# Daniel-Liu-c0deb0t/block-aligner

Measured on AMD Instinct MI355X. Metric: GCUPS (DP cells/s) on 10 kbp DNA X-drop batch; bit-exact score+CIGAR vs AVX2, higher is better.
Workload: dtype i16 (saturating lane scores) + i32 block offsets

## Files before the change

### block_aligner_amd/csrc/ba_driver.hpp

```cpp
#pragma once
#include "ba_device.hpp"

namespace ba {

#ifndef BA_BIG
#define BA_BIG 0
#endif
constexpr bool kBig = BA_BIG != 0;
__device__ __forceinline__ void lds_sync() {
    if (kBig) __builtin_amdgcn_fence(__ATOMIC_ACQ_REL, "workgroup");
    else __builtin_amdgcn_fence(__ATOMIC_ACQ_REL, "wavefront");
    __builtin_amdgcn_wave_barrier();
}
__device__ __forceinline__ void lds_fill0(short* a, uint32_t n) {
    for (uint32_t k = 2 * lane_id(); k < n; k += 128) *(int*)(a + k) = 0;
    lds_sync();
}
__device__ __forceinline__ void lds_copy(short* dst, const short* src, uint32_t n) {
    lds_sync();
    for (uint32_t k = 2 * lane_id(); k < n; k += 128) {
        const int v = *(const int*)(src + k);
        lds_sync();
        *(int*)(dst + k) = v;
    }
    lds_sync();
}
__device__ __forceinline__ int lds_prefix_max8(const short* a) {
    lds_sync();
    const int* p = (const int*)a;
    const s16x2 m = as_s(vmax(vmax(p[0], p[1]), vmax(p[2], p[3])));
    return uni(max((int)m.x, (int)m.y));
}
__device__ __forceinline__ int lds_suffix_max2(const short* a, uint32_t n) {
    lds_sync();
    s16x2 m = as_s(*(const int*)(a + n - 2));
    return uni(max((int)m.x, (int)m.y));
}
__device__ __forceinline__ int lds_shift_and_offset(uint32_t n, short* b1, short* b2, const short* t1, const short* t2, int off_add) {
    const int oa = splat(off_add);
    lds_sync();
    const int corner = uni((int)as_s(adds(splat((int)b1[STEP - 1]), oa)).x);
    for (uint32_t base = 0; base < n; base += 128) {
        const uint32_t k = base + 2 * lane_id();
        int v1 = 0, v2 = 0;
        const bool in = k < n;
        if (in) {
            if (k + STEP < n) {
                v1 = adds(*(const int*)(b1 + k + STEP), oa);
                v2 = adds(*(const int*)(b2 + k + STEP), oa);
            } else {
                v1 = *(const int*)(t1 + (k + STEP - n));
                v2 = *(const int*)(t2 + (k + STEP - n));
            }
        }
        lds_sync();
        if (in) { *(int*)(b1 + k) = v1; *(int*)(b2 + k) = v2; }
        lds_sync();
    }
    return corner;
}

struct Move { uint32_t op, di, dj, next; };
constexpr uint32_t TB_PENDING = 3;
__device__ __forceinline__ Move tb_lut(bool right_blk, uint32_t t, uint32_t t2, uint32_t table) {
    constexpr uint32_t OP_M = 1, OP_I = 4, OP_D = 5;
    const uint32_t gapA_op = right_blk ? OP_D : OP_I, gapB_op = right_blk ? OP_I : OP_D;
    const uint32_t A_di = right_blk ? 0 : 1, A_dj = right_blk ? 1 : 0;
    const uint32_t A_tab = right_blk ? 1 : 2, B_tab = right_blk ? 2 : 1;
    if (table == A_tab) return (t2 & 1) ? Move{gapA_op, A_di, A_dj, 0} : Move{gapA_op, A_di, A_dj, A_tab};
    if (table == B_tab) return Move{gapB_op, 1 - A_di, 1 - A_dj, TB_PENDING};
    if (t == 0) return Move{OP_M, 1, 1, 0};
    if (t & 1) return (t2 & 1) ? Move{gapA_op, A_di, A_dj, 0} : Move{gapA_op, A_di, A_dj, A_tab};
    return Move{gapB_op, 1 - A_di, 1 - A_dj, TB_PENDING};
}
__device__ __forceinline__ uint32_t tb_resolve(bool right_blk, uint32_t table, uint32_t nib) {
    return table == TB_PENDING ? ((nib & 8u) ? 0u : (right_blk ? 2u : 1u)) : table;
}
__device__ __forceinline__ uint32_t tb_next(bool right_blk, uint32_t next, uint32_t v) {
    return (next == TB_PENDING && v == 0) ? (right_blk ? 2u : 1u) : next;
}

__device__ __forceinline__ uint32_t traceback(const BlockRec* __restrict__ blocks, uint32_t nblocks, const uint32_t* __restrict__ trace,
                                     uint32_t i, uint32_t j, const uint8_t* __restrict__ q, const uint8_t* __restrict__ r, uint32_t flags,
                                     uint32_t* __restrict__ out, uint64_t out_lo, uint64_t out_hi, uint32_t* status) {
    const bool eq = flags & F_CIGAR_EQ, local = flags & F_LOCAL, fqs = flags & F_FQS;
    bool stop = false;
    uint64_t wp = out_hi;
    uint32_t run_op = 0, run_len = 0;
    uint32_t table = 0;
    uint32_t bidx = nblocks;
    while ((i > 0 || j > 0) && !stop) {
        BlockRec br;
        for (;;) {
            if (bidx == 0) { *status |= ST_TRACEBACK_LOST; return 0; }
            bidx--;
            br = blocks[bidx];
            if (i >= (br.i & 0x7fffffffu) && j >= br.j) break;
        }
        const bool right_blk = br.trace_base >> 31;
        const bool l2 = br.i >> 31;
        br.i &= 0x7fffffffu;
        if (br.trace_base & 0x40000000u) { *status |= ST_TRACEBACK_LOST; return 0; }
        const uint32_t tbase = br.trace_base & 0x3fffffffu;
        const uint32_t Hv = right_blk ? br.h : br.w;
        const uint32_t nch = Hv > 128 ? Hv / 128 : 1, nl = Hv > 128 ? 64 : Hv / 2;
        while (i >= br.i && j >= br.j && (i > 0 || j > 0)) {
            const uint32_t ci = i - br.i, cj = j - br.j;
            const uint32_t v = right_blk ? ci : cj, w = right_blk ? cj : ci;
            const uint32_t chunk = v >> 7, lane = (v & 127) >> 1;
            if (right_blk && fqs && i == 0) { stop = true; break; }
            uint32_t nib;
            if (l2) {
                const uint32_t word = trace[tbase + (v >> 3) * 8 + (w >> 1) * 2 + ((v >> 2) & 1)];
                nib = ((word >> ((v & 3) * 8 + (w & 1) * 4)) ^ 15u) & 15u;
            } else {
                const uint32_t word = trace[tbase + (((w >> 2) * nch + chunk) * nl + lane) * (local ? 2u : 1u)];
                nib = ((word >> ((v & 1) * 16 + (w & 3) * 4)) ^ 15u) & 15u;
            }
            table = tb_resolve(right_blk, table, nib);
            if (local && table == 0) {
                if (l2) {
                    const uint32_t z = trace[tbase + (uint32_t)br.h * br.w / 8 + (v >> 3) * 2 + ((v >> 2) & 1)];
                    if ((z >> ((v & 3) * 8 + w)) & 1) { stop = true; break; }
                } else {
                    const uint32_t z = trace[tbase + (((w >> 2) * nch + chunk) * nl + lane) * 2u + 1u];
                    if ((z >> ((v & 1) * 16 + (w & 3) * 4)) & 1) { stop = true; break; }
                }
            }
            const Move m = tb_lut(right_blk, nib & 3, (nib >> 2) & 1, table);
            uint32_t op = m.op;
            if (eq && op == 1) op = q[i] == r[j] ? 2 : 3;
            if (m.di > i || m.dj > j) { *status |= ST_TRACEBACK_LOST; return 0; }
            i -= m.di; j -= m.dj; table = tb_next(right_blk, m.next, v);
            if (op == run_op) run_len++;
            else {
                if (run_len) {
                    if (wp == out_lo) { *status |= ST_CIGAR_OVERFLOW; return 0; }
                    out[--wp] = (run_len << 4) | run_op;
                }
                run_op = op; run_len = 1;
            }
        }
    }
    if (run_len) {
        if (wp == out_lo) { *status |= ST_CIGAR_OVERFLOW; return 0; }
        out[--wp] = (run_len << 4) | run_op;
    }
    return (uint32_t)(out_hi - wp);
}

__device__ __forceinline__ uint32_t wave_excl_sum(uint32_t x, uint32_t lane) {
    uint32_t s = x;
#pragma unroll
    for (int d = 1; d < 64; d <<= 1) {
        const uint32_t o = (uint32_t)__shfl_up((int)s, d, 64);
        s += lane >= (uint32_t)d ? o : 0u;
    }
    return s - x;
}
template <bool L2OK>
__device__ __forceinline__ uint32_t walk_wave(const BlockRec* __restrict__ blocks, uint32_t nblocks_in, const uint32_t* __restrict__ trace,
                                              uint32_t i_in, uint32_t j_in, const uint8_t* __restrict__ q, const uint8_t* __restrict__ r, bool eq,
                                              uint32_t* __restrict__ out, uint64_t out_lo, uint64_t out_hi, uint32_t* status,
                                              uint32_t* __restrict__ lds, uint32_t budget) {
    const uint32_t lane = (uint32_t)lane_id();
    uint32_t lutv0, lutv1;
    {
        const Move a = tb_lut(false, lane & 3, (lane >> 2) & 1, (lane >> 4) & 3), b = tb_lut(true, lane & 3, (lane >> 2) & 1, (lane >> 4) & 3);
        lutv0 = a.op | (a.di << 3) | (a.dj << 4) | (a.next << 5);
        lutv1 = b.op | (b.di << 3) | (b.dj << 4) | (b.next << 5);
    }
    uint32_t i = (uint32_t)uni((int)i_in), j = (uint32_t)uni((int)j_in), bidx = (uint32_t)uni((int)nblocks_in);
    uint32_t table = 0, run_op = 0, run_len = 0, nrun = 0, runbuf = 0, st = 0;
    uint64_t wp = out_hi;
    uint32_t qw0 = 0, rw0 = 0, qwin = 0, rwin = 0;
    auto load_q = [&]() { qw0 = i >= 252u ? (i - 252u) & ~3u : 0u; const uint32_t a = qw0 + 4u * lane; qwin = a <= i ? *(const uint32_t*)(q + a) : 0u; };
    auto load_r = [&]() { rw0 = j >= 252u ? (j - 252u) & ~3u : 0u; const uint32_t a = rw0 + 4u * lane; rwin = a <= j ? *(const uint32_t*)(r + a) : 0u; };
    if (eq) { load_q(); load_r(); }
    auto flush = [&]() {
        if (lane < nrun) out[wp - 1u - lane] = runbuf;
        wp -= nrun; nrun = 0;
    };
    auto emit = [&]() -> bool {
        if (!run_len) return true;
        if (wp - nrun == out_lo) return false;
        asm volatile("s_mov_b32 m0, %2\n\tv_writelane_b32 %0, %1, m0" : "+v"(runbuf) : "s"(__builtin_amdgcn_readfirstlane((int)((run_len << 4) | run_op))), "s"(__builtin_amdgcn_readfirstlane((int)nrun)) : "m0");
        if (++nrun == 64u) flush();
        return true;
    };
    bool ok = true;
    while (ok && (i > 0 || j > 0)) {
        if (bidx == 0) { st = ST_TRACEBACK_LOST; ok = false; break; }
        const uint32_t nvalid = min(bidx, 64u);
        uint4 rec = uint4{0, 0, 0, 0};
        if (lane < nvalid) rec = *(const uint4*)(blocks + (bidx - 1u - lane));
        const bool untr = rec.w & 0x40000000u;
        const uint32_t words = untr ? 0u : (rec.z & 0xffffu) * (rec.z >> 16) / 8u;
        const uint32_t tb = rec.w & 0x3fffffffu;
        uint32_t toff = wave_excl_sum(lane < nvalid ? words : 0u, lane);
        const uint32_t nfit = (uint32_t)__popcll(__ballot(lane < nvalid && toff + words <= budget));
        const uint32_t tb_up = (uint32_t)__shfl_up((int)tb, 1, 64);
        const bool flat = nfit > 1 && !__any(lane > 0 && lane < nfit && tb + words != tb_up);
        if (nfit > 0) {
            const uint32_t total = (uint32_t)__builtin_amdgcn_readlane((int)(toff + words), (int)(nfit - 1u));
            if (flat) {
                const uint32_t lo = (uint32_t)__builtin_amdgcn_readlane((int)tb, (int)(nfit - 1u));
                for (uint32_t x = lane; x < total; x += 64u) lds[x] = trace[lo + x];
                toff = tb - lo;
            } else {
                for (uint32_t k = 0; k < nfit; k++) {
                    const uint32_t base = (uint32_t)__builtin_amdgcn_readlane((int)tb, (int)k), sz = (uint32_t)__builtin_amdgcn_readlane((int)words, (int)k);
                    const uint32_t off = (uint32_t)__builtin_amdgcn_readlane((int)toff, (int)k);
                    for (uint32_t x = lane; x < sz; x += 64u) lds[off + x] = trace[base + x];
                }
            }
            asm volatile("s_waitcnt vmcnt(0) lgkmcnt(0)" ::: "memory");
        }
        const bool direct = nfit == 0;
        const uint32_t ntake = direct ? 1u : nfit;
        auto walk_rects = [&](auto direct_c) {
        constexpr bool DIRECT = decltype(direct_c)::value;
        uint32_t cur = 0;
        while (cur < ntake && ok && (i > 0 || j > 0)) {
            const uint32_t rx = (uint32_t)__builtin_amdgcn_readlane((int)rec.x, (int)cur), bj = (uint32_t)__builtin_amdgcn_readlane((int)rec.y, (int)cur);
            const uint32_t bi = rx & 0x7fffffffu;
            if (!(i >= bi && j >= bj)) { cur++; continue; }
            const uint32_t rz = (uint32_t)__builtin_amdgcn_readlane((int)rec.z, (int)cur), rw = (uint32_t)__builtin_amdgcn_readlane((int)rec.w, (int)cur);
            if (rw & 0x40000000u) { st = ST_TRACEBACK_LOST; ok = false; break; }
            const uint32_t off = DIRECT ? (rw & 0x3fffffffu) : (uint32_t)__builtin_amdgcn_readlane((int)toff, (int)cur);
            const bool right = rw >> 31, l2 = L2OK && (rx >> 31);
            const uint32_t Hv = right ? (rz & 0xffffu) : (rz >> 16);
            const uint32_t nch = Hv > 128u ? Hv / 128u : 1u, nl = Hv > 128u ? 64u : Hv / 2u;
            const uint32_t lutr = right ? lutv1 : lutv0;
            while (i >= bi && j >= bj && (i > 0 || j > 0)) {
                const uint32_t ci = i - bi, cj = j - bj;
                const uint32_t v = right ? ci : cj, w = right ? cj : ci;
                uint32_t widx, sh;
                if (l2) { widx = (v >> 3) * 8u + (w >> 1) * 2u + ((v >> 2) & 1u); sh = (v & 3u) * 8u + (w & 1u) * 4u; }
                else { widx = ((w >> 2) * nch + (v >> 7)) * nl + ((v & 127u) >> 1); sh = (v & 1u) * 16u + (w & 3u) * 4u; }
                uint32_t word;
                if (table == 0u && i > 0u && j > 0u && min(v, w) >= 1u) {
                    const uint32_t lim = min(min(v, w), min(i, j) - 1u);
                    const bool valid = lane <= lim;
                    const uint32_t vv = v - lane, ww = w - lane;
                    uint32_t widx_k, sh_k;
                    if (l2) { widx_k = (vv >> 3) * 8u + (ww >> 1) * 2u + ((vv >> 2) & 1u); sh_k = (vv & 3u) * 8u + (ww & 1u) * 4u; }
                    else { widx_k = ((ww >> 2) * nch + (vv >> 7)) * nl + ((vv & 127u) >> 1); sh_k = (vv & 1u) * 16u + (ww & 3u) * 4u; }
                    uint32_t word_k = 0;
                    if (valid) { if constexpr (DIRECT) word_k = trace[off + widx_k]; else word_k = lds[off + widx_k]; }
                    const unsigned long long cm = __ballot(valid && ((word_k >> sh_k) & 3u) == 3u);
                    uint32_t n = cm == ~0ull ? 64u : (uint32_t)__builtin_ctzll(~cm);
                    if (eq && n >= 2u) {
                        if (i < qw0) load_q();
                        if (j < rw0) load_r();
                        n = min(n, min(i - qw0, j - rw0) + 1u);
                    }
                    if (n >= 2u) {
                        bool fits = true;
                        if (!eq) {
                            if (run_op == 1u) run_len += n;
                            else { fits = emit(); run_op = 1u; run_len = n; }
                        } else {
                            const uint32_t qa = i - lane - qw0, ra = j - lane - rw0;
                            const uint32_t qd = (uint32_t)__builtin_amdgcn_ds_bpermute((int)(qa & ~3u), (int)qwin), rd = (uint32_t)__builtin_amdgcn_ds_bpermute((int)(ra & ~3u), (int)rwin);
                            const bool same = ((qd >> ((qa & 3u) * 8u)) & 255u) == ((rd >> ((ra & 3u) * 8u)) & 255u);
                            unsigned long long bits = __ballot(lane < n && same);
                            uint32_t rem = n;
                            while (rem && fits) {
                                const bool e = bits & 1ull;
                                const unsigned long long x = e ? ~bits : bits;
                                const uint32_t len = min(x ? (uint32_t)__builtin_ctzll(x) : 64u, rem), op2 = e ? 2u : 3u;
                                if (op2 == run_op) run_len += len;
                                else { fits = emit(); run_op = op2; run_len = len; }
                                bits = len < 64u ? bits >> len : 0ull; rem -= len;
                            }
                        }
                        if (!fits) { st = ST_CIGAR_OVERFLOW; ok = false; break; }
                        i -= n; j -= n;
                        continue;
                    }
                    word = (uint32_t)__builtin_amdgcn_readlane((int)word_k, 0);
                } else {
                if constexpr (DIRECT) word = (uint32_t)uni((int)trace[off + widx]); else word = (uint32_t)uni((int)lds[off + widx]);
                }
                const uint32_t nib = ((word >> sh) ^ 15u) & 15u;
                table = tb_resolve(right, table, nib);
                const uint32_t m = (uint32_t)__builtin_amdgcn_readlane((int)lutr, (int)((table << 4) | nib));
                uint32_t op = m & 7u;
                const uint32_t di = (m >> 3) & 1u, dj = (m >> 4) & 1u;
                if (eq && op == 1u) {
                    if (i < qw0) load_q();
                    if (j < rw0) load_r();
                    const uint32_t qd = (uint32_t)__builtin_amdgcn_readlane((int)qwin, (int)((i - qw0) >> 2)), rd = (uint32_t)__builtin_amdgcn_readlane((int)rwin, (int)((j - rw0) >> 2));
                    op = ((qd >> ((i & 3u) * 8u)) & 255u) == ((rd >> ((j & 3u) * 8u)) & 255u) ? 2u : 3u;
                }
                if (di > i || dj > j) { st = ST_TRACEBACK_LOST; ok = false; break; }
                i -= di; j -= dj; table = tb_next(right, m >> 5, v);
                if (op == run_op) run_len++;
                else {
                    if (!emit()) { st = ST_CIGAR_OVERFLOW; ok = false; break; }
                    run_op = op; run_len = 1;
                }
            }
        }
        };
        if (direct) walk_rects(std::true_type{}); else walk_rects(std::false_type{});
        bidx -= ntake;
    }
    if (ok && !emit()) { st = ST_CIGAR_OVERFLOW; ok = false; }
    if (!ok) { *status |= st; return 0; }
    flush();
    return (uint32_t)(out_hi - wp);
}

#define BA_RLX_AGENT __ATOMIC_RELAXED, __HIP_MEMORY_SCOPE_AGENT

struct TbLane {
    uint32_t slot, pair, i, j, table, bidx, run_op, run_len, status;
    uint64_t wp, lo;
    const BlockRec* blocks; const uint32_t* trace; const uint8_t* q; const uint8_t* r;
    uint32_t bi, bj, tbase, zoff, nch, nl; bool right, in_rect, l2;
    uint4 nrec[4]; uint32_t nq;
    uint32_t tw_chunk, tw_g, tw_lane0; bool tw_ok;
    uint32_t qw0, rw0;
    uint32_t pv[6], po[6], pmask;
};

__device__ __forceinline__ void tb_emit(TbLane& t, uint32_t* __restrict__ out) {
    if (t.run_len) {
        if (t.wp == t.lo) { t.status |= ST_CIGAR_OVERFLOW; t.i = t.j = 0; return; }
        out[--t.wp] = (t.run_len << 4) | t.run_op;
    }
}
__device__ __forceinline__ void tb_fail(TbLane& t) { t.status |= ST_TRACEBACK_LOST; t.i = t.j = 0; t.run_len = 0; }

constexpr int TB_CELLS_PER_STEP = 4;
#ifndef BA_WALK_CELLS
#define BA_WALK_CELLS 8
#endif
#ifndef BA_RING_DEPTH
#define BA_RING_DEPTH 2
#endif
#ifndef BA_WALK_DEPTH
#define BA_WALK_DEPTH 4
#endif
#ifndef BA_HELPER_CELLS
#define BA_HELPER_CELLS 4
#endif
template <int CELLS = TB_CELLS_PER_STEP, int DEPTH = 1, int LB = (int)TB_LANE_BYTES>
__device__ __forceinline__ void tb_step(TbLane& t, uint32_t flags, uint32_t* __restrict__ out, unsigned char* lrec,
                                        const unsigned char* lut, unsigned long long* tacc = nullptr) {
    constexpr bool LOCREC = LB == (int)TB_LANE_BYTES_LOC;
    constexpr bool L2OK = LB == (int)TB_LANE_BYTES_L2 || LOCREC;
    constexpr int SEQ_Q = LOCREC ? 80 : (L2OK ? 64 : 40), SEQ_R = SEQ_Q + 16;
    const bool eq = flags & F_CIGAR_EQ, local = LOCREC && (flags & F_LOCAL), fqs = flags & F_FQS;
    BA_TSTAMP(ts0);
    if (!t.in_rect || !(t.i >= t.bi && t.j >= t.bj)) {
        bool found = false, untraced = false;
#pragma unroll
        for (int a = 0; a < DEPTH; a++) {
            if (!found && (a == 0 || t.nq)) {
                if (t.bidx == 0) { tb_fail(t); return; }
                uint4 rec;
                if (t.nq) {
                    rec = t.nrec[0];
#pragma unroll
                    for (int k = 0; k + 1 < DEPTH; k++) t.nrec[k] = t.nrec[k + 1];
                    t.nq--;
                } else rec = *(const uint4*)(t.blocks + t.bidx - 1);
                t.bidx--;
                t.l2 = L2OK && (rec.x >> 31); t.bi = rec.x & 0x7fffffffu; t.bj = rec.y;
                const uint32_t h = rec.z & 0xffffu, w = rec.z >> 16;
                t.in_rect = t.i >= t.bi && t.j >= t.bj;
                t.zoff = h * w / 8;
                t.right = rec.w >> 31;
                t.tbase = rec.w & 0x3fffffffu;
                const uint32_t Hv = t.right ? h : w;
                t.nch = Hv > 128 ? Hv / 128 : 1; t.nl = Hv > 128 ? 64 : Hv / 2;
                untraced = rec.w & 0x40000000u;
                found = t.in_rect;
            }
        }
        if (t.nq == 0 && t.bidx > 0) {
#pragma unroll
            for (int k = 0; k < DEPTH; k++) if (t.bidx > (uint32_t)k) t.nrec[k] = *(const uint4*)(t.blocks + t.bidx - 1 - k);
            t.nq = min((uint32_t)DEPTH, t.bidx);
        }
        t.tw_ok = false;
        if (!t.in_rect) return;
        if (untraced) { tb_fail(t); return; }
    }
    {
        const uint32_t ci = t.i - t.bi, cj = t.j - t.bj;
        const uint32_t v = t.right ? ci : cj, w = t.right ? cj : ci;
        const uint32_t chunk = v >> 7, lc = (v & 127) >> 1, g = w >> 2;
        if (L2OK && t.l2) {
            const uint32_t L8 = v >> 3;
            if (!(t.tw_ok && t.tw_chunk == 0xffffu && L8 - t.tw_lane0 < 2u)) {
                t.tw_chunk = 0xffffu; t.tw_g = 0; t.tw_lane0 = L8 ? L8 - 1 : 0u; t.tw_ok = true;
                const uint32_t* wp = t.trace + t.tbase + t.tw_lane0 * 8;
                uint4 a0, a1, a2, a3;
                __builtin_memcpy(&a0, wp, 16); __builtin_memcpy(&a1, wp + 4, 16); __builtin_memcpy(&a2, wp + 8, 16); __builtin_memcpy(&a3, wp + 12, 16);
                uint4* lw = (uint4*)lrec;
                lw[0] = a0; lw[1] = a1; lw[2] = a2; lw[3] = a3;
                if (local) {
                    uint4 z;
                    __builtin_memcpy(&z, t.trace + t.tbase + t.zoff + t.tw_lane0 * 2, 16);
                    lw[4] = z;
                }
            }
        } else
        if (local) {
            if (!(t.tw_ok && chunk == t.tw_chunk && t.tw_g - g < 2u && lc - t.tw_lane0 < 5u)) {
                t.tw_chunk = chunk; t.tw_g = g; t.tw_lane0 = min(lc >= 4 ? lc - 4 : 0u, t.nl - 5u); t.tw_ok = true;
                const uint32_t* hi = t.trace + t.tbase + ((g * t.nch + chunk) * t.nl + t.tw_lane0) * 2u;
                const uint32_t* lo = g ? hi - t.nch * t.nl * 2u : hi;
                uint4 h0, h1, l0, l1; uint2 h2, l2;
                __builtin_memcpy(&h0, hi, 16); __builtin_memcpy(&h1, hi + 4, 16); __builtin_memcpy(&h2, hi + 8, 8);
                __builtin_memcpy(&l0, lo, 16); __builtin_memcpy(&l1, lo + 4, 16); __builtin_memcpy(&l2, lo + 8, 8);
                uint32_t* lw = (uint32_t*)lrec;
                lw[0] = h0.x; lw[1] = h0.y; lw[2] = h0.z; lw[3] = h0.w; lw[4] = h1.x; lw[5] = h1.y; lw[6] = h1.z; lw[7] = h1.w; lw[8] = h2.x; lw[9] = h2.y;
                lw[10] = l0.x; lw[11] = l0.y; lw[12] = l0.z; lw[13] = l0.w; lw[14] = l1.x; lw[15] = l1.y; lw[16] = l1.z; lw[17] = l1.w; lw[18] = l2.x; lw[19] = l2.y;
            }
        } else
        if (!(t.tw_ok && chunk == t.tw_chunk && t.tw_g - g < 2u && lc - t.tw_lane0 < 5u)) {
            t.tw_chunk = chunk; t.tw_g = g; t.tw_lane0 = min(lc >= 4 ? lc - 4 : 0u, t.nl - 5u); t.tw_ok = true;
            const uint32_t* hi = t.trace + t.tbase + (g * t.nch + chunk) * t.nl + t.tw_lane0;
            const uint32_t* lo = g ? hi - t.nch * t.nl : hi;
            uint32_t wv[10];
            {
                uint4 h4, l4;
                __builtin_memcpy(&h4, hi, 16); __builtin_memcpy(&l4, lo, 16);
                wv[0] = h4.x; wv[1] = h4.y; wv[2] = h4.z; wv[3] = h4.w; wv[4] = hi[4];
                wv[5] = l4.x; wv[6] = l4.y; wv[7] = l4.z; wv[8] = l4.w; wv[9] = lo[4];
            }
#pragma unroll
            for (int k = 0; k < 10; k++) ((uint32_t*)lrec)[k] = wv[k];
        }
        if (eq) {
            if (t.qw0 == 0xffffffffu || t.i < t.qw0 + 8 || t.i >= t.qw0 + 16) {
                t.qw0 = t.i >= 12 ? (t.i - 12) & ~3u : 0;
                const uint32_t* p = (const uint32_t*)(t.q + t.qw0);
                uint32_t b4[4];
#pragma unroll
                for (int k = 0; k < 4; k++) b4[k] = p[k];
#pragma unroll
                for (int k = 0; k < 4; k++) ((uint32_t*)lrec)[SEQ_Q / 4 + k] = b4[k];
            }
            if (t.rw0 == 0xffffffffu || t.j < t.rw0 + 8 || t.j >= t.rw0 + 16) {
                t.rw0 = t.j >= 12 ? (t.j - 12) & ~3u : 0;
                const uint32_t* p = (const uint32_t*)(t.r + t.rw0);
                uint32_t b4[4];
#pragma unroll
                for (int k = 0; k < 4; k++) b4[k] = p[k];
#pragma unroll
                for (int k = 0; k < 4; k++) ((uint32_t*)lrec)[SEQ_R / 4 + k] = b4[k];
            }
        }
    }
#ifdef BA_TIMING
    const unsigned long long ts1 = __builtin_amdgcn_s_memtime();
    asm volatile("s_waitcnt vmcnt(0)" ::: "memory");
    const unsigned long long ts2 = __builtin_amdgcn_s_memtime();
    if (tacc) { tacc[0] += ts1 - ts0; tacc[1] += ts2 - ts1; }
#endif
    {
        bool alive = true;
#pragma unroll
        for (int s = 0; s < CELLS; s++) {
            alive = alive && (t.i > 0 || t.j > 0) && t.i >= t.bi && t.j >= t.bj;
            const uint32_t ci = t.i - t.bi, cj = t.j - t.bj;
            const uint32_t v = t.right ? ci : cj, w = t.right ? cj : ci;
            const uint32_t lc = (v & 127) >> 1;
            if (fqs) {
                const bool stop = alive && t.right && t.i == 0;
                if (stop) t.i = t.j = 0;
                alive = alive && !stop;
            }
            const uint32_t gi = t.tw_g - (w >> 2);
            uint32_t baddr, zaddr = 0, zbit = 0;
            if (L2OK && t.l2) {
                const uint32_t k8 = (v >> 3) - t.tw_lane0;
                alive = alive && t.tw_chunk == 0xffffu && k8 <= 1u;
                baddr = k8 * 32 + (w >> 1) * 8 + ((v >> 2) & 1) * 4 + (v & 3);
                zaddr = 64 + k8 * 8 + ((v >> 2) & 1) * 4 + (v & 3); zbit = w;
            } else {
                const uint32_t k = lc - t.tw_lane0;
                alive = alive && (v >> 7) == t.tw_chunk && gi <= 1u && k <= 4u;
                baddr = local ? gi * 40 + k * 8 + (v & 1) * 2 + ((w & 3) >> 1) : gi * 20 + k * 4 + (v & 1) * 2 + ((w & 3) >> 1);
                zaddr = baddr + 4; zbit = (w & 1) * 4;
            }
            const uint32_t qo = t.i - t.qw0, ro = t.j - t.rw0;
            const uint32_t byte = lrec[alive ? baddr : 0u];
            const uint32_t qb = lrec[SEQ_Q + (qo & 15u)], rb = lrec[SEQ_R + (ro & 15u)];
            const uint32_t nib = ((byte >> ((w & 1) * 4)) ^ 15u) & 15u;
            const uint32_t table = tb_resolve(t.right, t.table, nib);
            if (local) {
                const uint32_t zb = lrec[alive ? zaddr : 0u];
                const bool stop = alive && table == 0 && ((zb >> zbit) & 1u);
                if (stop) t.i = t.j = 0;
                alive = alive && !stop;
            }
            const uint32_t m = lut[((uint32_t)t.right << 6) | (table << 4) | nib];
            uint32_t op = m & 7u;
            const uint32_t di = (m >> 3) & 1u, dj = (m >> 4) & 1u;
            const bool is_match = eq && op == 1;
            alive = alive && !(is_match && (qo > 15u || ro > 15u));
            if (is_match) op = qb == rb ? 2u : 3u;
            if (alive && (di > t.i || dj > t.j)) { tb_fail(t); alive = false; }
            const bool same = op == t.run_op;
            if (alive && !same && t.run_len) {
                if (t.wp == t.lo) { t.status |= ST_CIGAR_OVERFLOW; t.i = t.j = 0; alive = false; }
                else out[--t.wp] = (t.run_len << 4) | t.run_op;
            }
            t.i -= alive ? di : 0u; t.j -= alive ? dj : 0u;
            t.table = alive ? tb_next(t.right, m >> 5, v) : t.table;
            t.run_len = alive ? (same ? t.run_len + 1 : 1u) : t.run_len;
            t.run_op = alive ? op : t.run_op;
        }
    }
}

#ifndef BA_TB_FAST
#define BA_TB_FAST 1
#endif
#ifndef BA_TB_FCELLS
#define BA_TB_FCELLS 1
#endif
#ifndef BA_TB_DIAG_RUNS
#define BA_TB_DIAG_RUNS 2
#endif
#ifndef BA_TB_DIAG2
#define BA_TB_DIAG2 1
#endif
#ifndef BA_TB_FDEPTH
#define BA_TB_FDEPTH 3
#endif
typedef uint32_t tb_u32x4 __attribute__((ext_vector_type(4)));
__device__ __forceinline__ uint4 tb_ld16(const void* p) {
    typedef tb_u32x4 __attribute__((aligned(4))) V;
    const tb_u32x4 v = *(const V*)p;
    return uint4{v.x, v.y, v.z, v.w};
}
__device__ __forceinline__ uint32_t ffbl_u32(uint32_t x) { uint32_t r; asm("v_ffbl_b32 %0, %1" : "=v"(r) : "v"(x)); return r; }
__device__ __forceinline__ void tb_prefetch2(TbLane& t) {
    if (t.bidx > 0u) t.nrec[0] = *(const uint4*)(t.blocks + t.bidx - 1);
    if (t.bidx > 1u) t.nrec[1] = *(const uint4*)(t.blocks + t.bidx - 2);
    t.nq = min(2u, t.bidx);
}
template <bool L2W>
__device__ __forceinline__ void tb_diag_lut_fill(unsigned char* dlut) {
    if constexpr (L2W) {
#pragma unroll
        for (int e = 0; e < 3; e++) {
            const uint32_t idx = (uint32_t)lane_id() + 64u * e;
            const uint32_t k = idx & 7u, p = idx >> 3;
            const uint32_t x = (p - k) & 15u, c = ((p - 16u) - k) & 7u;
            dlut[idx] = (unsigned char)(p < 16u ? (((x & 8u) << 2) | (x & 7u)) : ((c >> 1) << 3));
        }
    }
    {
        const uint32_t idx = (uint32_t)lane_id(), k = idx & 7u, x = ((idx >> 3) - k) & 7u;
        dlut[(L2W ? TB_DIAG_LUT_L2 - TB_DIAG_LUT_STD : 0u) + idx] = (unsigned char)((x < 4u ? 20u : 0u) + ((x & 3u) >> 1));
    }
}
template <int S>
__device__ __forceinline__ void tb_push(TbLane& t, const bool cond, const uint32_t val, bool& ovf) {
    const bool room = t.wp != t.lo, go = cond && room;
    t.wp -= go ? 1u : 0u;
    t.pv[S] = go ? val : t.pv[S];
    t.po[S] = go ? (uint32_t)t.wp - (uint32_t)t.lo : t.po[S];
    t.pmask |= go ? (1u << S) : 0u;
    ovf = ovf || (cond && !room);
}
__device__ __forceinline__ void tb_flush(TbLane& t, uint32_t* __restrict__ out) {
#pragma unroll
    for (int s = 0; s < 6; s++) if ((t.pmask >> s) & 1u) out[t.lo + t.po[s]] = t.pv[s];
    t.pmask = 0;
}

template <bool L2W, int SEQ_Q, int SEQ_R, int S0>
__device__ __forceinline__ void tb_diag(TbLane& t, const bool eq, const unsigned char* lrec, const unsigned char* dlut, bool& ovf) {
    static_assert(BA_TB_DIAG_RUNS >= 1 && BA_TB_DIAG_RUNS <= 2, "two slots per call site");
    const uint32_t ci = t.i - t.bi, cj = t.j - t.bj;
    const uint32_t v = t.right ? ci : cj, w = t.right ? cj : ci;
    bool ok = t.in_rect && t.tw_ok && t.i >= t.bi && t.j >= t.bj && (t.table == 0u || t.table == TB_PENDING);
    uint32_t K = min(min(t.i, t.j), min(v, w) + 1u);
    uint32_t alo, ahi;
    {
        const uint32_t u = (v & 127u) - 2u * t.tw_lane0, x = w + 4u - 4u * t.tw_g;
        const bool ok_s = !t.l2 && (v >> 7) == t.tw_chunk && u < 10u && x < 8u;
        const uint32_t K_s = min(u, x) + 1u;
        const uint2 C = *(const uint2*)(dlut + (L2W ? TB_DIAG_LUT_L2 - TB_DIAG_LUT_STD : 0u) + (x & 7u) * 8u);
        const uint32_t r2 = (2u * (u & 15u)) * 0x01010101u;
        alo = ((r2 - 0x06040200u) + C.x) & 0x3f3f3f3fu; ahi = ((r2 - 0x0e0c0a08u) + C.y) & 0x3f3f3f3fu;
        if constexpr (L2W) {
            const uint32_t u2 = v - 8u * t.tw_lane0;
            const bool ok_2 = t.l2 && t.tw_chunk == 0xffffu && u2 < 16u;
            const uint2 F = *(const uint2*)(dlut + (u2 & 15u) * 8u), G = *(const uint2*)(dlut + 128u + (w & 7u) * 8u);
            alo = t.l2 ? F.x + G.x : alo; ahi = t.l2 ? F.y + G.y : ahi;
            ok = ok && (ok_2 || ok_s);
            K = min(K, t.l2 ? u2 + 1u : K_s);
        } else {
            ok = ok && ok_s;
            K = min(K, K_s);
        }
    }
    const uint32_t qo = t.i - t.qw0, ro = t.j - t.rw0;
    if (eq) { ok = ok && qo <= 15u && ro <= 15u; K = min(K, min(qo, ro) + 1u); }
    K = ok ? min(K, 8u) : 0u;
    uint32_t b[8];
#pragma unroll
    for (int k = 0; k < 8; k++) b[k] = lrec[((k < 4 ? alo : ahi) >> (8 * (k & 3))) & 0xffu];
    const uint32_t sh0 = (w & 1u) * 4u;
    const uint32_t e4 = (b[0] | (b[2] << 8) | (b[4] << 16) | (b[6] << 24)) >> sh0, o4 = (b[1] | (b[3] << 8) | (b[5] << 16) | (b[7] << 24)) >> (4u - sh0);
    const uint32_t z = ((e4 & (e4 >> 1)) & 0x01010101u) | (((o4 & (o4 >> 1)) & 0x01010101u) << 4);
    uint32_t n = ffbl_u32(~z & 0x11111111u) >> 2;
    const bool d_state = t.table == 0u || !((e4 >> 3) & 1u);
    n = d_state ? min(n, K) : 0u;
    uint32_t ne = 0;
    if (eq) {
        const unsigned char* qb = lrec + SEQ_Q + (ok ? qo : 7u) - 7u; const unsigned char* rb = lrec + SEQ_R + (ok ? ro : 7u) - 7u;
#pragma unroll
        for (int k = 0; k < 8; k++) ne |= min((uint32_t)qb[7 - k] ^ (uint32_t)rb[7 - k], 1u) << (4 * k);
    }
    uint32_t pos = 0;
#pragma unroll
    for (int it = 0; it < (BA_TB_DIAG_RUNS); it++) {
        if (it > 0 && !eq) break;
        const uint32_t rem = n - pos;
        const uint32_t cur = ne >> ((4u * pos) & 31u);
        const uint32_t is_x = cur & 1u;
        const uint32_t y = (cur ^ (0u - is_x)) & 0x11111111u;
        const uint32_t len = min(ffbl_u32(y) >> 2, rem);
        const uint32_t op = eq ? 2u + is_x : 1u;
        const bool same = op == t.run_op;
        if (it == 0) tb_push<S0>(t, rem > 0u && !same && t.run_len != 0u, (t.run_len << 4) | t.run_op, ovf);
        else tb_push<S0 + 1>(t, rem > 0u && !same && t.run_len != 0u, (t.run_len << 4) | t.run_op, ovf);
        t.run_len = same ? t.run_len + len : (rem > 0u ? len : t.run_len);
        t.run_op = rem > 0u ? op : t.run_op;
        pos += len;
    }
    t.i -= pos; t.j -= pos;
    t.table = pos ? 0u : t.table;
}

template <int DEPTH, int LB>
__device__ __forceinline__ void tb_step_fast(TbLane& t, const bool eq, uint32_t* __restrict__ out, unsigned char* lrec, const unsigned char* lut, const unsigned char* dlut) {
    static_assert(DEPTH >= 2 && DEPTH <= 4 && (BA_TB_FCELLS) >= 1 && (BA_TB_FCELLS) <= 2, "");
    constexpr bool L2OK = LB == (int)TB_LANE_BYTES_L2;
    constexpr int SEQ_Q = L2OK ? 64 : 40, SEQ_R = SEQ_Q + 16;
    if (!t.in_rect || !(t.i >= t.bi && t.j >= t.bj)) {
        if (t.bidx == 0) { tb_fail(t); return; }
        bool found = false;
        uint32_t take = t.nq;
        uint4 rec = t.nrec[0];
#pragma unroll
        for (int a = DEPTH - 1; a >= 0; a--) {
            const bool c = (uint32_t)a < t.nq && t.i >= (t.nrec[a].x & 0x7fffffffu) && t.j >= t.nrec[a].y;
            rec.x = c ? t.nrec[a].x : rec.x; rec.y = c ? t.nrec[a].y : rec.y; rec.z = c ? t.nrec[a].z : rec.z; rec.w = c ? t.nrec[a].w : rec.w;
            take = c ? (uint32_t)a + 1u : take;
            found = found || c;
        }
        const uint32_t nq_old = t.nq;
        t.bidx -= take;
        uint4 nn[DEPTH];
#pragma unroll
        for (int k = 0; k < DEPTH; k++) {
            nn[k] = t.nrec[k];
            bool have = false;
#pragma unroll
            for (int sft = 1; k + sft < DEPTH; sft++) {
                const bool m = take == (uint32_t)sft && (uint32_t)(k + sft) < nq_old;
                nn[k].x = m ? t.nrec[k + sft].x : nn[k].x; nn[k].y = m ? t.nrec[k + sft].y : nn[k].y; nn[k].z = m ? t.nrec[k + sft].z : nn[k].z; nn[k].w = m ? t.nrec[k + sft].w : nn[k].w;
                have = have || m;
            }
            if (!have && t.bidx > (uint32_t)k) nn[k] = *(const uint4*)(t.blocks + t.bidx - 1 - k);
        }
#pragma unroll
        for (int k = 0; k < DEPTH; k++) t.nrec[k] = nn[k];
        t.nq = min((uint32_t)DEPTH, t.bidx);
        t.in_rect = found;
        t.l2 = L2OK && (rec.x >> 31); t.bi = rec.x & 0x7fffffffu; t.bj = rec.y;
        t.right = rec.w >> 31;
        t.tbase = rec.w & 0x3fffffffu;
        const uint32_t Hv = t.right ? (rec.z & 0xffffu) : (rec.z >> 16);
        t.nch = Hv > 128 ? Hv / 128 : 1; t.nl = Hv > 128 ? 64 : Hv / 2;
        t.tw_ok = false;
        if (!found) return;
        if (rec.w & 0x40000000u) { tb_fail(t); return; }
    }
    const uint32_t ci0 = t.i - t.bi, cj0 = t.j - t.bj;
    const uint32_t v0 = t.right ? ci0 : cj0, w0 = t.right ? cj0 : ci0;
    const bool is_l2 = L2OK && t.l2;
    bool ld_l2 = false, ld_std = false;
    if constexpr (L2OK) {
        const uint32_t L8 = v0 >> 3;
        ld_l2 = is_l2 && !(t.tw_ok && t.tw_chunk == 0xffffu && L8 - t.tw_lane0 < 2u);
        if (ld_l2) { t.tw_chunk = 0xffffu; t.tw_g = 0; t.tw_lane0 = L8 ? L8 - 1 : 0u; t.tw_ok = true; }
    }
    {
        const uint32_t chunk = v0 >> 7, lc = (v0 & 127) >> 1, g = w0 >> 2;
        ld_std = !is_l2 && !(t.tw_ok && chunk == t.tw_chunk && t.tw_g - g < 2u && lc - t.tw_lane0 < 5u);
        if (ld_std) { t.tw_chunk = chunk; t.tw_g = g; t.tw_lane0 = min(lc >= 4 ? lc - 4 : 0u, t.nl - 5u); t.tw_ok = true; }
    }
    uint4 wa = {0, 0, 0, 0}, wb = {0, 0, 0, 0}, wc = {0, 0, 0, 0}, wd = {0, 0, 0, 0};
    {
        const uint32_t* tb0 = t.trace + t.tbase;
        const uint32_t o_hi = (t.tw_g * t.nch + t.tw_chunk) * t.nl + t.tw_lane0, o_lo = t.tw_g ? o_hi - t.nch * t.nl : o_hi;
        const uint32_t o_l2 = t.tw_lane0 * 8;
        const uint32_t o0 = is_l2 ? o_l2 : o_hi, o1 = is_l2 ? o_l2 + 4 : o_lo, o2 = is_l2 ? o_l2 + 8 : o_hi + 4, o3 = is_l2 ? o_l2 + 12 : o_lo + 4;
        if (ld_l2 || ld_std) { wa = tb_ld16(tb0 + o0); wb = tb_ld16(tb0 + o1); wc = tb_ld16(tb0 + o2); wd = tb_ld16(tb0 + o3); }
    }
    uint4 qv = {0, 0, 0, 0}, rv = {0, 0, 0, 0};
    const bool ld_q = eq && (t.qw0 == 0xffffffffu || t.i < t.qw0 + 8 || t.i >= t.qw0 + 16);
    const bool ld_r = eq && (t.rw0 == 0xffffffffu || t.j < t.rw0 + 8 || t.j >= t.rw0 + 16);
    if (ld_q) { t.qw0 = t.i >= 12 ? (t.i - 12) & ~3u : 0; qv = tb_ld16(t.q + t.qw0); }
    if (ld_r) { t.rw0 = t.j >= 12 ? (t.j - 12) & ~3u : 0; rv = tb_ld16(t.r + t.rw0); }
    tb_flush(t, out);
    if constexpr (L2OK) if (ld_l2) { uint4* lw = (uint4*)lrec; lw[0] = wa; lw[1] = wb; lw[2] = wc; lw[3] = wd; }
    if (ld_std) {
        uint32_t* lw = (uint32_t*)lrec;
        lw[0] = wa.x; lw[1] = wa.y; lw[2] = wa.z; lw[3] = wa.w; lw[4] = wc.x; lw[5] = wb.x; lw[6] = wb.y; lw[7] = wb.z; lw[8] = wb.w; lw[9] = wd.x;
    }
    if (ld_q) { uint32_t* lw = (uint32_t*)lrec + SEQ_Q / 4; lw[0] = qv.x; lw[1] = qv.y; lw[2] = qv.z; lw[3] = qv.w; }
    if (ld_r) { uint32_t* lw = (uint32_t*)lrec + SEQ_R / 4; lw[0] = rv.x; lw[1] = rv.y; lw[2] = rv.z; lw[3] = rv.w; }
    bool ovf = false;
    tb_diag<L2OK, SEQ_Q, SEQ_R, 0>(t, eq, lrec, dlut, ovf);
    {
        bool alive = true;
#pragma unroll
        for (int s = 0; s < (BA_TB_FCELLS); s++) {
            alive = alive && (t.i > 0 || t.j > 0) && t.i >= t.bi && t.j >= t.bj;
            const uint32_t ci = t.i - t.bi, cj = t.j - t.bj;
            const uint32_t v = t.right ? ci : cj, w = t.right ? cj : ci;
            const uint32_t lc = (v & 127) >> 1;
            const uint32_t gi = t.tw_g - (w >> 2);
            uint32_t baddr;
            if (L2OK && t.l2) {
                const uint32_t k8 = (v >> 3) - t.tw_lane0;
                alive = alive && t.tw_chunk == 0xffffu && k8 <= 1u;
                baddr = k8 * 32 + (w >> 1) * 8 + ((v >> 2) & 1) * 4 + (v & 3);
            } else {
                const uint32_t k = lc - t.tw_lane0;
                alive = alive && (v >> 7) == t.tw_chunk && gi <= 1u && k <= 4u;
                baddr = gi * 20 + k * 4 + (v & 1) * 2 + ((w & 3) >> 1);
            }
            const uint32_t qo = t.i - t.qw0, ro = t.j - t.rw0;
            const uint32_t byte = lrec[alive ? baddr : 0u];
            const uint32_t qb = lrec[SEQ_Q + (qo & 15u)], rb = lrec[SEQ_R + (ro & 15u)];
            const uint32_t nib = ((byte >> ((w & 1) * 4)) ^ 15u) & 15u;
            const uint32_t table = tb_resolve(t.right, t.table, nib);
            const uint32_t m = lut[((uint32_t)t.right << 6) | (table << 4) | nib];
            uint32_t op = m & 7u;
            const uint32_t di = (m >> 3) & 1u, dj = (m >> 4) & 1u;
            const bool is_match = eq && op == 1;
            alive = alive && !(is_match && (qo > 15u || ro > 15u));
            if (is_match) op = qb == rb ? 2u : 3u;
            if (alive && (di > t.i || dj > t.j)) { tb_fail(t); alive = false; }
            const bool same = op == t.run_op;
            if (s == 0) tb_push<2>(t, alive && !same && t.run_len != 0u, (t.run_len << 4) | t.run_op, ovf);
            else tb_push<3>(t, alive && !same && t.run_len != 0u, (t.run_len << 4) | t.run_op, ovf);
            t.i -= alive ? di : 0u; t.j -= alive ? dj : 0u;
            t.table = alive ? tb_next(t.right, m >> 5, v) : t.table;
            t.run_len = alive ? (same ? t.run_len + 1 : 1u) : t.run_len;
            t.run_op = alive ? op : t.run_op;
        }
    }
    if constexpr ((BA_TB_DIAG2) != 0) tb_diag<L2OK, SEQ_Q, SEQ_R, 4>(t, eq, lrec, dlut, ovf);
    if (ovf) { t.status |= ST_CIGAR_OVERFLOW; t.i = t.j = 0; }
}

template <int LB = (int)TB_LANE_BYTES, int CELLS = TB_CELLS_PER_STEP, int DEPTH = BA_RING_DEPTH>
__device__ __forceinline__ void traceback_consumer(const BatchParams& bp, uint32_t flag_mask, unsigned char* tb_lds, uint32_t nlanes, bool dedicated, int prio = -1) {
    enum { IDLE = 0, WAIT = 1, WALK = 2, RETIRED = 3 };
    int phase = (uint32_t)lane_id() < nlanes ? IDLE : RETIRED;
    uint32_t claimed = 0, pend = 0;
    const uint32_t reserve_from = bp.n > bp.tb_reserve ? bp.n - bp.tb_reserve : 0u;
    TbLane t{};
    const uint32_t eq = bp.flags & flag_mask;
    uint32_t* head = bp.tb_ctrl + 32;
    unsigned char* lut = tb_lds;
    unsigned char* lrec = tb_lds + TB_LUT_BYTES + (uint32_t)lane_id() * (uint32_t)LB;
    constexpr bool FASTP = (BA_TB_FAST) != 0 && LB != (int)TB_LANE_BYTES_LOC;
    unsigned char* dlut = tb_lds + ((TB_LUT_BYTES + nlanes * (uint32_t)LB + 7u) & ~7u);
#pragma unroll
    for (int e = 0; e < 2; e++) {
        const uint32_t idx = (uint32_t)lane_id() + 64u * e;
        const Move mv = tb_lut(idx >> 6, idx & 3, (idx >> 2) & 1, (idx >> 4) & 3);
        lut[idx] = (unsigned char)(mv.op | (mv.di << 3) | (mv.dj << 4) | (mv.next << 5));
    }
    if constexpr (FASTP) tb_diag_lut_fill<LB == (int)TB_LANE_BYTES_L2>(dlut);
    lds_sync();
#ifndef BA_TB_PRIO
#define BA_TB_PRIO 3
#endif
#ifndef MQ_TB_PRIO
#define MQ_TB_PRIO 1
#endif
    if (prio == 1) __builtin_amdgcn_s_setprio(MQ_TB_PRIO); else __builtin_amdgcn_s_setprio(BA_TB_PRIO);
#ifdef BA_TIMING
    unsigned long long c_sec[3] = {};
    unsigned long long c_iters = 0, c_walk_lanes = 0, c_walk_iters = 0, c_poll_iters = 0, c_walk_ticks = 0, c_t0 = __builtin_amdgcn_s_memtime();
#endif
    for (;;) {
#ifdef BA_TIMING
        const unsigned long long it0 = __builtin_amdgcn_s_memtime();
        const bool any_walk = __any(phase == WALK);
        c_iters++; c_walk_lanes += __popcll(__ballot(phase == WALK)); c_walk_iters += any_walk; c_poll_iters += __any(phase == WAIT);
#endif
        if (phase == IDLE) {
            if (dedicated && __hip_atomic_load(head, BA_RLX_AGENT) >= reserve_from) phase = RETIRED;
            else {
                claimed = __hip_atomic_fetch_add(head, 1u, BA_RLX_AGENT);
                phase = claimed >= bp.n ? RETIRED : WAIT;
            }
            pend = 0;
        }
        const bool got = phase == WAIT && pend != 0;
        const bool walking = phase == WALK;
        const uint32_t entry = pend;
        if (__any(got)) {
            __builtin_amdgcn_fence(__ATOMIC_ACQUIRE, "agent");
            if (got) __hip_atomic_store(bp.tb_queue + (claimed & bp.tb_qmask), 0u, BA_RLX_AGENT);
            if (got && (entry & 0x80000000u)) {
                bp.cig_len[entry & 0x7fffffffu] = 0;
                phase = IDLE;
            } else if (got) {
                t = TbLane{};
                t.qw0 = t.rw0 = 0xffffffffu; t.tw_ok = false;
                t.slot = entry - 1;
                const SlotInfo si = bp.slot_info[t.slot];
                t.pair = si.pair; t.i = si.end_i; t.j = si.end_j; t.bidx = si.nblocks;
                t.blocks = bp.blocks + (uint64_t)t.slot * bp.blocks_stride;
                t.trace = bp.trace_arena + (uint64_t)t.slot * bp.trace_stride;
                t.q = bp.pool + bp.q_off[t.pair]; t.r = bp.pool + bp.r_off[t.pair];
                t.lo = bp.cig_off[t.pair]; t.wp = bp.cig_off[t.pair + 1];
                t.status = bp.status[t.pair];
                if (t.status || (bp.flags & 0x200u)) t.i = t.j = 0;
                if constexpr (FASTP) tb_prefetch2(t);
                phase = WALK;
            }
        }
        if (walking) {
#ifdef BA_TIMING
            const unsigned long long tq0 = __builtin_amdgcn_s_memtime();
            if (t.i > 0 || t.j > 0) {
                if constexpr (FASTP) tb_step_fast<BA_TB_FDEPTH, LB>(t, eq != 0u, bp.cig_ops, lrec, lut, dlut);
                else tb_step<CELLS, DEPTH, LB>(t, eq, bp.cig_ops, lrec, lut, c_sec);
            }
            c_sec[2] += __builtin_amdgcn_s_memtime() - tq0;
#else
            if (t.i > 0 || t.j > 0) {
                if constexpr (FASTP) tb_step_fast<BA_TB_FDEPTH, LB>(t, eq != 0u, bp.cig_ops, lrec, lut, dlut);
                else
                if (BA_HELPER_CELLS != CELLS && !dedicated) tb_step<BA_HELPER_CELLS, BA_WALK_DEPTH, LB>(t, eq, bp.cig_ops, lrec, lut);
                else tb_step<CELLS, DEPTH, LB>(t, eq, bp.cig_ops, lrec, lut);
            }
#endif
            if (!(t.i > 0 || t.j > 0)) {
                if constexpr (FASTP) tb_flush(t, bp.cig_ops);
                tb_emit(t, bp.cig_ops);
                bp.cig_len[t.pair] = t.status ? 0u : (uint32_t)(bp.cig_off[t.pair + 1] - t.wp);
                if (t.status) bp.status[t.pair] = t.status;
                __hip_atomic_store(bp.slot_free + t.slot, 1u, BA_RLX_AGENT);
                phase = IDLE;
            }
        }
        if (phase == WAIT) pend = __hip_atomic_load(bp.tb_queue + (claimed & bp.tb_qmask), BA_RLX_AGENT);
#ifdef BA_TIMING
        if (any_walk) c_walk_ticks += __builtin_amdgcn_s_memtime() - it0;
#endif
        if (__all(phase == RETIRED)) break;
        if (!__any(phase == WALK)) __builtin_amdgcn_s_sleep(32);
    }
#ifdef BA_TIMING
    if (bp.prof && dedicated && is_lane(0)) {
        atomicAdd(bp.prof + 20, c_iters); atomicAdd(bp.prof + 21, c_walk_lanes); atomicAdd(bp.prof + 22, c_walk_iters);
        atomicAdd(bp.prof + 23, c_poll_iters); atomicAdd(bp.prof + 24, c_walk_ticks);
        atomicAdd(bp.prof + 25, __builtin_amdgcn_s_memtime() - c_t0); atomicAdd(bp.prof + 26, 1ull);
        atomicAdd(bp.prof + 27, c_sec[0]); atomicAdd(bp.prof + 28, c_sec[1]); atomicAdd(bp.prof + 29, c_sec[2]);
    }
#endif
}

template <int LB = (int)TB_LANE_BYTES>
__device__ __forceinline__ bool traceback_help_one(const BatchParams& bp, uint32_t flag_mask, unsigned char* tb_lds) {
    uint32_t entry = 0;
    if (is_lane(0)) {
        uint32_t h = __hip_atomic_load(bp.tb_ctrl + 32, BA_RLX_AGENT);
        if (h < bp.n) {
            const uint32_t e = __hip_atomic_load(bp.tb_queue + (h & bp.tb_qmask), BA_RLX_AGENT);
            if (e && __hip_atomic_compare_exchange_strong(bp.tb_ctrl + 32, &h, h + 1u, __ATOMIC_RELAXED, __ATOMIC_RELAXED, __HIP_MEMORY_SCOPE_AGENT)) {
                entry = e;
                __hip_atomic_store(bp.tb_queue + (h & bp.tb_qmask), 0u, BA_RLX_AGENT);
            }
        }
    }
    entry = (uint32_t)uni((int)entry);
    if (!entry) return false;
    if (entry & 0x80000000u) {
        if (is_lane(0)) bp.cig_len[entry & 0x7fffffffu] = 0;
        return true;
    }
    unsigned char* lut = tb_lds;
    unsigned char* lrec = tb_lds + TB_LUT_BYTES;
    lds_sync();
#pragma unroll
    for (int e = 0; e < 2; e++) {
        const uint32_t idx = (uint32_t)lane_id() + 64u * e;
        const Move mv = tb_lut(idx >> 6, idx & 3, (idx >> 2) & 1, (idx >> 4) & 3);
        lut[idx] = (unsigned char)(mv.op | (mv.di << 3) | (mv.dj << 4) | (mv.next << 5));
    }
    lds_sync();
    __builtin_amdgcn_fence(__ATOMIC_ACQUIRE, "agent");
    if (is_lane(0)) {
        const uint32_t eq = bp.flags & flag_mask;
        TbLane t{};
        t.qw0 = t.rw0 = 0xffffffffu; t.tw_ok = false;
        t.slot = entry - 1;
        const SlotInfo si = bp.slot_info[t.slot];
        t.pair = si.pair; t.i = si.end_i; t.j = si.end_j; t.bidx = si.nblocks;
        t.blocks = bp.blocks + (uint64_t)t.slot * bp.blocks_stride;
        t.trace = bp.trace_arena + (uint64_t)t.slot * bp.trace_stride;
        t.q = bp.pool + bp.q_off[t.pair]; t.r = bp.pool + bp.r_off[t.pair];
        t.lo = bp.cig_off[t.pair]; t.wp = bp.cig_off[t.pair + 1];
        t.status = bp.status[t.pair];
        if (t.status || (bp.flags & 0x200u)) t.i = t.j = 0;
        while (t.i > 0 || t.j > 0) tb_step<TB_CELLS_PER_STEP, BA_RING_DEPTH, LB>(t, eq, bp.cig_ops, lrec, lut);
        tb_emit(t, bp.cig_ops);
        bp.cig_len[t.pair] = t.status ? 0u : (uint32_t)(bp.cig_off[t.pair + 1] - t.wp);
        if (t.status) bp.status[t.pair] = t.status;
        __hip_atomic_store(bp.slot_free + t.slot, 1u, BA_RLX_AGENT);
    }
    lds_sync();
    return true;
}

template <bool L2OK>
__device__ __forceinline__ void traceback_helper_wave(const BatchParams& bp, uint32_t* lds, uint32_t budget) {
    uint32_t* head = bp.tb_ctrl + 32;
    for (;;) {
        uint32_t claimed = 0;
        if (is_lane(0)) claimed = __hip_atomic_fetch_add(head, 1u, BA_RLX_AGENT);
        claimed = (uint32_t)uni((int)claimed);
        if (claimed >= bp.n) break;
        uint32_t entry = 0;
        for (;;) {
            if (is_lane(0)) entry = __hip_atomic_load(bp.tb_queue + (claimed & bp.tb_qmask), BA_RLX_AGENT);
            entry = (uint32_t)uni((int)entry);
            if (entry) break;
            __builtin_amdgcn_s_sleep(32);
        }
        __builtin_amdgcn_fence(__ATOMIC_ACQUIRE, "agent");
        if (is_lane(0)) __hip_atomic_store(bp.tb_queue + (claimed & bp.tb_qmask), 0u, BA_RLX_AGENT);
        if (entry & 0x80000000u) { if (is_lane(0)) bp.cig_len[entry & 0x7fffffffu] = 0; continue; }
        const uint32_t slot = entry - 1;
        const SlotInfo si = bp.slot_info[slot];
        const uint32_t pair = (uint32_t)uni((int)si.pair);
        uint32_t st = bp.status[pair], ncig = 0;
        lds_sync();
        if (!st && !(bp.flags & 0x200u))
            ncig = walk_wave<L2OK>(bp.blocks + (uint64_t)slot * bp.blocks_stride, si.nblocks, bp.trace_arena + (uint64_t)slot * bp.trace_stride, si.end_i, si.end_j,
                                   bp.pool + bp.q_off[pair], bp.pool + bp.r_off[pair], (bp.flags & F_CIGAR_EQ) != 0, bp.cig_ops, bp.cig_off[pair], bp.cig_off[pair + 1],
                                   &st, lds, budget);
        lds_sync();
        if (is_lane(0)) {
            bp.cig_len[pair] = st ? 0u : ncig;
            if (st) bp.status[pair] = st;
            __hip_atomic_store(bp.slot_free + slot, 1u, BA_RLX_AGENT);
        }
    }
}

template <bool L2OK = false, bool LOC = false>
__device__ __forceinline__ void traceback_all(const BatchParams& bp, uint32_t flag_mask, unsigned char* tb_lds) {
    constexpr int LB = LOC ? (int)TB_LANE_BYTES_LOC : (L2OK ? (int)TB_LANE_BYTES_L2 : (int)TB_LANE_BYTES);
    constexpr uint32_t WAVE_LDS = LOC ? TB_LDS_BYTES_LOC : (L2OK ? TB_LDS_BYTES_L2 : TB_LDS_BYTES);
    const uint32_t eq = bp.flags & flag_mask;
    unsigned char* lut = tb_lds;
    unsigned char* lrec = tb_lds + TB_LUT_BYTES + (uint32_t)lane_id() * (uint32_t)LB;
    constexpr bool FASTP = (BA_TB_FAST) != 0 && !LOC;
    unsigned char* dlut = tb_lds + ((TB_LUT_BYTES + 64u * (uint32_t)LB + 7u) & ~7u);
    static_assert(LOC || ((TB_LUT_BYTES + 64u * (uint32_t)LB + 7u) & ~7u) + (L2OK ? TB_DIAG_LUT_L2 : TB_DIAG_LUT_STD) <= WAVE_LDS, "k_walk LDS: tb_diag's tables");
#pragma unroll
    for (int e = 0; e < 2; e++) {
        const uint32_t idx = (uint32_t)lane_id() + 64u * e;
        const Move mv = tb_lut(idx >> 6, idx & 3, (idx >> 2) & 1, (idx >> 4) & 3);
        lut[idx] = (unsigned char)(mv.op | (mv.di << 3) | (mv.dj << 4) | (mv.next << 5));
    }
    if constexpr (FASTP) tb_diag_lut_fill<L2OK>(dlut);
    lds_sync();
    TbLane t{};
    bool walking = false, more = true;
    const uint32_t filter = bp.cont_mode;
    const uint32_t spec_flags = bp.flags & (F_LOCAL | F_FQS);
    const uint32_t n_wave = (LOC || spec_flags) ? 0u : min(bp.walk_wave_n, bp.n);
    if (n_wave) {
        __builtin_amdgcn_s_setprio(3);
        for (;;) {
            uint32_t p = 0;
            if (is_lane(0)) p = atomicAdd(bp.work_counter + 1, 1u);
            p = (uint32_t)uni((int)p);
            if (p >= n_wave) break;
            bool mine = true;
            if (filter) mine = (bp.cont_in_flag[p] == 0) == (filter == 1);
            SlotInfo si{0, 0, 0, 0};
            if (mine) { si = bp.slot_info[p]; mine = si.nblocks != ~0u; }
            if (!mine) continue;
            uint32_t st = bp.status[p], ncig = 0;
            if (!st && !(bp.flags & 0x200u))
                ncig = walk_wave<L2OK>(bp.blocks + bp.blocks_off[p], si.nblocks, bp.trace_arena + bp.trace_off[p], si.end_i, si.end_j, bp.pool + bp.q_off[p],
                                       bp.pool + bp.r_off[p], eq != 0, bp.cig_ops, bp.cig_off[p], bp.cig_off[p + 1], &st, (uint32_t*)tb_lds, WAVE_LDS / 4u);
            if (is_lane(0)) { bp.cig_len[p] = st ? 0u : ncig; if (st) bp.status[p] = st; }
        }
        __builtin_amdgcn_s_setprio(0);
        lds_sync();
#pragma unroll
        for (int e = 0; e < 2; e++) {
            const uint32_t idx = (uint32_t)lane_id() + 64u * e;
            const Move mv = tb_lut(idx >> 6, idx & 3, (idx >> 2) & 1, (idx >> 4) & 3);
            lut[idx] = (unsigned char)(mv.op | (mv.di << 3) | (mv.dj << 4) | (mv.next << 5));
        }
        if constexpr (FASTP) tb_diag_lut_fill<L2OK>(dlut);
        lds_sync();
    }
    uint32_t w_next = 0, w_end = 0;
    for (;;) {
        if (!__all(walking) && (more || w_next != w_end)) {
            if (w_next == w_end) {
                uint32_t base = 0;
                if (is_lane(0)) base = atomicAdd(bp.work_counter, 64u);
                base = (uint32_t)uni((int)base) + n_wave;
                if (base >= bp.n) { more = false; base = 0; w_next = w_end = 0; }
                else { w_next = base; w_end = min(base + 64u, bp.n); }
            }
            const unsigned long long im = __ballot(!walking);
            const uint32_t rank = (uint32_t)__popcll(im & ((1ull << lane_id()) - 1ull));
            const uint32_t take = min((uint32_t)__popcll(im), w_end - w_next);
            const uint32_t p = w_next + rank;
            w_next += take;
            bool mine = !walking && rank < take;
            if (filter && mine) mine = (bp.cont_in_flag[p] == 0) == (filter == 1);
            SlotInfo si{0, 0, 0, 0};
            if (mine) { si = bp.slot_info[p]; mine = si.nblocks != ~0u; }
            if (mine) {
                t = TbLane{};
                t.qw0 = t.rw0 = 0xffffffffu; t.tw_ok = false;
                t.slot = p; t.pair = p; t.i = si.end_i; t.j = si.end_j; t.bidx = si.nblocks;
                t.blocks = bp.blocks + bp.blocks_off[p];
                t.trace = bp.trace_arena + bp.trace_off[p];
                t.q = bp.pool + bp.q_off[p]; t.r = bp.pool + bp.r_off[p];
                t.lo = bp.cig_off[p]; t.wp = bp.cig_off[p + 1];
                t.status = bp.status[p];
                if (t.status || (bp.flags & 0x200u)) t.i = t.j = 0;
                if constexpr (FASTP) tb_prefetch2(t);
                walking = true;
            }
        }
        if (!__any(walking)) break;
        if (walking) {
            if (t.i > 0 || t.j > 0) {
                if constexpr (LOC) tb_step<BA_WALK_CELLS, BA_WALK_DEPTH, LB>(t, spec_flags | (eq ? (uint32_t)F_CIGAR_EQ : 0u), bp.cig_ops, lrec, lut);
                else if constexpr (FASTP) { if (eq) tb_step_fast<BA_TB_FDEPTH, LB>(t, true, bp.cig_ops, lrec, lut, dlut); else tb_step_fast<BA_TB_FDEPTH, LB>(t, false, bp.cig_ops, lrec, lut, dlut); }
                else
                if (eq) tb_step<BA_WALK_CELLS, BA_WALK_DEPTH, LB>(t, (uint32_t)F_CIGAR_EQ, bp.cig_ops, lrec, lut);
                else tb_step<BA_WALK_CELLS, BA_WALK_DEPTH, LB>(t, 0u, bp.cig_ops, lrec, lut);
            }
            if (!(t.i > 0 || t.j > 0)) {
                if constexpr (FASTP) tb_flush(t, bp.cig_ops);
                tb_emit(t, bp.cig_ops);
                bp.cig_len[t.pair] = t.status ? 0u : (uint32_t)(bp.cig_off[t.pair + 1] - t.wp);
                if (t.status) bp.status[t.pair] = t.status;
                walking = false;
            }
        }
    }
}

struct PairState {
    uint32_t si, sj; int dir, prev_dir, off, off_max, best_max; uint32_t y_drop_iter; int x_drop_iter, D_corner;
    uint32_t best_i, best_j, ck_i, ck_j; int ck_off; uint32_t ck_tt, ck_nb;
    unsigned long long cells; uint32_t step_budget, trace_top, nblocks, status;
    int exited;
};
constexpr uint32_t MQ_B = 128;
enum { MM_NONE = -1, MM_FRESH = 0, MM_RESUME = 1 };

struct NoState { int exited; };
template <int PMAX, int KIND, bool TRACE, bool XDROP, bool SPECIAL, bool MULTI = false, int SLOT_B_ = 128>
struct Aligner {
    static constexpr uint32_t SLOT_B = (uint32_t)SLOT_B_;
    typedef std::conditional_t<MULTI, PairState, NoState> RunOut;
    uint32_t h_flags, h_max_size; int h_x_drop;
    typedef const __attribute__((address_space(4))) BatchParams* ColdPtr;
    __device__ __forceinline__ static ColdPtr coldp() {
        ColdPtr p = (ColdPtr)__builtin_amdgcn_kernarg_segment_ptr();
        asm volatile("" : "+s"(p));
        return p;
    }
    const WaveLds& L;
    const FillConsts& fc;
    const uint8_t* q; const uint8_t* r;
    uint32_t qlen, rlen;
    uint32_t* trace; BlockRec* blocks; short* ckpt;
    short* big_top = nullptr;
    uint32_t trace_top = 0, nblocks = 0;
    int parked = 0;
    uint32_t status = 0;
    unsigned long long cells = 0;
    int pf_qv = 0, pf_rv = 0;
    unsigned long long pf_qc = 0, pf_rc = 0;
    bool pf_ok = false;
#ifdef BA_TIMING
    unsigned long long prof[48] = {};
#else
    unsigned long long* prof = nullptr;
#endif
    typedef const __attribute__((address_space(4))) unsigned long long* ConstU64;
    __device__ __forceinline__ static unsigned long long load_cols(const uint8_t* p) {
        return *(ConstU64)(uintptr_t)p;
    }
    __device__ __forceinline__ void prefetch_seq(uint32_t si, uint32_t sj, uint32_t B) {
        const int lane = lane_id();
        pf_qv = *(const unsigned short*)(q + si + 2 * lane);
        pf_rv = *(const unsigned short*)(r + sj + 2 * lane);
        pf_qc = load_cols(q + si + B);
        pf_rc = load_cols(r + sj + B);
        pf_ok = true;
    }
    int ck_reg[4] = {0, 0, 0, 0};
    bool ck_in_regs = false;
    bool chain = false;

    __device__ __forceinline__ static bool fast_eligible(uint32_t ri, uint32_t B, uint32_t lenV, uint32_t rj, uint32_t lenC) {
        return XDROP || ri + B <= lenV || rj + STEP <= lenC;
    }

    enum { RUN_EXIT_POST = 0, RUN_EXIT_TOP = 1, RUN_EXIT_FATAL = 2 };
    struct RunState {
        uint32_t si, sj; int dir, prev_dir, off, prev_off, off_max, off_add, best_max; uint32_t y_drop_iter; int x_drop_iter, D_corner;
        uint32_t step_budget; int run_exit; Best cur; FastOut fo;
    };
    __device__ __forceinline__ RunState fast_run(const RunState in, int corner, const uint32_t B, const uint32_t min_size, const uint32_t max_size, const bool one_step = false) {
        uint32_t si = in.si, sj = in.sj; int dir = in.dir, prev_dir = in.prev_dir, off = in.off, prev_off = in.prev_off, off_max = in.off_max;
        int off_add = in.off_add, best_max = in.best_max; uint32_t y_drop_iter = in.y_drop_iter; int x_drop_iter = in.x_drop_iter, D_corner = in.D_corner;
        uint32_t step_budget = in.step_budget; int run_exit = RUN_EXIT_POST; FastOut fo{};
        constexpr int PR_DIST = (int)(lds_array_bytes_h(kBig ? 128u : (uint32_t)PMAX * 128u) / 2);
        const int lane = lane_id();
        const int nl = (int)(B >> 1);
        int Dcol, Ccol, Drow, Rrow;
        lds_sync();
        Dcol = *(const int*)(L.D_col + 2 * lane); Ccol = *(const int*)(L.C_col + 2 * lane);
        Drow = *(const int*)(L.D_row + 2 * lane); Rrow = *(const int*)(L.R_row + 2 * lane);
        lds_sync();
        bool improved = false;
        int n_best_i = 0, n_best_j = 0, n_ck_i = 0, n_ck_j = 0, n_ck_off = 0, n_ck_tt = 0, n_ck_nb = 0;
        Best cur{0, 0, 0};
        for (;;) {
            const bool right = dir == DIR_RIGHT;
            const uint8_t* seqV = right ? q : r; const uint8_t* seqC = right ? r : q;
            const uint32_t ri = right ? si : sj, rj = (right ? sj : si) + B - STEP;
            int vc; unsigned long long cb;
            if (pf_ok) { vc = right ? pf_qv : pf_rv; cb = right ? pf_rc : pf_qc; }
            else {
                vc = 2 * lane < (int)B ? (int)*(const unsigned short*)(seqV + ri + 2 * lane) : 0;
                cb = load_cols(seqC + rj);
            }
            asm volatile("" : "+v"(vc));
            const uint32_t tb = trace_top;
            if (TRACE) {
                if (right) add_block(ri, rj, STEP, B, true);
                else add_block(rj, ri, B, STEP, false);
                if (status) { run_exit = RUN_EXIT_FATAL; break; }
            }
            uint32_t* tout = TRACE ? trace + tb : nullptr;
            const int loc_thr = best_max - off + ZERO;
            const bool sp_local = SPECIAL && (h_flags & F_LOCAL);
            const int rz2 = SPECIAL ? (sp_local ? splat(clamp16(-off + ZERO)) : (int)0x80008000u) : 0;
#define BA_FAST(LANES) do { if (right) fast_rect<KIND, TRACE, XDROP, LANES, PR_DIST, SPECIAL>(L.table, fc, Dcol, Ccol, Drow, Rrow, L.D_row, L.D_col, vc & 0xff, (vc >> 8) & 0xff, cb, nl, corner, off_add, loc_thr, tout, fo, rz2, sp_local); \
                           else fast_rect<KIND, TRACE, XDROP, LANES, PR_DIST, SPECIAL>(L.table, fc, Drow, Rrow, Dcol, Ccol, L.D_col, L.D_row, vc & 0xff, (vc >> 8) & 0xff, cb, nl, corner, off_add, loc_thr, tout, fo, rz2, sp_local); } while (0)
            if (B == 128) BA_FAST(64); else if (B == 32) BA_FAST(16); else if (B == 64) BA_FAST(32); else BA_FAST(0);
#undef BA_FAST
            cells += (unsigned long long)(STEP * B);
            prefetch_seq(si, sj, B);
            cur = Best{fo.mx, fo.row, fo.col};

            const int right_max = right ? fo.act_max8 : fo.pas_max8, down_max = right ? fo.pas_max8 : fo.act_max8;
            const int mx = fo.mx;
            const int new_off_max = off + mx - ZERO;
            const bool improve = new_off_max > best_max;
            const uint32_t new_y = improve ? 0u : y_drop_iter + 1;
            const bool q_out = si + B > qlen, r_out = sj + B > rlen;
            bool leave = q_out && r_out;
            if (XDROP) leave = leave || (!improve && new_off_max < best_max - h_x_drop && x_drop_iter >= 1);
            if (!q_out && !r_out) {
                leave = leave || (2 * B <= max_size && new_y > B / STEP - 1);
                if (B > min_size && new_y == 0) {
                    const s16x2 a = as_s(__builtin_amdgcn_readlane(Drow, nl - 1)), b = as_s(__builtin_amdgcn_readlane(Dcol, nl - 1));
                    leave = leave || max(max((int)a.x, (int)a.y), max((int)b.x, (int)b.y)) >= mx;
                }
            }
            if (TRACE && chain && improve) leave = true;
            if (leave) { run_exit = RUN_EXIT_POST; break; }

            off_max = new_off_max; y_drop_iter = new_y; prev_dir = dir; D_corner = fo.corner_new;
            if (improve) {
                improved = true;
                if (XDROP) {
                    if (right) { n_best_i = (int)(si + (uint32_t)cur.row); n_best_j = (int)(sj + (B - STEP) + (uint32_t)cur.col); }
                    else { n_best_i = (int)(si + (B - STEP) + (uint32_t)cur.col); n_best_j = (int)(sj + (uint32_t)cur.row); }
                }
                if (B < max_size) {
                    n_ck_i = (int)si; n_ck_j = (int)sj; n_ck_off = off;
                    ck_reg[0] = Dcol; ck_reg[1] = Ccol; ck_reg[2] = Drow; ck_reg[3] = Rrow; ck_in_regs = true;
                    if (TRACE) { n_ck_tt = (int)trace_top; n_ck_nb = (int)nblocks; }
                }
                best_max = off_max;
            }
            if (XDROP) {
                if (off_max < best_max - h_x_drop) x_drop_iter++;
                else x_drop_iter = 0;
            }
            const bool go_down = r_out || (!q_out && down_max > right_max);
            si += go_down ? (uint32_t)STEP : 0u; sj += go_down ? 0u : (uint32_t)STEP;
            dir = go_down ? DIR_DOWN : DIR_RIGHT;

            if (one_step || !fast_eligible(dir == DIR_RIGHT ? si : sj, B, dir == DIR_RIGHT ? qlen : rlen, (dir == DIR_RIGHT ? sj : si) + B - STEP, dir == DIR_RIGHT ? rlen : qlen)) { run_exit = RUN_EXIT_TOP; break; }
            if (--step_budget == 0) { status |= ST_WATCHDOG; run_exit = RUN_EXIT_FATAL; break; }
#ifdef BA_TIMING
            prof[16]++;
#endif
            prev_off = off; off = off_max;
            off_add = clamp16(prev_off - off);
            corner = prev_dir != dir ? (int)as_s(adds(splat(D_corner), splat(off_add))).x : 0;
        }
        lds_sync();
        if (lane < nl) {
            *(int*)(L.D_col + 2 * lane) = Dcol; *(int*)(L.C_col + 2 * lane) = Ccol;
            *(int*)(L.D_row + 2 * lane) = Drow; *(int*)(L.R_row + 2 * lane) = Rrow;
        }
        lds_sync();
        if (improved) {
            if (XDROP) { park<5>(parked, n_best_i); park<6>(parked, n_best_j); }
            if (B < max_size) {
// ... 398 lines not shown
                D_corner = fo.corner_new;
            } else if (dir == DIR_RIGHT) {
                right_max = lds_prefix_max8(L.D_col);
                D_corner = lds_shift_and_offset(block_size, L.D_row, L.R_row, temp1, temp2, off_add);
                down_max = lds_prefix_max8(L.D_row);
            } else if (dir == DIR_DOWN) {
                down_max = lds_prefix_max8(L.D_row);
                D_corner = lds_shift_and_offset(block_size, L.D_col, L.C_col, temp1, temp2, off_add);
                right_max = lds_prefix_max8(L.D_col);
            } else {
                right_max = lds_prefix_max8(L.D_col);
                down_max = lds_prefix_max8(L.D_row);
                save_ckpt_borders(block_size);
                if (TRACE) { park<3>(parked, (int)trace_top); park<4>(parked, (int)nblocks); }
            }

            BA_TSTAMP(tpa);
            const int this_dir = dir;
            prev_dir = dir;
            const bool was_grow = dir == DIR_GROW;
            const int D_max_max = FQE ? fq.M : cur.mx, grow_max = was_grow ? unpark<9>(parked) : 0;
            const int mx = max(D_max_max, grow_max);
            off_max = off + mx - ZERO;
            if (TRACE && chain && off_max > best_max) { rollback(); continue; }
            if (TRACE && no_spec && off_max > best_max) no_spec = false;
            y_drop_iter++;
            bool grow_no_max = this_dir == DIR_GROW;

            if (off_max > best_max) {
                if (FQE) {
                    park<5>(parked, (int)qlen);
                    if (this_dir == DIR_RIGHT) park<6>(parked, (int)(sj + (block_size - STEP) + (uint32_t)fq.j));
                    else if (this_dir == DIR_GROW) park<6>(parked, (int)(sj + prev_size + (uint32_t)fq.j));
                    else status |= ST_MODE;
                }
                if (XDROP) {
                    uint32_t bi_, bj_;
                    if (this_dir == DIR_RIGHT) { bi_ = si + cur.row; bj_ = sj + (block_size - STEP) + cur.col; }
                    else if (this_dir == DIR_DOWN) { bi_ = si + (block_size - STEP) + cur.col; bj_ = sj + cur.row; }
                    else if (D_max_max >= grow_max) { bi_ = si + cur.row; bj_ = sj + prev_size + cur.col; }
                    else { bi_ = si + prev_size + (uint32_t)unpark<11>(parked); bj_ = sj + (uint32_t)unpark<10>(parked); }
                    park<5>(parked, (int)bi_); park<6>(parked, (int)bj_);
                }
                if (block_size < max_size) {
                    park<0>(parked, (int)si); park<1>(parked, (int)sj); park<2>(parked, off);
                    save_ckpt_borders(block_size);
                    if (TRACE) { park<3>(parked, (int)trace_top); park<4>(parked, (int)nblocks); }
                    grow_no_max = false;
                }
                best_max = off_max;
                y_drop_iter = 0;
            }
            BA_TSTAMP(tpb);
            if (XDROP) {
                if (off_max < best_max - h_x_drop) {
                    if (x_drop_iter < 1) x_drop_iter++;
                    else break;
                } else x_drop_iter = 0;
            }
            BA_TSTAMP(ts3);
            BA_TADD(prof, 14, ts2, ts3);
            BA_TADD(prof, 35, ts2, tpa); BA_TADD(prof, 36, tpa, tpb); BA_TADD(prof, 37, tpb, ts3);
            if (si + block_size > qlen && sj + block_size > rlen) {
                if (TRACE && chain && !XDROP) { rollback(); continue; }
                break;
            }
            if (sj + block_size > rlen) { si += STEP; dir = DIR_DOWN; continue; }
            if (si + block_size > qlen) { sj += STEP; dir = DIR_RIGHT; continue; }

            const uint32_t next_size = block_size * 2;
            if (next_size <= max_size && (y_drop_iter > block_size / STEP - 1 || grow_no_max)) {
                if constexpr (CLASS_BET) { if (next_size > CLASS_CAP) { status |= ST_CLASS_OVERFLOW; break; } }
                if (TRACE && XDROP && KIND != KIND_PROFILE && !SPECIAL && !kBig && !chain && !no_spec && !(h_flags & 0x400u)) {
                    ub_size = block_size; ub_tt = (uint32_t)unpark<3>(parked); ub_nb = (uint32_t)unpark<4>(parked);
                    ub_xiter = x_drop_iter; ub_cells = cells; ub_budget = step_budget;
                    copy_ckpt(true, block_size);
                    chain = true;
                }
                prev_size = block_size; block_size = next_size; dir = DIR_GROW;
                si = (uint32_t)unpark<0>(parked); sj = (uint32_t)unpark<1>(parked); off = unpark<2>(parked);
                restore_ckpt_borders(prev_size);
                if (TRACE) { trace_top = (uint32_t)unpark<3>(parked); nblocks = (uint32_t)unpark<4>(parked); }
                y_drop_iter = 0;
                continue;
            }
            if (block_size > min_size && y_drop_iter == 0) {
                const int shrink_max = max(lds_suffix_max2(L.D_row, block_size), lds_suffix_max2(L.D_col, block_size));
                if (shrink_max >= mx) {
                    pf_ok = false;
                    prev_dir = DIR_GROW;
                    block_size /= 2;
                    lds_copy(L.D_col, L.D_col + block_size, block_size); lds_copy(L.C_col, L.C_col + block_size, block_size);
                    lds_copy(L.D_row, L.D_row + block_size, block_size); lds_copy(L.R_row, L.R_row + block_size, block_size);
                    si += block_size; sj += block_size;
                    park<0>(parked, (int)si); park<1>(parked, (int)sj); park<2>(parked, off);
                    save_ckpt_borders(block_size);
                    right_max = lds_prefix_max8(L.D_col);
                    down_max = lds_prefix_max8(L.D_row);
                    if (TRACE) { park<3>(parked, (int)trace_top); park<4>(parked, (int)nblocks); }
                    y_drop_iter = 0;
                }
            }
            if (down_max > right_max) { si += STEP; dir = DIR_DOWN; }
            else { sj += STEP; dir = DIR_RIGHT; }
        }

        BA_TSTAMP(tr1);
        BA_TADD(prof, 15, tr0, tr1);
#ifdef BA_TIMING
        prof[16] += steps;
#endif
        if (TRACE && XDROP && chain && coldp()->prof) {
            uint32_t sc = 0;
            const uint32_t first = ub_nb < nblocks ? ub_nb : nblocks;
            for (uint32_t k = first + (uint32_t)lane_id(); k < nblocks; k += 64u) {
                const uint32_t* rp = (const uint32_t*)(blocks + k);
                const uint32_t hw = __hip_atomic_load(rp + 2, BA_RLX_AGENT), tb = __hip_atomic_load(rp + 3, BA_RLX_AGENT);
                if (tb & 0x40000000u) sc += (hw & 0xffffu) * (hw >> 16);
            }
#pragma unroll
            for (int d = 32; d >= 1; d >>= 1) sc += (uint32_t)__shfl_xor((int)sc, d, 64);
            if (is_lane(0) && sc && !(status & ST_CLASS_OVERFLOW)) atomicAdd(coldp()->prof + 60, (unsigned long long)sc);
        }
        if constexpr (XDROP && (KIND == KIND_NUC || KIND == KIND_AA) && !SPECIAL && !kBig) {
            const uint32_t sk = (uint32_t)unpark<14>(parked);
            if (sk && coldp()->prof && is_lane(0) && !(status & ST_CLASS_OVERFLOW)) atomicAdd(coldp()->prof + 61, (unsigned long long)sk);
        }
        const uint32_t pair = (uint32_t)unpark<7>(parked), slot = (uint32_t)unpark<8>(parked);
        int score; uint32_t ri, rj;
        if (XDROP || FQE) { score = best_max; ri = (uint32_t)unpark<5>(parked); rj = (uint32_t)unpark<6>(parked); }
        else {
            lds_sync();
            if (dir == DIR_DOWN) score = off + uni((int)L.D_row[rlen - sj]) - ZERO;
            else score = off + uni((int)L.D_col[qlen - si]) - ZERO;
            ri = qlen; rj = rlen;
        }
        uint32_t ncig = 0;
        if (TRACE && batch_traceback) {
            if (is_lane(0)) {
                coldp()->score[pair] = score; coldp()->query_idx[pair] = ri; coldp()->reference_idx[pair] = rj;
                if (coldp()->cells) coldp()->cells[pair] = cells;
                if (coldp()->nblocks_out) coldp()->nblocks_out[pair] = nblocks;
                if (coldp()->trace_words_out) coldp()->trace_words_out[pair] = trace_top;
            }
            hand_off(slot, pair, ri, rj);
            return mout;
        }
        const bool walk_later = TRACE && coldp()->trace_off && qlen + rlen < coldp()->inline_len2 && !(MULTI && walk_now && !SPECIAL);
        if (TRACE && coldp()->cig_ops && !status && !walk_later) {
            __builtin_amdgcn_fence(__ATOMIC_SEQ_CST, "agent");
            if constexpr (SPECIAL) {
                if (is_lane(0)) {
                    uint32_t st = 0;
                    ncig = traceback(blocks, nblocks, trace, ri, rj, q, r, h_flags, coldp()->cig_ops, coldp()->cig_off[pair], coldp()->cig_off[pair + 1], &st);
                    status |= st;
                }
            } else {
                uint32_t st = 0;
                lds_sync();
                ncig = walk_wave<MULTI>(blocks, nblocks, trace, ri, rj, q, r, (h_flags & F_CIGAR_EQ) != 0, coldp()->cig_ops, coldp()->cig_off[pair],
                                        coldp()->cig_off[pair + 1], &st, (uint32_t*)L.D_col, lds_array_bytes_h(kBig ? 128u : (uint32_t)PMAX * 128u));
                lds_sync();
                status |= st;
            }
        }
        if (is_lane(0)) {
            coldp()->score[pair] = score; coldp()->query_idx[pair] = ri; coldp()->reference_idx[pair] = rj;
            if (coldp()->cig_len) coldp()->cig_len[pair] = ncig;
            if (coldp()->cells) coldp()->cells[pair] = cells;
            if (coldp()->status) coldp()->status[pair] = status;
            if (coldp()->nblocks_out) coldp()->nblocks_out[pair] = nblocks;
            if (coldp()->trace_words_out) coldp()->trace_words_out[pair] = trace_top;
            if (coldp()->slot_out) coldp()->slot_out[pair] = slot;
            if (TRACE && coldp()->trace_off) coldp()->slot_info[pair] = SlotInfo{pair, walk_later ? nblocks : ~0u, ri, rj};
        }
        return mout;
    }

    __device__ __forceinline__ void import_slot(const int (&reg)[16], const int (&ckr)[16], uint32_t pair_in, bool have_ck, bool ck_pre, int ck_dir, int ck_offadd, int ck_corner,
                                                uint32_t ck_i, uint32_t ck_j, uint32_t& best_i, uint32_t& best_j, int ck_off = 0) {
        constexpr int SLOT_LANES = (int)SLOT_B / 8;
        const int lane = lane_id(), l8 = 8 * (lane & (SLOT_LANES - 1));
        const bool mine = lane < SLOT_LANES;
        q = coldp()->pool + coldp()->q_off[pair_in]; r = coldp()->pool + coldp()->r_off[pair_in];
        if (have_ck) {
            lds_sync();
            if (mine) {
                *(int4*)(L.D_col + l8) = int4{ckr[0], ckr[1], ckr[2], ckr[3]}; *(int4*)(L.C_col + l8) = int4{ckr[4], ckr[5], ckr[6], ckr[7]};
                *(int4*)(L.D_row + l8) = int4{ckr[8], ckr[9], ckr[10], ckr[11]}; *(int4*)(L.R_row + l8) = int4{ckr[12], ckr[13], ckr[14], ckr[15]};
            }
            lds_sync();
            constexpr bool WIDE = SLOT_B > 128;
            constexpr int NCH_S = WIDE ? (int)SLOT_B / 128 : 1;
            int cDc = 0, cCc = 0, cDr = 0, cRr = 0;
            if constexpr (!WIDE) {
                cDc = *(const int*)(L.D_col + 2 * lane); cCc = *(const int*)(L.C_col + 2 * lane);
                cDr = *(const int*)(L.D_row + 2 * lane); cRr = *(const int*)(L.R_row + 2 * lane);
                lds_sync();
            }
            if (ck_pre) {
                constexpr int PR_DIST = (int)(lds_array_bytes_h(kBig ? 128u : (uint32_t)PMAX * 128u) / 2);
                const bool cright = ck_dir == DIR_RIGHT;
                const uint8_t* seqV = cright ? q : r; const uint8_t* seqC = cright ? r : q;
                const uint32_t cri = cright ? ck_i : ck_j, crj = (cright ? ck_j : ck_i) + SLOT_B - STEP;
                FastOut fo{};
                if constexpr (KIND != KIND_PROFILE && !SPECIAL && !WIDE) {
                    constexpr int FL = (int)SLOT_B / 2;
                    const int vc = 2 * lane < (int)SLOT_B ? (int)*(const unsigned short*)(seqV + cri + 2 * lane) : 0;
                    const unsigned long long cb = load_cols(seqC + crj);
                    if (cright) fast_rect<KIND, false, XDROP, FL, PR_DIST>(L.table, fc, cDc, cCc, cDr, cRr, L.D_row, L.D_col, vc & 0xff, (vc >> 8) & 0xff, cb, FL, ck_corner, ck_offadd, -1, nullptr, fo);
                    else fast_rect<KIND, false, XDROP, FL, PR_DIST>(L.table, fc, cDr, cRr, cDc, cCc, L.D_col, L.D_row, vc & 0xff, (vc >> 8) & 0xff, cb, FL, ck_corner, ck_offadd, -1, nullptr, fo);
                } else {
                    const uint32_t pq_len = coldp()->q_len[pair_in], pr_len = coldp()->r_len[pair_in];
                    ProfileView pvv{};
                    if constexpr (KIND == KIND_PROFILE) {
                        pvv.P = profile_positions(pr_len, h_max_size);
                        pvv.pos_aa = (const signed char*)r;
                        pvv.aa_pos = (const short*)(r + (uint64_t)pvv.P * 32);
                        pvv.goC = pvv.aa_pos + (uint64_t)pvv.P * 32; pvv.clC = pvv.goC + pvv.P; pvv.goR = pvv.clC + pvv.P;
                    }
                    constexpr int PD_R = KIND == KIND_PROFILE ? 1 : 0, PD_D = KIND == KIND_PROFILE ? 2 : 0;
                    const uint32_t spb = SPECIAL ? (((h_flags & F_LOCAL) ? SP_LOCAL : 0u) | (((h_flags & F_FQS) && cright) ? SP_FQS_ROW0 : 0u)) : 0u;
                    const int crz = clamp16(-ck_off + ZERO);
                    short* t1 = L.misc + 16; short* t2 = L.misc + 32;
                    lds_fill0(t1, 32);
                    unsigned long long none = 0;
                    Best cur;
                    if (cright) {
                        cur = place_rect<NCH_S, KIND, false, XDROP, PD_R>(L, fc, q, r, pq_len, pr_len, cri, crj, STEP, SLOT_B, L.D_col, L.C_col, t1, t2, ck_corner, crz, ck_offadd, nullptr, none, nullptr, spb, nullptr, &pvv);
                        (void)lds_shift_and_offset(SLOT_B, L.D_row, L.R_row, t1, t2, ck_offadd);
                    } else {
                        cur = place_rect<NCH_S, KIND, false, XDROP, PD_D>(L, fc, r, q, pr_len, pq_len, cri, crj, STEP, SLOT_B, L.D_row, L.R_row, t1, t2, ck_corner, crz, ck_offadd, nullptr, none, nullptr, spb, nullptr, &pvv);
                        (void)lds_shift_and_offset(SLOT_B, L.D_col, L.C_col, t1, t2, ck_offadd);
                    }
                    fo.row = cur.row; fo.col = cur.col;
                    lds_sync();
                    if constexpr (!WIDE) {
                        cDc = *(const int*)(L.D_col + 2 * lane); cCc = *(const int*)(L.C_col + 2 * lane);
                        cDr = *(const int*)(L.D_row + 2 * lane); cRr = *(const int*)(L.R_row + 2 * lane);
                    }
                }
                if (XDROP) {
                    if (cright) { best_i = ck_i + (uint32_t)fo.row; best_j = ck_j + (SLOT_B - STEP) + (uint32_t)fo.col; }
                    else { best_i = ck_i + (SLOT_B - STEP) + (uint32_t)fo.col; best_j = ck_j + (uint32_t)fo.row; }
                }
                lds_sync();
            }
            if constexpr (WIDE) save_ckpt_borders(SLOT_B);
            else { ck_reg[0] = cDc; ck_reg[1] = cCc; ck_reg[2] = cDr; ck_reg[3] = cRr; ck_in_regs = true; }
        }
        lds_sync();
        if (mine) {
            *(int4*)(L.D_col + l8) = int4{reg[0], reg[1], reg[2], reg[3]}; *(int4*)(L.C_col + l8) = int4{reg[4], reg[5], reg[6], reg[7]};
            *(int4*)(L.D_row + l8) = int4{reg[8], reg[9], reg[10], reg[11]}; *(int4*)(L.R_row + l8) = int4{reg[12], reg[13], reg[14], reg[15]};
        }
        lds_sync();
    }
};

template <int PMAX, int KIND, bool TRACE, bool XDROP, bool SPECIAL>
__global__ void __launch_bounds__(WAVES_PER_WG * 64, (PMAX >= 16 ? 2 : (PMAX <= 2 ? 6 : 4))) k_align(const BatchParams bp) {
    extern __shared__ __attribute__((aligned(16))) char smem[];
    const int lane = lane_id();
    const int wave = uni((int)threadIdx.x >> 6);
    {
        char* tab = smem;
        if (KIND == KIND_NUC) {
            nuc_table_fill(tab, bp.matrix, (int)threadIdx.x, WAVES_PER_WG * 64);
        } else {
            const int nbytes = KIND == KIND_AA ? 27 * 32 : (KIND == KIND_BYTES ? 2 : 0);
            for (int k = (int)threadIdx.x; k < nbytes; k += WAVES_PER_WG * 64) tab[k] = (char)bp.matrix[k];
        }
    }
    __syncthreads();
    constexpr uint32_t LCLS = kBig ? 128u : (uint32_t)PMAX * 128u;
    constexpr uint32_t ab = lds_array_bytes_h(LCLS);
    char* base = smem + lds_table_bytes_h(KIND) + (uint32_t)wave * lds_wave_bytes_h(LCLS);
    WaveLds L;
    L.D_col = (short*)(base + 0 * ab); L.C_col = (short*)(base + 1 * ab);
    L.D_row = (short*)(base + 2 * ab); L.R_row = (short*)(base + 3 * ab);
    L.misc = (short*)(base + 4 * ab);
    L.table = smem;
    const FillConsts fc = make_fill_consts(lane, bp.gap_open, bp.gap_extend);
    const uint32_t stride = bp.tb_stride;
    const bool batch_traceback = TRACE && stride > 0;
#ifdef BA_TIMING
    if (bp.prof && blockIdx.x == 0 && wave == 1 && is_lane(0)) atomicMax(bp.prof + 43, (unsigned long long)__builtin_amdgcn_s_memrealtime());
#endif
    if (batch_traceback && wave == 0 && blockIdx.x % stride == 0) {
        if (!(bp.flags & 0x800u))
        traceback_consumer<SPECIAL ? (int)TB_LANE_BYTES_LOC : (int)TB_LANE_BYTES>(bp, SPECIAL ? ~0u : (uint32_t)F_CIGAR_EQ,
                           (unsigned char*)smem + lds_table_bytes_h(KIND) + WAVES_PER_WG * lds_wave_bytes_h(LCLS), 64u, true);
#ifdef BA_TIMING
        if (bp.prof && is_lane(0)) atomicMax(bp.prof + 41, (unsigned long long)__builtin_amdgcn_s_memrealtime());
#endif
        return;
    }
    {
        const uint32_t cons_before = batch_traceback ? (blockIdx.x + stride - 1) / stride + (blockIdx.x % stride == 0 ? 1u : 0u) : 0u;
        const uint32_t fill_wave = blockIdx.x * WAVES_PER_WG + (uint32_t)wave - cons_before;
        uint32_t turn = 0;
        uint32_t w_next = 0, w_end = 0;
        bool closing = false;
        if (!TRACE && bp.cont_mode == 2 && bp.cq_side) __builtin_amdgcn_s_setprio(3);
        if (bp.cont_mode == 2 && bp.cq_side) {
            uint32_t spins = 0; bool up = false;
            for (;;) {
                uint32_t f = 0;
                if (is_lane(0)) f = __hip_atomic_load(bp.cq_ctrl + 20, BA_RLX_AGENT);
                if (uni((int)f)) { up = true; break; }
                if (++spins > (1u << 20)) break;
                __builtin_amdgcn_s_sleep(32);
            }
// ... 91 lines not shown
```

### block_aligner_amd/csrc/ba_host.cpp

```cpp
#include <hip/hip_runtime.h>

#include <algorithm>
#include <functional>
#include <cmath>
#include <cstdarg>
#include <cstdio>
#include <cstdlib>
#include <cstring>
#include <map>
#include <memory>
#include <string>
#include <type_traits>
#include <vector>
#include <atomic>
#include <chrono>
#include <thread>

#include "../../include/block_aligner_hip.h"
#include "aa_matrices.inc"
#include "ba_launch.h"

using ba::BatchParams;
using ba::BlockRec;

// ... 70 lines not shown
            m.scores[ib * 32 + ia] = tri[idx];
            idx++;
        }
    return m;
}
static constexpr NucMatrix nuc_simple(int8_t match, int8_t mismatch) {
    NucMatrix m{};
    for (int k = 0; k < 8 * 16; k++) m.scores[k] = -128;
    const char alpha[5] = {'A', 'T', 'C', 'G', 'N'};
    for (int i = 0; i < 5; i++)
        for (int j = 0; j < 5; j++) m.scores[(alpha[i] & 7) * 16 + (alpha[j] & 15)] = i == j ? match : mismatch;
    return m;
}
extern "C" {
extern const NucMatrix NW1 = nuc_simple(1, -1);
extern const AAMatrix BLOSUM45 = expand_tri(BA_TRI_BLOSUM45);
extern const AAMatrix BLOSUM50 = expand_tri(BA_TRI_BLOSUM50);
extern const AAMatrix BLOSUM62 = expand_tri(BA_TRI_BLOSUM62);
extern const AAMatrix BLOSUM80 = expand_tri(BA_TRI_BLOSUM80);
extern const AAMatrix BLOSUM90 = expand_tri(BA_TRI_BLOSUM90);
extern const AAMatrix PAM100 = expand_tri(BA_TRI_PAM100);
extern const AAMatrix PAM120 = expand_tri(BA_TRI_PAM120);
extern const AAMatrix PAM160 = expand_tri(BA_TRI_PAM160);
extern const AAMatrix PAM200 = expand_tri(BA_TRI_PAM200);
extern const AAMatrix PAM250 = expand_tri(BA_TRI_PAM250);
extern const ByteMatrix BYTES1 = {1, -1};
}

static inline uint8_t upper(uint8_t c) { return (c >= 'a' && c <= 'z') ? (uint8_t)(c - 32) : c; }
static inline int seq_kind(int kind) { return kind == BA_KIND_PROFILE_ ? BA_KIND_AA : kind; }
static inline uint8_t null_byte(int kind) { kind = seq_kind(kind); return kind == BA_KIND_AA ? 26 : (kind == BA_KIND_NUC ? 'Z' : 0); }
static inline bool convert_char(int kind, uint8_t c, uint8_t* out) {
    kind = seq_kind(kind);
    if (kind == BA_KIND_BYTES) { *out = c; return true; }
    c = upper(c);
    if (kind == BA_KIND_AA) { if (c < 'A' || c > 'A' + 26) return false; *out = (uint8_t)(c - 'A'); return true; }
    if (c < 'A' || c > 'Z') return false;
    *out = c;
    return true;
}

struct PaddedBytes {
    std::vector<uint8_t> s;
    size_t len;
    int kind;
};
struct Cigar {
    std::vector<OpLen> ops;
    size_t capacity;
};
struct AAProfile {
    std::vector<int8_t> pos_aa;
    std::vector<int16_t> gap_open_C, gap_close_C, gap_open_R;
    int8_t gap_extend;
    size_t max_len, curr_len, str_len;
};

struct DevBuf {
    void* p = nullptr;
    size_t bytes = 0;
    bool owned = true;
    void view(void* q, size_t n) { free_(); p = q; bytes = n; owned = false; }
    int alloc(size_t n) {
        free_();
        owned = true;
        if (n == 0) n = 4;
        hipError_t e = hipMalloc(&p, n);
        if (e != hipSuccess) { p = nullptr; return fail("hipMalloc(%zu bytes) failed: %s", n, hipGetErrorString(e)); }
        bytes = n;
        return 0;
    }
    void free_() { if (p && owned) (void)hipFree(p); p = nullptr; bytes = 0; }
    ~DevBuf() { free_(); }
    template <class T> T* as() const { return (T*)p; }
};

struct TextState {
    DevBuf len, off, pos, buf;
    uint64_t buf_cap = 0, run = 0;
    uint32_t what = ~0u;
    bool sized = false;
    hipEvent_t ev[2] = {};
    float ms = 0;
    ~TextState() { for (hipEvent_t e : ev) if (e) (void)hipEventDestroy(e); }
};

struct BaBatch {
    int device = 0;
    hipStream_t stream = nullptr, stream2 = nullptr;
    hipEvent_t ev0 = nullptr, ev1 = nullptr, ev_fork = nullptr, ev_join = nullptr, ev_l0 = nullptr, ev_m1 = nullptr;
    int kind = 0; uint32_t mode = 0;
    uint32_t n = 0, min_size = 0, max_size = 0, pclass = 0;
    int gap_open = 0, gap_extend = 0, x_drop = 0;
    uint32_t grid = 0, lds = 0, slots = 0;
    uint64_t trace_stride = 0, blocks_stride = 0, cig_total = 0, pool_bytes = 0;
    uint64_t trace_full = 0;
    bool adaptive = false;
    bool opt_class = false;
    bool bet_lost = false;
    uint64_t plan_fixed = 0, plan_maxlen2 = 0, plan_avg = 0;
    uint32_t retried = 0;
    uint64_t cap_n = 0, cap_pool = 0, cap_cig = 0, cap_maxlen2 = 0;
    DevBuf pool, q_off, q_len, r_off, r_len, matrix, score, qidx, ridx, cig_ops, cig_off, cig_len, cells, status, nblocks, pair_slot, trace_words, trace, blocks, ckpt, big, counter,
           tb_queue, tb_ctrl, slot_free, slot_info, prof, params_dev, donate;
    std::vector<uint32_t> h_order;
    uint32_t tb_stride = 0, n_fill_waves = 0, slots_per_wave = 1, tb_qsize = 1, tb_reserve = 0;
    std::vector<uint64_t> h_q_off, h_r_off;
    bool ran = false, in_flight = false;
    uint32_t work_chunk = 1;
    uint32_t mq_drain = 0;
    bool multi = false;
    uint32_t multi_b = 128;
    uint32_t geom = 0;
    uint32_t wpw = ba::WAVES_PER_WG;
    uint32_t walk_wave_n = 0;
    uint32_t sm_excl_n = 0;
    uint32_t sm_side_n = 0;
    bool small = false;
    bool quad = false;
    DevBuf contA, cont_n;
    DevBuf cq_queue, cq_ctrl;
    uint32_t quad_grid = 0, cq_grid = 0;
    bool pipe = false;
    DevBuf trace_off, blocks_off;
    uint64_t pipe_words = 0, pipe_recs = 0;
    DevBuf compact, compact_off, compact_total, dev_of;
    DevBuf stats, stats_pos;
    hipEvent_t ev_s0 = nullptr, ev_s1 = nullptr;
    float stats_ms = 0;
    DevBuf ex_rows, ex_work, ex_out, ex_counter;
    hipEvent_t ev_x0 = nullptr, ev_x1 = nullptr;
    float exact_ms = 0; uint64_t exact_cells = 0;
    DevBuf xt_trace, xt_rev, xt_rev_off, xt_nrun, xt_off, xt_runs;
    float xt_ms = 0; uint64_t xt_cells = 0;
    bool xt_valid = false; uint32_t xt_what = 0; int32_t xt_x_drop = 0; uint64_t xt_loads = 0;
    std::vector<uint32_t> xt_devpos; std::vector<BaExact> xt_out; std::vector<uint64_t> xt_h_off;
    int xt_form = 0;
    float xp_ms = 0; uint64_t xp_cells = 0;
    DevBuf xt_start; std::vector<uint32_t> xt_h_start;
    uint64_t loads = 0;
    TextState text;
    uint64_t runs_done = 0;
    uint64_t compact_cap = 0, compact_used_cap = 0; bool compacted = false; uint32_t* compact_host = nullptr;
    unsigned long long* h_total = nullptr;
    bool pad_negative = false;
    bool handle_mode = false;
    DevBuf hblk, rblk;
    BatchParams params() const {
        BatchParams bp{};
        bp.pool = pool.as<uint8_t>();
        bp.q_off = q_off.as<uint64_t>(); bp.q_len = q_len.as<uint32_t>();
        bp.r_off = r_off.as<uint64_t>(); bp.r_len = r_len.as<uint32_t>();
        bp.n = n; bp.gap_open = gap_open; bp.gap_extend = gap_extend;
        bp.min_size = min_size; bp.max_size = max_size; bp.x_drop = x_drop; bp.flags = mode | (dev_env("BA_NO_FAST") ? 0x100u : 0u) | ((dev_env("BA_SKIP_WALK") || dev_env("BA_NO_TRACEBACK")) ? 0x200u : 0u) | ((handle_mode || dev_env("BA_NO_SPEC")) ? 0x400u : 0u) | (dev_env("BA_NO_TB_WAVES") ? 0x800u : 0u) | (dev_env("BA_NO_REFILL") ? 0x1000u : 0u) | (dev_env("BA_NO_STEAL") ? 0x2000u : 0u) | ((pad_negative && !dev_env("BA_NO_END_CLIP")) ? (uint32_t)ba::F_PAD_NEG : 0u);
        bp.matrix = matrix.as<int8_t>();
        bp.score = score.as<int32_t>(); bp.query_idx = qidx.as<uint32_t>(); bp.reference_idx = ridx.as<uint32_t>();
        bp.cig_ops = ((mode & BA_TRACE) && !handle_mode && !dev_env("BA_NO_TRACEBACK")) ? cig_ops.as<uint32_t>() : nullptr;
        bp.cig_off = cig_off.as<uint64_t>(); bp.cig_start = nullptr; bp.cig_len = cig_len.as<uint32_t>();
        bp.cells = cells.as<unsigned long long>(); bp.status = status.as<uint32_t>(); bp.nblocks_out = nblocks.as<uint32_t>(); bp.slot_out = pair_slot.as<uint32_t>(); bp.trace_words_out = trace_words.as<uint32_t>();
        bp.walk_wave_n = walk_wave_n;
        bp.trace_arena = trace.as<uint32_t>(); bp.trace_stride = trace_stride;
        bp.blocks = blocks.as<BlockRec>(); bp.blocks_stride = blocks_stride;
        bp.trace_off = pipe ? trace_off.as<uint64_t>() : nullptr; bp.blocks_off = pipe ? blocks_off.as<uint64_t>() : nullptr;
        bp.ckpt = ckpt.as<short>(); bp.big = big.as<short>();
        bp.tb_stride = tb_stride; bp.slots_per_wave = slots_per_wave; bp.n_slots = slots; bp.tb_reserve = tb_reserve;
        bp.tb_qmask = tb_qsize - 1;
        bp.tb_queue = tb_queue.as<uint32_t>(); bp.tb_ctrl = tb_ctrl.as<uint32_t>();
        bp.slot_free = slot_free.as<uint32_t>(); bp.slot_info = slot_info.as<ba::SlotInfo>();
        bp.work_counter = counter.as<uint32_t>();
        bp.work_chunk = work_chunk;
        bp.mq_drain = mq_drain;
        bp.mq_waves = grid * wpw;
        bp.mq_donate = (multi && (mode & BA_TRACE) && !special_of(mode) && donate.p && !dev_env("BA_NO_DONATE")) ? donate.as<uint32_t>() : nullptr;
        bp.sm_excl_n = small ? sm_excl_n : 0; bp.sm_excl_first = 0;
        bp.prof = prof.as<unsigned long long>();
        return bp;
    }
    ~BaBatch() {
        if (ev0) (void)hipEventDestroy(ev0);
        if (ev1) (void)hipEventDestroy(ev1);
        if (ev_fork) (void)hipEventDestroy(ev_fork);
        if (ev_join) (void)hipEventDestroy(ev_join);
        if (h_total) (void)hipHostFree(h_total);
        if (ev_l0) (void)hipEventDestroy(ev_l0);
        if (ev_m1) (void)hipEventDestroy(ev_m1);
        if (ev_s0) (void)hipEventDestroy(ev_s0);
        if (ev_s1) (void)hipEventDestroy(ev_s1);
        if (ev_x0) (void)hipEventDestroy(ev_x0);
        if (ev_x1) (void)hipEventDestroy(ev_x1);
        if (stream2) (void)hipStreamDestroy(stream2);
        if (stream) (void)hipStreamDestroy(stream);
    }
};

static int check_align_params(bool profile, Gaps g, size_t min_size, size_t max_size, int32_t x_drop, uint32_t mode, std::string* why, bool linear_ok = false) {
    if (profile) { if (!(g.extend < 0)) { *why = "Gap extend cost must be negative!"; return 1; } }
    else {
        if (!(g.open < 0 && g.extend < 0)) { *why = "Gap costs must be negative!"; return 1; }
        if (!(g.open < g.extend) && !(linear_ok && g.open == g.extend)) { *why = "Gap open must cost more than gap extend!"; return 1; }
    }
    if (!(min_size < 65535 && max_size < 65535)) { *why = "Block sizes must be smaller than 2^16 - 1!"; return 1; }
    if ((min_size & (min_size - 1)) || (max_size & (max_size - 1))) { *why = "Block sizes must be powers of two!"; return 1; }
    if ((mode & BA_X_DROP) && x_drop < 0) { *why = "X-drop threshold amount must be nonnegative!"; return 1; }
    if ((mode & BA_LOCAL_START) && (mode & BA_FREE_QUERY_START_GAPS)) { *why = "Cannot set both LOCAL_START and FREE_QUERY_START_GAPS!"; return 1; }
    if ((mode & BA_X_DROP) && (mode & BA_FREE_QUERY_END_GAPS)) { *why = "Cannot set both X_DROP and FREE_QUERY_END_GAPS!"; return 1; }
    return 0;
}

constexpr size_t BA_MAX_BLOCK = 32768;
static int pclass_of(size_t max_size) {
    if (max_size <= 128) return 0;
    if (max_size == 256) return 1;
    if (max_size == 512) return 2;
    if (max_size == 1024) return 3;
    if (max_size == 2048) return 4;
    if (max_size == 4096 || max_size == 8192 || max_size == 16384 || max_size == 32768) return BA_PCLASS_BIG;
    return -1;
}
static inline uint32_t lds_class_cells(int pc) { return pc == BA_PCLASS_BIG ? 128u : 128u << pc; }

static void profile_image(const AAProfile* pr, uint32_t P, uint8_t* dst) {
    int8_t* pos_aa = (int8_t*)dst;
    int16_t* aa_pos = (int16_t*)(dst + (size_t)P * 32);
    int16_t* goC = aa_pos + (size_t)P * 32; int16_t* clC = goC + P; int16_t* goR = clC + P;
    const size_t have = std::min<size_t>(P, pr->curr_len);
    memset(pos_aa, 0x80, (size_t)P * 32);
    memcpy(pos_aa, pr->pos_aa.data(), have * 32);
    for (size_t c = 0; c < 32; c++)
        for (size_t i = 0; i < P; i++) aa_pos[c * P + i] = (int16_t)pos_aa[i * 32 + c];
    for (size_t i = 0; i < P; i++) {
        goC[i] = i < have ? pr->gap_open_C[i] : (int16_t)-128;
        clC[i] = i < have ? pr->gap_close_C[i] : (int16_t)-128;
        goR[i] = i < have ? pr->gap_open_R[i] : (int16_t)-128;
    }
}
struct NoProfiles { const AAProfile* operator()(size_t) const { return nullptr; } };

constexpr size_t POOL_SLACK = 256;
struct ExtImages {
    const uint8_t* host_base = nullptr; const uint8_t* dev_base = nullptr;
    const uint8_t* flags = nullptr;
    const uint32_t* seed_of = nullptr;
    float* pack_ms = nullptr;
};
struct Packed {
    std::vector<uint64_t> qo, ro, cig_off;
    std::vector<uint32_t> ql, rl;
    std::vector<uint8_t> image;
    uint64_t total = 0, maxlen2 = 0, cig_total = 0;
    bool on_device = false;
    const uint8_t* raw = nullptr; uint64_t raw_bytes = 0; uint32_t pad = 0;
    std::vector<uint64_t> raw_qo, raw_ro;
    const ExtImages* ext = nullptr; std::vector<uint8_t> ext_flags;
    std::vector<uint32_t> order;
    size_t who(size_t s) const { return order.empty() ? s : order[s]; }
};
template <class GetSeq, class GetProfile, class Lap>
static int pack_pairs_in_order(int kind, Gaps gaps, size_t min_size, size_t max_size, uint32_t mode, size_t n, bool already_converted,
                               GetSeq get, GetProfile getp, Packed& P, Lap lap, const ExtImages* ext = nullptr) {
    const bool profile = kind == BA_KIND_PROFILE_;
    const size_t pad = max_size + 16;
    std::vector<uint64_t>& qo = P.qo; std::vector<uint64_t>& ro = P.ro;
    qo.resize(n); ro.resize(n);
    std::vector<uint32_t>& ql = P.ql; std::vector<uint32_t>& rl = P.rl;
    ql.resize(n); rl.resize(n);
    uint64_t total = 0, maxlen2 = 0, cig_total = 0;
    std::vector<uint64_t>& cig_off = P.cig_off;
    cig_off.resize(n + 1);
    const uint8_t* lo = nullptr; const uint8_t* hi = nullptr; uint64_t sum_len = 0;
    auto span = [&](const uint8_t* ptr, size_t len) {
        if (!lo || ptr < lo) lo = ptr;
        if (!hi || ptr + len > hi) hi = ptr + len;
        sum_len += len;
    };
    for (size_t p = 0; p < n; p++) {
        const uint8_t* ptr; size_t len;
        get(p, 0, &ptr, &len);
        if (len > 0x3fffffffu) { fail("sequence too long"); return 1; }
        span(ptr, len);
        ql[p] = (uint32_t)len; qo[p] = total; total += (1 + len + pad + 3) & ~(size_t)3;
        if ((mode & BA_FREE_QUERY_END_GAPS) && !(min_size > len)) {
            fail("pair %zu: Min block size must be larger than the query length for FREE_QUERY_END_GAPS!", P.who(p)); return 1;
        }
        if (profile) {
            const AAProfile* pr = getp(p);
            if (!pr) { fail("pair %zu: null profile", P.who(p)); return 1; }
            if (pr->gap_extend != gaps.extend) { fail("pair %zu: profile gap_extend %d differs from the batch's %d", P.who(p), pr->gap_extend, gaps.extend); return 1; }
            len = pr->str_len;
            if (len > 0x3fffffffu) { fail("profile too long"); return 1; }
            rl[p] = (uint32_t)len; ro[p] = total; total += ba::profile_image_bytes((uint32_t)len, (uint32_t)max_size);
        } else {
            get(p, 1, &ptr, &len);
            if (len > 0x3fffffffu) { fail("sequence too long"); return 1; }
            span(ptr, len);
            rl[p] = (uint32_t)len; ro[p] = total; total += (1 + len + pad + 3) & ~(size_t)3;
        }
        maxlen2 = std::max<uint64_t>(maxlen2, (uint64_t)ql[p] + rl[p] + 2);
        cig_off[p] = cig_total;
        cig_total += (uint64_t)ql[p] + rl[p] + 1;
    }
    cig_off[n] = cig_total;
    total += POOL_SLACK;
    lap("offsets");
    P.total = total; P.maxlen2 = maxlen2; P.cig_total = cig_total; P.pad = (uint32_t)pad;
    if (ext) {
        P.on_device = true; P.ext = ext; P.raw = ext->host_base;
        P.raw_qo.resize(n); P.raw_ro.resize(n); P.ext_flags.resize(2 * n);
// ... 2733 lines not shown
```

### block_aligner_amd/csrc/ba_multi.hpp

```cpp
#pragma once
#include "ba_quad.hpp"

namespace ba {
#ifndef MQ_SOLO_PRIO
#define MQ_SOLO_PRIO 2
#endif

template <int N>
__device__ __forceinline__ int row_bcast(int v) { return __builtin_amdgcn_update_dpp(v, v, 0x150 + N, 0xf, 0xf, false); }
__device__ __forceinline__ int row_shl1_keep(int last, int src) { return __builtin_amdgcn_update_dpp(last, src, 0x101, 0xf, 0xf, false); }
__device__ __forceinline__ int splat_hi(int x) { const s16x2 t = as_s(x); return as_i(s16x2{t.y, t.y}); }
__device__ __forceinline__ int splat_lo(int x) { const s16x2 t = as_s(x); return as_i(s16x2{t.x, t.x}); }

__device__ __forceinline__ int sel_mask(unsigned long long m, int a, int b) {
    int r;
    asm("v_cndmask_b32_e64 %0, %1, %2, %3" : "=v"(r) : "v"(b), "v"(a), "s"(m));
    return r;
}

template <int SL> __device__ __forceinline__ int slot_first(int v) {
    if constexpr (SL == 16) return row_bcast<0>(v);
    else if constexpr (SL == 64) return __builtin_amdgcn_readfirstlane(v);
    else return __builtin_amdgcn_ds_bpermute((lane_id() & 32) << 2, v);
}
// ... 8 lines not shown
    else { const int t = wave_shr1_z(v); return l == 0 ? 0 : t; }
}
template <int SL> __device__ __forceinline__ int slot_shl1_keep(int last, int src, int l) {
    if constexpr (SL == 16) return row_shl1_keep(last, src);
    else { const int t = __builtin_amdgcn_update_dpp(last, src, 0x130, 0xf, 0xf, false); return l == SL - 1 ? last : t; }
}

__device__ __forceinline__ void cells_split(int (&v)[4]) {
    const int a = v[0], b = v[1], c = v[2], d = v[3];
    v[0] = __builtin_amdgcn_perm(c, a, 0x05040100); v[1] = __builtin_amdgcn_perm(c, a, 0x07060302);
    v[2] = __builtin_amdgcn_perm(d, b, 0x05040100); v[3] = __builtin_amdgcn_perm(d, b, 0x07060302);
}
__device__ __forceinline__ void cells_join(int (&v)[4]) {
    const int a = v[0], b = v[1], c = v[2], d = v[3];
    v[0] = __builtin_amdgcn_perm(b, a, 0x05040100); v[1] = __builtin_amdgcn_perm(d, c, 0x05040100);
    v[2] = __builtin_amdgcn_perm(b, a, 0x07060302); v[3] = __builtin_amdgcn_perm(d, c, 0x07060302);
}
__device__ __forceinline__ int4 cells_split(int4 q) { int v[4] = {q.x, q.y, q.z, q.w}; cells_split(v); return int4{v[0], v[1], v[2], v[3]}; }
__device__ __forceinline__ int4 cells_join(int4 q) { int v[4] = {q.x, q.y, q.z, q.w}; cells_join(v); return int4{v[0], v[1], v[2], v[3]}; }
__device__ __forceinline__ int adds_lo(int a, int k) {
    int t;
    asm("v_pk_add_i16 %0, %1, %2 op_sel_hi:[0,1] clamp" : "=v"(t) : "v"(a), "s"(k));
    return t;
}
__device__ __forceinline__ int max_hi_lo(int a, int b) {
    asm("v_max_i16_sdwa %0, %0, %1 dst_sel:WORD_1 dst_unused:UNUSED_PRESERVE src0_sel:WORD_1 src1_sel:WORD_0" : "+v"(a) : "v"(b));
    return a;
}

struct MultiConsts {
    int g2, g3;
    int K4, G48;
    int laneKG, lanem1KG;
    int w0;
};

__device__ __forceinline__ MultiConsts make_multi_consts(int l, int gx) {
    MultiConsts mc;
    mc.laneKG = l * 8 * gx; mc.lanem1KG = l ? (l - 1) * 8 * gx : -32768;
    mc.g2 = splat(max(-32768, 2 * gx)); mc.g3 = splat(max(-32768, 3 * gx));
    mc.K4 = pk(0, max(-32768, 4 * gx)); mc.G48 = pk(max(-32768, 4 * gx), max(-32768, 8 * gx));
    mc.w0 = pk(0, l == 0 ? 0 : ((l & 1) ? max(-32768, 8 * l * gx) : 4 * gx));
    return mc;
}
template <int SL = 16>
__device__ __forceinline__ int multi_carry(int r3, const MultiConsts& mc, int l = 0) {
    if constexpr (SL == 16) {
        const int pm = wave_prefix_max16((int)as_s(r3).y - mc.laneKG);
        return vmax(scan8_splat_lo(add_row_shr1(pm, mc.lanem1KG)), mc.w0);
    } else {
        const int pm = SL == 64 ? wave_prefix_max((int)as_s(r3).y - mc.laneKG) : wave_prefix_max32((int)as_s(r3).y - mc.laneKG);
        const int cin = add_shr1(pm, mc.lanem1KG);
        return vmax(scan8_splat_lo(l == 0 ? -32768 : cin), mc.w0);
    }
}

__device__ __forceinline__ int scan_halves(int (&r)[4], int ge2, const MultiConsts& mc) {
#pragma unroll
    for (int k = 1; k < 4; k++) r[k] = vmax(r[k], adds(r[k - 1], ge2));
    return vmax(r[3], adds_lo(r[3], mc.K4));
}
__device__ __forceinline__ void apply_halves(int (&r)[4], int r3, int cs, int ge2, const MultiConsts& mc) {
    const int t = max_hi_lo(adds_lo(cs, mc.K4), r[3]);
    r[0] = vmax(r[0], adds(t, ge2)); r[1] = vmax(r[1], adds(t, mc.g2)); r[2] = vmax(r[2], adds(t, mc.g3));
    r[3] = vmax(r3, adds(cs, mc.G48));
}

typedef int lds_v4i __attribute__((ext_vector_type(4)));
typedef int vec_v4i __attribute__((ext_vector_type(4)));
struct MultiOut { int mx, act_max8, pas_max8, corner_new; };

template <int KIND, bool TRACE, int SPM = 0, int SL = 16>
__device__ __forceinline__ void multi_rect(const char* table, const FillConsts& fc, const MultiConsts& mc, int l, int (&Ad)[4], int (&Ac)[4],
                                           int (&Pd)[4], int (&Pr)[4], uint2 vb, uint32_t cb_lo, uint32_t cb_hi, int corner, int off_add,
                                           uint32_t* __restrict__ tout, bool store, MultiOut& o, int rz2 = 0, bool fqs_row0 = false, int* zout = nullptr) {
    uint32_t zacc[2] = {0, 0};
    const int offa = splat(off_add);
    int d[4], c[4], pd[4], pr[4];
#pragma unroll
    for (int k = 0; k < 4; k++) {
        d[k] = adds(Ad[k], offa); c[k] = adds(Ac[k], offa); pd[k] = adds(Pd[k], offa); pr[k] = adds(Pr[k], offa);
    }
    o.corner_new = slot_first<SL>(pd[3]) >> 16;
    ScoreKey<KIND> key[4];
#pragma unroll
    for (int k = 0; k < 4; k++) key[k] = make_key<KIND>((int)((vb.x >> (8 * k)) & 0xffu), (int)((vb.y >> (8 * k)) & 0xffu));
    uint32_t kb[4] = {0, 0, 0, 0}, cbs_lo = 0, cbs_hi = 0;
    if constexpr (KIND == KIND_NUC) {
        const uint32_t tb = (uint32_t)(uintptr_t)table;
        const uint32_t k01 = nuc_keys2((uint32_t)__builtin_amdgcn_perm((int)vb.y, (int)vb.x, 0x05010400)), k23 = nuc_keys2((uint32_t)__builtin_amdgcn_perm((int)vb.y, (int)vb.x, 0x07030602));
        kb[0] = add_word(k01, tb, 0); kb[1] = add_word(k01, tb, 1); kb[2] = add_word(k23, tb, 0); kb[3] = add_word(k23, tb, 1);
        cbs_lo = nuc_col_offsets(cb_lo); cbs_hi = nuc_col_offsets(cb_hi);
    }
    int dmax[4] = {0, 0, 0, 0}, tacc[8] = {0, 0, 0, 0, 0, 0, 0, 0};
    int nvD[4] = {0, 0, 0, 0}, nvR[4] = {0, 0, 0, 0};
    int holdD[4] = {0, 0, 0, 0}, holdR[4] = {0, 0, 0, 0};
#pragma unroll
    for (int j = 0; j < STEP; j++) {
        const int cb = (int)(((j < 4 ? cb_lo : cb_hi) >> (8 * (j & 3))) & 0xffu);
        int sc[4];
#pragma unroll
        for (int k = 0; k < 4; k++) {
            if constexpr (KIND == KIND_NUC) sc[k] = lds_read_i32(add_byte(j < 4 ? cbs_lo : cbs_hi, kb[k], j));
            else sc[k] = fetch_score<KIND>(table, key[k], cb);
        }
        int prev = slot_shr1_z<SL>(d[3], l);
        if (j == 0) prev = l == 0 ? (int)((uint32_t)corner << 16) : prev;
        int d00[4];
        d00[0] = __builtin_amdgcn_alignbit(d[3], prev, 16);
#pragma unroll
        for (int k = 1; k < 4; k++) d00[k] = d[k - 1];
        int d11[4], copen[4], cn[4], x[4], r[4];
#pragma unroll
        for (int k = 0; k < 4; k++) {
            d11[k] = adds(d00[k], sc[k]);
            if (SPM == 2 && k == 0) d11[0] = fqs_row0 ? (int)(((uint32_t)d11[0] & 0xffff0000u) | ((uint32_t)rz2 & 0xffffu)) : d11[0];
            if (SPM == 1) d11[k] = vmax(d11[k], rz2);
            copen[k] = adds(d[k], fc.go2);
            cn[k] = vmax(adds(c[k], fc.ge2), copen[k]);
            d11[k] = vmax(d11[k], cn[k]);
            x[k] = adds(d11[k], fc.ome2);
            r[k] = x[k];
        }
        const int r3 = scan_halves(r, fc.ge2, mc);
        const int cs = multi_carry<SL>(r3, mc, l);
        apply_halves(r, r3, cs, fc.ge2, mc);
        int dn[4];
        uint32_t sC[4], sR[4], sCo[4], sRo[4];
#pragma unroll
        for (int k = 0; k < 4; k++) {
            dn[k] = vmax(d11[k], r[k]);
            if (TRACE) {
                sC[k] = (uint32_t)subs(cn[k], dn[k]); sR[k] = (uint32_t)subs(r[k], dn[k]); sCo[k] = (uint32_t)subs(copen[k], cn[k]); sRo[k] = (uint32_t)subs(x[k], r[k]);
            }
            dmax[k] = vmax(dmax[k], dn[k]);
            d[k] = dn[k]; c[k] = cn[k];
        }
        if (TRACE && SPM == 1) {
#pragma unroll
            for (int p2 = 0; p2 < 2; p2++) {
                const uint32_t pZ = (uint32_t)__builtin_amdgcn_perm(subs(rz2, dn[2 * p2 + 1]), subs(rz2, dn[2 * p2]), 0x0b090a08);
                zacc[p2] |= pZ & (0x01010101u << j);
            }
        }
        if (TRACE) {
#pragma unroll
            for (int p2 = 0; p2 < 2; p2++) {
                const uint32_t pC = (uint32_t)__builtin_amdgcn_perm((int)sC[2 * p2 + 1], (int)sC[2 * p2], 0x0b090a08), pR = (uint32_t)__builtin_amdgcn_perm((int)sR[2 * p2 + 1], (int)sR[2 * p2], 0x0b090a08);
                const uint32_t pCo = (uint32_t)__builtin_amdgcn_perm((int)sCo[2 * p2 + 1], (int)sCo[2 * p2], 0x0b090a08), pRo = (uint32_t)__builtin_amdgcn_perm((int)sRo[2 * p2 + 1], (int)sRo[2 * p2], 0x0b090a08);
                const uint32_t lo2 = bfi(0x55555555u, pC, pR), hi2 = bfi(0x55555555u, pCo, pRo);
                const uint32_t nib = bfi(0x33333333u, lo2, hi2);
                if (j & 1) tacc[2 * (j >> 1) + p2] = (int)bfi(0xF0F0F0F0u, nib, (uint32_t)tacc[2 * (j >> 1) + p2]);
                else tacc[2 * (j >> 1) + p2] = (int)nib;
            }
            if (j & 1) {
                const int wa = tacc[j - 1], wb = tacc[j];
                tacc[j - 1] = __builtin_amdgcn_perm(wb, wa, 0x05040100); tacc[j] = __builtin_amdgcn_perm(wb, wa, 0x07060302);
            }
        }
        if (j >= 4) { nvD[j - 4] = __builtin_amdgcn_perm(dn[3], holdD[j - 4], 0x07060302); nvR[j - 4] = __builtin_amdgcn_perm(r[3], holdR[j - 4], 0x07060302); }
        else { holdD[j] = dn[3]; holdR[j] = r[3]; }
    }
    if (TRACE) {
#ifndef MQ_X_NOTRSTORE
        if (store) { *(int4*)tout = int4{tacc[0], tacc[1], tacc[2], tacc[3]}; *(int4*)(tout + 4) = int4{tacc[4], tacc[5], tacc[6], tacc[7]}; }
#else
        asm volatile("" :: "v"(tacc[0]), "v"(tacc[1]), "v"(tacc[2]), "v"(tacc[3]), "v"(tacc[4]), "v"(tacc[5]), "v"(tacc[6]), "v"(tacc[7]));
#endif
    }
#pragma unroll
    for (int k = 0; k < 4; k++) {
        Pd[k] = slot_shl1_keep<SL>(nvD[k], pd[k], l); Pr[k] = slot_shl1_keep<SL>(nvR[k], pr[k], l);
        Ad[k] = d[k]; Ac[k] = c[k];
    }
    {
        const int ma = vmax(vmax(d[0], d[1]), vmax(d[2], d[3])), mb = vmax(vmax(Pd[0], Pd[1]), vmax(Pd[2], Pd[3]));
        const s16x2 sa = as_s(ma), sb = as_s(mb);
        const int xa = vmax(ma, as_i(s16x2{sa.y, sa.x})), xb = vmax(mb, as_i(s16x2{sb.y, sb.x}));
        const s16x2 rr = as_s(slot_first<SL>(__builtin_amdgcn_perm(xb, xa, 0x05040100)));
        o.act_max8 = rr.x; o.pas_max8 = rr.y;
    }
    const int mm = vmax(vmax(dmax[0], dmax[1]), vmax(dmax[2], dmax[3]));
    const int m32 = max(mm & 0xffff, (int)((uint32_t)mm >> 16));
    o.mx = slot_last<SL>(SL == 16 ? wave_prefix_max16(m32) : (SL == 64 ? wave_prefix_max(m32) : wave_prefix_max32(m32)));
    if constexpr (TRACE && SPM == 1) { zout[0] = ~__builtin_amdgcn_perm((int)zacc[1], (int)zacc[0], 0x05040100); zout[1] = ~__builtin_amdgcn_perm((int)zacc[1], (int)zacc[0], 0x07060302); }
}

enum { MR_PAIR = 0, MR_BEST_I, MR_BEST_J, MR_CELLS_LO, MR_CELLS_HI, MR_BUDGET, MR_STATUS, MR_TSLOT, MR_SI, MR_SJ, MR_DIR, MR_PREV_DIR, MR_OFF, MR_OFF_MAX,
       MR_BEST_MAX, MR_Y_DROP, MR_X_ITER, MR_D_CORNER, MR_NSTEPS, MR_TRACE_TOP, MR_NBLOCKS, MR_SEL, MR_WORDS };
__device__ __forceinline__ int mq_load(const char* p) { return __hip_atomic_load((const int*)p, BA_RLX_AGENT); }

#ifndef MQ_PARTIAL_MB
#define MQ_PARTIAL_MB 256
#endif
#ifndef MQ_WAVES_EU
#define MQ_WAVES_EU 4
#endif
template <int PMAX, int KIND, bool TRACE, bool XDROP, int SPM = 0, int MBP = 128, int WPW = WAVES_PER_WG, int EU = MQ_WAVES_EU>
__global__ void __launch_bounds__(WPW * 64, (PMAX >= 16 ? 2 : EU)) k_multi(const BatchParams bp) {
    constexpr uint32_t MB = (uint32_t)MBP;
    constexpr int SL = MBP / 8, NSLOT = 64 / SL;
    constexpr uint32_t ALLM = (1u << NSLOT) - 1u;
    constexpr uint32_t ARR = 2u * MB, BUFL = 4u * ARR, BUFA = BUFL + 64u, SLOTA = 2u * BUFA + 128u;
    static_assert((MBP == 128 || MBP == 256 || MBP == 512) && NSLOT * SLOTA <= MQ_WAVE_BYTES && NSLOT * 2u * BUFL <= MQ_LDS_SCALARS && (MBP == 128 || SPM == 0), "k_multi slot geometry");
    static_assert(MBP != 128 || (BUFA == MQ_BUF_BYTES && SLOTA == MQ_SLOT_BYTES), "ba_params.h");
    constexpr uint32_t MQ_TW = (STEP * MB / 8) * (SPM == 1 ? 2u : 1u);
    constexpr int TB_LB = SPM ? (int)TB_LANE_BYTES_LOC : (int)TB_LANE_BYTES_L2;
    constexpr uint32_t TB_MASK = SPM ? ~0u : (uint32_t)F_CIGAR_EQ;
    extern __shared__ __attribute__((aligned(16))) char smem[];
    const int lane = lane_id(), l = lane & (SL - 1), g = lane / SL;
    const int wave = uni((int)threadIdx.x >> 6);
    {
        char* tab = smem;
        if (KIND == KIND_NUC) {
            nuc_table_fill(tab, bp.matrix, (int)threadIdx.x, WPW * 64);
        } else {
            const int nbytes = KIND == KIND_AA ? 27 * 32 : 2;
            for (int k = (int)threadIdx.x; k < nbytes; k += WPW * 64) tab[k] = (char)bp.matrix[k];
        }
    }
    __syncthreads();
    constexpr uint32_t LCLS = (uint32_t)PMAX * 128u;
    constexpr uint32_t ab = lds_array_bytes_h(LCLS);
    char* base = smem + lds_table_bytes_h(KIND) + (uint32_t)wave * mq_wave_bytes_h(LCLS);
    WaveLds L;
    L.D_col = (short*)(base + 0 * ab); L.C_col = (short*)(base + 1 * ab);
    L.D_row = (short*)(base + 2 * ab); L.R_row = (short*)(base + 3 * ab);
    L.misc = (short*)(base + 4 * ab);
    L.table = smem;
    const int gx = bp.gap_extend;
    const uint32_t stride = bp.tb_stride;
    const bool batch_traceback = TRACE && stride > 0;
#if defined(BA_TIMING) || defined(BA_ENDHIST)
    if (bp.prof && blockIdx.x == 0 && wave == 1 && is_lane(0)) atomicMax(bp.prof + 43, (unsigned long long)__builtin_amdgcn_s_memrealtime());
#endif
#ifdef BA_TIMING
    unsigned long long t_solo = 0, t_quad = 0, t_wait = 0, n_solo = 0, n_quad = 0;
#endif
    if (batch_traceback && wave == 0 && blockIdx.x % stride == 0) {
        if (!(bp.flags & 0x800u))
        traceback_consumer<TB_LB, 8, 3>(bp, TB_MASK, (unsigned char*)base, 64u, true, 1);
#if defined(BA_TIMING) || defined(BA_ENDHIST)
        if (bp.prof && is_lane(0)) atomicMax(bp.prof + 42, (unsigned long long)__builtin_amdgcn_s_memrealtime());
#endif
        return;
    }
    const uint32_t cons_before = batch_traceback ? (blockIdx.x + stride - 1) / stride + (blockIdx.x % stride == 0 ? 1u : 0u) : 0u;
    const uint32_t fill_wave = blockIdx.x * WPW + (uint32_t)wave - cons_before;
    const uint32_t max_size = bp.max_size;
    const bool keep_pre = XDROP || MB < max_size;
    char* const wave_mem = (char*)bp.big + (uint64_t)fill_wave * MQ_WAVE_BYTES;

    auto coldp_big = [&]() { const __attribute__((address_space(4))) BatchParams* p = (const __attribute__((address_space(4))) BatchParams*)__builtin_amdgcn_kernarg_segment_ptr(); asm volatile("" : "+s"(p)); return p->big; };
    auto fill_wave_of = [&]() { uint32_t b = blockIdx.x, w = (uint32_t)wave; asm volatile("" : "+s"(b), "+s"(w)); const uint32_t st = ((const __attribute__((address_space(4))) BatchParams*)__builtin_amdgcn_kernarg_segment_ptr())->tb_stride;
                                const uint32_t cb = (TRACE && st > 0) ? (b + st - 1) / st + (b % st == 0 ? 1u : 0u) : 0u; return b * WPW + w - cb; };
    uint32_t live_m = 0, pend_m = 0;
    uint32_t w_next = 0, w_end = 0;
    bool more = true, drain = false, fin_counted = false;
#define don_final (bp.mq_donate + gridDim.x * WPW)
#define don_offers (don_final + 32)
    auto slot_mem_of = [&](uint32_t id, uint32_t s_i) {
        const uint32_t db = id / WPW;
        const uint32_t dcb = batch_traceback ? (db + stride - 1) / stride + (db % stride == 0 ? 1u : 0u) : 0u;
        return (char*)bp.big + (uint64_t)(id - dcb) * MQ_WAVE_BYTES + s_i * SLOTA;
    };
    auto claim_offer = [&](uint32_t my_id, uint32_t& id_out, int& s_out) {
        uint32_t avail = 0;
        if (is_lane(0)) avail = __hip_atomic_load(don_offers, BA_RLX_AGENT);
        if ((int)uni((int)avail) <= 0) return false;
        const uint32_t n_ids = gridDim.x * WPW;
        for (uint32_t k0 = 0; k0 < n_ids; k0 += 64) {
            const uint32_t idx = ((my_id & ~63u) + k0 + (uint32_t)lane) % n_ids;
            const uint32_t v = __hip_atomic_load(bp.mq_donate + idx, BA_RLX_AGENT) & ALLM;
            unsigned long long m = __ballot(v != 0u);
            while (m) {
                const int src = __builtin_ctzll(m);
                const uint32_t vv = (uint32_t)__builtin_amdgcn_readlane((int)v, src), id = (uint32_t)__builtin_amdgcn_readlane((int)idx, src);
                const int s_i = __builtin_ctz(vv);
                uint32_t old = 0;
                if (is_lane(0)) {
                    old = __hip_atomic_fetch_and(bp.mq_donate + id, ~(1u << s_i), BA_RLX_AGENT);
                    if ((old >> s_i) & 1u) __hip_atomic_fetch_sub(don_offers, 1u, BA_RLX_AGENT);
                }
                old = (uint32_t)uni((int)old);
                if ((old >> s_i) & 1u) { id_out = id; s_out = s_i; return true; }
                m &= m - 1;
            }
        }
        return false;
    };
    auto try_refill = [&](uint32_t my_id) {
        uint32_t id = 0; int s_o = 0;
        if ((bp.flags & 0x1000u) || !claim_offer(my_id, id, s_o)) return false;
        __builtin_amdgcn_fence(__ATOMIC_ACQUIRE, "agent");
        const int e = __builtin_ctz(~live_m & ALLM);
        const char* src = slot_mem_of(id, (uint32_t)s_o);
        char* dst = wave_mem + (uint32_t)e * SLOTA;
#pragma unroll
        for (int k = 0; k < (int)(SLOTA / 256u); k++) *(int*)(dst + 256 * k + 4 * lane) = mq_load(src + 256 * k + 4 * lane);
        asm volatile("s_waitcnt vmcnt(0)" ::: "memory");
        live_m |= 1u << e;
        return true;
    };
    auto my_id_of = [&]() { uint32_t b = blockIdx.x, w = (uint32_t)wave; asm volatile("" : "+s"(b), "+s"(w)); return b * WPW + w; };

    for (;;) {
        for (;;) {
            int solo = -1; bool fresh = false, to_end = false;
            uint32_t new_pair = 0, donor_id = ~0u;
            if (pend_m) solo = __builtin_ctz(pend_m);
            else if (more && (drain ? live_m == 0u : live_m != ALLM)) {
                if (w_next == w_end) {
                    uint32_t v = 0;
                    if (is_lane(0)) v = atomicAdd(bp.work_counter, bp.work_chunk);
                    w_next = (uint32_t)uni((int)v);
                    if (w_next >= bp.n) { more = false; w_next = w_end = 0; continue; }
                    w_end = min(w_next + bp.work_chunk, bp.n);
                }
                new_pair = w_next++; solo = __builtin_ctz(~live_m & ALLM); fresh = true;
                to_end = drain;
                if (new_pair + bp.mq_drain >= bp.n) drain = true;
            } else if (live_m && live_m != ALLM && MB < (uint32_t)(MQ_PARTIAL_MB)) {
                solo = __builtin_ctz(live_m); to_end = true;
                if (TRACE && bp.mq_donate) {
                    const uint32_t my_id = my_id_of();
                    uint32_t don = 0;
                    if (is_lane(0)) don = __hip_atomic_load(bp.mq_donate + my_id, BA_RLX_AGENT);
                    don = (uint32_t)uni((int)don) >> 8;
                    if (!(don & 1u)) {
                        if (try_refill(my_id)) continue;
                        const uint32_t others = live_m & ~(1u << solo);
                        if (others) {
                            __builtin_amdgcn_fence(__ATOMIC_RELEASE, "agent");
                            asm volatile("s_waitcnt vmcnt(0)" ::: "memory");
                        }
                        if (is_lane(0)) {
                            __hip_atomic_store(bp.mq_donate + my_id, others | 0x100u | (others ? 0x200u : 0u), BA_RLX_AGENT);
                            if (others) __hip_atomic_fetch_add(don_offers, (uint32_t)__builtin_popcount(others), BA_RLX_AGENT);
                        }
                        asm volatile("s_waitcnt vmcnt(0)" ::: "memory");
                        if (is_lane(0)) __hip_atomic_fetch_add(don_final, 1u, BA_RLX_AGENT);
                    } else if (don & 2u) {
                        uint32_t old = 0;
                        if (is_lane(0)) {
                            old = __hip_atomic_fetch_and(bp.mq_donate + my_id, ~(1u << solo), BA_RLX_AGENT);
                            if ((old >> solo) & 1u) __hip_atomic_fetch_sub(don_offers, 1u, BA_RLX_AGENT);
                        }
                        old = (uint32_t)uni((int)old);
                        if (!((old >> solo) & 1u)) { live_m &= ~(1u << solo); continue; }
                    }
                }
            } else if (TRACE && bp.mq_donate && !live_m && !more) {
                const uint32_t my_id = my_id_of();
                if (is_lane(0) && !(__hip_atomic_fetch_or(bp.mq_donate + my_id, 0x100u, BA_RLX_AGENT) & 0x100u)) __hip_atomic_fetch_add(don_final, 1u, BA_RLX_AGENT);
                const uint32_t n_fill = gridDim.x * WPW - (batch_traceback ? (gridDim.x + stride - 1) / stride : 0u);
                bool got = false;
                uint32_t nap = 1;
                for (;;) {
                    uint32_t nf = 0;
                    if (is_lane(0)) nf = __hip_atomic_load(don_final, BA_RLX_AGENT);
                    nf = (uint32_t)uni((int)nf);
                    got = !(bp.flags & 0x2000u) && claim_offer(my_id, donor_id, solo);
                    if (got || nf >= n_fill) break;
                    for (uint32_t z = 0; z < nap; z++) __builtin_amdgcn_s_sleep(127);
                    nap = nap < 16u ? nap * 2u : 16u;
                }
                if (!got) { donor_id = ~0u; break; }
                __builtin_amdgcn_fence(__ATOMIC_ACQUIRE, "agent");
                to_end = true;
            }
            else {
                if constexpr (TRACE && MB >= (uint32_t)(MQ_PARTIAL_MB)) {
                    if (bp.mq_donate && live_m && live_m != ALLM && !more && !fin_counted) {
                        fin_counted = true;
                        const uint32_t my_id = my_id_of();
                        if (is_lane(0) && !(__hip_atomic_fetch_or(bp.mq_donate + my_id, 0x100u, BA_RLX_AGENT) & 0x100u)) __hip_atomic_fetch_add(don_final, 1u, BA_RLX_AGENT);
                    }
                }
                break;
            }

            BA_TSTAMP(ts_a);
            const FillConsts fc = make_fill_consts(lane, bp.gap_open, gx);
            Aligner<PMAX, KIND, TRACE, XDROP, SPM != 0, true, MBP> al(bp, L, fc);
            PairState st{};
            uint32_t s_pair, s_slot;
            char* smem_s = wave_mem + (uint32_t)solo * SLOTA;
            if (donor_id != ~0u) smem_s = slot_mem_of(donor_id, (uint32_t)solo);
            char* const rec = smem_s + 2 * BUFA;
            al.ckpt = bp.ckpt + (uint64_t)(fill_wave + bp.ckpt_wave0) * 8 * bp.max_size;
            if (fresh) {
                s_pair = new_pair;
                s_slot = fill_wave * bp.slots_per_wave;
                if (batch_traceback) {
                    BA_TSTAMP(tw_a);
                    uint32_t seen = 0, idle_n = 0;
                    for (;;) {
                        uint32_t f = 0, head = 0;
                        if ((uint32_t)lane < bp.slots_per_wave) f = __hip_atomic_load(bp.slot_free + s_slot + lane, BA_RLX_AGENT);
                        if (is_lane(0)) head = __hip_atomic_load(bp.tb_ctrl + 32, BA_RLX_AGENT);
                        const unsigned long long fm = __ballot(f != 0);
                        if (fm) {
                            s_slot += (uint32_t)__builtin_ctzll(fm);
                            if (is_lane(0)) __hip_atomic_store(bp.slot_free + s_slot, 0u, BA_RLX_AGENT);
                            break;
                        }
                        head = (uint32_t)uni((int)head);
                        if (head != seen) { seen = head; idle_n = 0; }
                        else if ((++idle_n & 2047u) == 0 && traceback_help_one<TB_LB>(bp, TB_MASK, (unsigned char*)base)) idle_n = 0;
                        __builtin_amdgcn_s_sleep(64);
                    }
#ifdef BA_TIMING
                    t_wait += __builtin_amdgcn_s_memtime() - tw_a;
#endif
                } else if (TRACE) {
                    s_slot += (uint32_t)solo;
                }
            } else {
                const int rv = lane < MR_WORDS ? mq_load(rec + 4 * lane) : 0;
#define BA_W(v, k) __builtin_amdgcn_readlane(v, k)
                const uint32_t s_sel = (uint32_t)BA_W(rv, MR_SEL);
                const char* live_b = smem_s + (s_sel ^ 1u) * BUFA; const char* ck_b = smem_s + s_sel * BUFA;
                const int cv = lane < 16 ? mq_load(ck_b + BUFL + 4 * lane) : 0;
                s_pair = (uint32_t)BA_W(rv, MR_PAIR); s_slot = (uint32_t)BA_W(rv, MR_TSLOT);
                st.si = (uint32_t)BA_W(rv, MR_SI); st.sj = (uint32_t)BA_W(rv, MR_SJ); st.dir = BA_W(rv, MR_DIR); st.prev_dir = BA_W(rv, MR_PREV_DIR);
                st.off = BA_W(rv, MR_OFF); st.off_max = BA_W(rv, MR_OFF_MAX); st.best_max = BA_W(rv, MR_BEST_MAX);
                st.y_drop_iter = (uint32_t)BA_W(rv, MR_Y_DROP); st.x_drop_iter = BA_W(rv, MR_X_ITER); st.D_corner = BA_W(rv, MR_D_CORNER);
                st.trace_top = (uint32_t)BA_W(rv, MR_TRACE_TOP); st.nblocks = (uint32_t)BA_W(rv, MR_NBLOCKS);
                const uint32_t ns = (uint32_t)BA_W(rv, MR_NSTEPS);
                st.best_i = (uint32_t)BA_W(rv, MR_BEST_I); st.best_j = (uint32_t)BA_W(rv, MR_BEST_J);
                st.cells = ((unsigned long long)(uint32_t)BA_W(rv, MR_CELLS_LO) | ((unsigned long long)(uint32_t)BA_W(rv, MR_CELLS_HI) << 32)) + (unsigned long long)ns * (STEP * MB);
                const uint32_t bud = (uint32_t)BA_W(rv, MR_BUDGET);
                st.step_budget = bud > ns ? bud - ns : 1u;
                st.status = (uint32_t)BA_W(rv, MR_STATUS);
                const int flag = BA_W(cv, 0);
                const bool ck_pre = flag != 0;
                st.ck_i = (uint32_t)BA_W(cv, 1); st.ck_j = (uint32_t)BA_W(cv, 2); st.ck_off = BA_W(cv, 3);
                st.ck_tt = (uint32_t)BA_W(cv, 4) + (flag ? MQ_TW : 0u); st.ck_nb = (uint32_t)BA_W(cv, 5) + (flag ? 1u : 0u);
                const int ck_dir = BA_W(cv, 6), ck_offadd = BA_W(cv, 7), ck_corner = BA_W(cv, 8);
#undef BA_W
                {
                    int reg[16], ckr[16];
                    const bool lr = st.dir == DIR_RIGHT, cr = ck_dir == DIR_RIGHT;
                    const uint32_t oAd = (lr ? 0u : 2 * ARR) + l * 16, oAc = (lr ? ARR : 3 * ARR) + l * 16, oPd = (lr ? 2 * ARR : 0u) + l * 16, oPr = (lr ? 3 * ARR : ARR) + l * 16;
                    const uint32_t cAd = (cr ? 0u : 2 * ARR) + l * 16, cAc = (cr ? ARR : 3 * ARR) + l * 16, cPd = (cr ? 2 * ARR : 0u) + l * 16, cPr = (cr ? 3 * ARR : ARR) + l * 16;
#pragma unroll
                    for (int k = 0; k < 4; k++) {
                        reg[k] = mq_load(live_b + oAd + 4 * k); reg[4 + k] = mq_load(live_b + oAc + 4 * k); reg[8 + k] = mq_load(live_b + oPd + 4 * k); reg[12 + k] = mq_load(live_b + oPr + 4 * k);
                        ckr[k] = mq_load(ck_b + cAd + 4 * k); ckr[4 + k] = mq_load(ck_b + cAc + 4 * k); ckr[8 + k] = mq_load(ck_b + cPd + 4 * k); ckr[12 + k] = mq_load(ck_b + cPr + 4 * k);
                    }
                    al.import_slot(reg, ckr, s_pair, ck_pre || MB < max_size, ck_pre, ck_dir, ck_offadd, ck_corner, st.ck_i, st.ck_j, st.best_i, st.best_j, st.ck_off);
                }
            }
            al.trace = bp.trace_arena + (uint64_t)s_slot * bp.trace_stride;
            al.blocks = bp.blocks + (uint64_t)s_slot * bp.blocks_stride;
            int keepv = 0;
            park<0>(keepv, (int)live_m); park<1>(keepv, (int)pend_m); park<2>(keepv, (int)w_next); park<3>(keepv, (int)w_end);
            park<4>(keepv, (more ? 1 : 0) | (fresh ? 2 : 0) | (to_end ? 4 : 0) | (drain ? 8 : 0)); park<5>(keepv, solo); park<6>(keepv, (int)s_pair); park<7>(keepv, (int)s_slot);
            BA_TSTAMP(tr_a);
            __builtin_amdgcn_s_setprio(MQ_SOLO_PRIO);
            st = al.run(s_pair, s_slot, batch_traceback, nullptr, fresh ? MM_FRESH : MM_RESUME, st, !to_end, !fresh && !to_end);
            __builtin_amdgcn_s_setprio(0);
            live_m = (uint32_t)unpark<0>(keepv); pend_m = (uint32_t)unpark<1>(keepv); w_next = (uint32_t)unpark<2>(keepv); w_end = (uint32_t)unpark<3>(keepv);
            { const int fl = unpark<4>(keepv); more = fl & 1; fresh = fl & 2; to_end = fl & 4; drain = fl & 8; }
            solo = unpark<5>(keepv); s_pair = (uint32_t)unpark<6>(keepv); s_slot = (uint32_t)unpark<7>(keepv);
            char* const smem_s2 = (char*)coldp_big() + (uint64_t)fill_wave_of() * MQ_WAVE_BYTES + (uint32_t)solo * SLOTA;
            char* const rec2 = smem_s2 + 2 * BUFA;
#ifdef BA_TIMING
            {
                const unsigned long long tr_b = __builtin_amdgcn_s_memtime();
                al.prof[45] += tr_b - tr_a; al.prof[46] += fresh ? 1 : 0;
                if (bp.prof && is_lane(0)) {
                    for (int k = 0; k < 48; k++) if (k != 17 && !(k >= 20 && k < 32) && !(k >= 40 && k < 44)) atomicAdd(bp.prof + k, al.prof[k]);
                    atomicAdd(bp.prof + (fresh ? 56 : (to_end ? 58 : 57)), tr_b - tr_a);
                }
            }
#endif
            pend_m &= ~(1u << solo);
            if (st.exited) {
                const bool rgt = st.dir == DIR_RIGHT;
                if (lane < SL) {
                    const int l8 = 8 * l;
                    const int4 a_d = *(const int4*)((rgt ? L.D_col : L.D_row) + l8), a_c = *(const int4*)((rgt ? L.C_col : L.R_row) + l8);
                    const int4 p_d = *(const int4*)((rgt ? L.D_row : L.D_col) + l8), p_r = *(const int4*)((rgt ? L.R_row : L.C_col) + l8);
                    char* b1 = smem_s2 + BUFA;
                    *(int4*)(b1 + l * 16) = a_d; *(int4*)(b1 + ARR + l * 16) = a_c; *(int4*)(b1 + 2 * ARR + l * 16) = p_d; *(int4*)(b1 + 3 * ARR + l * 16) = p_r;
                    if (MB < max_size) {
                        char* b0 = smem_s2;
                        *(int4*)(b0 + l * 16) = *(const int4*)(L.D_col + MB + l8); *(int4*)(b0 + ARR + l * 16) = *(const int4*)(L.C_col + MB + l8);
                        *(int4*)(b0 + 2 * ARR + l * 16) = *(const int4*)(L.D_row + MB + l8); *(int4*)(b0 + 3 * ARR + l * 16) = *(const int4*)(L.R_row + MB + l8);
                    }
                }
                if (is_lane(0)) {
                    char* b0 = smem_s2;
                    *(int4*)(b0 + BUFL) = int4{0, (int)st.ck_i, (int)st.ck_j, st.ck_off}; *(int4*)(b0 + BUFL + 16) = int4{(int)st.ck_tt, (int)st.ck_nb, DIR_RIGHT, 0};
                    *(int*)(b0 + BUFL + 32) = 0;
                    int* rc = (int*)rec2;
                    rc[MR_PAIR] = (int)s_pair; rc[MR_BEST_I] = (int)st.best_i; rc[MR_BEST_J] = (int)st.best_j; rc[MR_CELLS_LO] = (int)(uint32_t)st.cells; rc[MR_CELLS_HI] = (int)(uint32_t)(st.cells >> 32);
                    rc[MR_BUDGET] = (int)st.step_budget; rc[MR_STATUS] = (int)st.status; rc[MR_TSLOT] = (int)s_slot; rc[MR_SI] = (int)st.si; rc[MR_SJ] = (int)st.sj; rc[MR_DIR] = st.dir;
                    rc[MR_PREV_DIR] = st.prev_dir; rc[MR_OFF] = st.off; rc[MR_OFF_MAX] = st.off_max; rc[MR_BEST_MAX] = st.best_max; rc[MR_Y_DROP] = (int)st.y_drop_iter;
                    rc[MR_X_ITER] = st.x_drop_iter; rc[MR_D_CORNER] = st.D_corner; rc[MR_NSTEPS] = 0; rc[MR_TRACE_TOP] = (int)st.trace_top; rc[MR_NBLOCKS] = (int)st.nblocks; rc[MR_SEL] = 0;
                }
                lds_sync();
                live_m |= 1u << solo;
            } else live_m &= ~(1u << solo);
#ifdef BA_TIMING
            t_solo += __builtin_amdgcn_s_memtime() - ts_a; n_solo++;
#endif
        }
        if (!live_m) break;

        {
            BA_TSTAMP(tq_a);
            char* const slot_mem = wave_mem + (uint32_t)g * SLOTA;
            const int x_drop = bp.x_drop;
            FillConsts fq;
            fq.go2 = splat(bp.gap_open); fq.ge2 = splat(gx); fq.ome2 = splat(clamp16(bp.gap_open - gx));
            MultiConsts mc = make_multi_consts(l, gx);
            const uint64_t tcap64 = bp.trace_stride, bcap64 = bp.blocks_stride;
            const uint32_t tcap = (uint32_t)(tcap64 < 0x7fffffffull ? tcap64 : 0x7fffffffull), bcap = (uint32_t)(bcap64 < 0x7fffffffull ? bcap64 : 0x7fffffffull);
            const bool live = (live_m >> g) & 1u;
            const char* rec = slot_mem + 2 * BUFA;
#define BA_R(k) (live ? mq_load(rec + 4 * (k)) : 0)
            const uint32_t pair = (uint32_t)BA_R(MR_PAIR), tslot = (uint32_t)BA_R(MR_TSLOT);
            uint32_t si = (uint32_t)BA_R(MR_SI), sj = (uint32_t)BA_R(MR_SJ), y_drop = (uint32_t)BA_R(MR_Y_DROP);
            uint32_t nblocks = (uint32_t)BA_R(MR_NBLOCKS), sel = (uint32_t)BA_R(MR_SEL);
            const uint32_t tt_in = (uint32_t)BA_R(MR_TRACE_TOP), tt0 = tt_in - nblocks * MQ_TW;
            int dir = BA_R(MR_DIR), prev_dir = BA_R(MR_PREV_DIR), off = BA_R(MR_OFF), off_max = BA_R(MR_OFF_MAX), best_max = BA_R(MR_BEST_MAX);
            int x_iter = BA_R(MR_X_ITER), D_corner = BA_R(MR_D_CORNER);
#undef BA_R
            int A_d[4], A_c[4], P_d[4], P_r[4];
            {
                const char* b = slot_mem + (sel ^ 1u) * BUFA + l * 16;
#pragma unroll
                for (int k = 0; k < 4; k++) {
                    A_d[k] = live ? mq_load(b + 4 * k) : 0; A_c[k] = live ? mq_load(b + ARR + 4 * k) : 0;
                    P_d[k] = live ? mq_load(b + 2 * ARR + 4 * k) : 0; P_r[k] = live ? mq_load(b + 3 * ARR + 4 * k) : 0;
                }
                cells_split(A_d); cells_split(A_c); cells_split(P_d); cells_split(P_r);
            }
            char* const lbuf = base + (uint32_t)g * (2u * BUFL);
            constexpr uint32_t MQ_LSC_STATE = 9u, MQ_LSC_PAIR = 20u;
            static_assert(2u * MQ_LSC_STATE <= MQ_LSC_PAIR && MQ_LSC_PAIR + 12u <= MQ_LSC_INTS && (4u * MQ_LSC_PAIR) % 16u == 0 && (4u * MQ_LSC_INTS) % 16u == 0, "a slot's scalars in LDS");
            int* const lsc = (int*)(base + MQ_LDS_SCALARS) + (uint32_t)g * MQ_LSC_INTS;
            lds_sync();
            const unsigned long long qa_r = TRACE ? 0ull : (unsigned long long)(bp.pool + (live ? bp.q_off[pair] : 0ull)), ra_r = TRACE ? 0ull : (unsigned long long)(bp.pool + (live ? bp.r_off[pair] : 0ull));
            const uint32_t qlen_r = (!TRACE && live) ? bp.q_len[pair] : 0u, rlen_r = (!TRACE && live) ? bp.r_len[pair] : 0u;
            if (TRACE && l == 0) {
                const unsigned long long qa = (unsigned long long)(bp.pool + (live ? bp.q_off[pair] : 0ull)), ra = (unsigned long long)(bp.pool + (live ? bp.r_off[pair] : 0ull));
                *(int4*)(lsc + MQ_LSC_PAIR) = int4{(int)(uint32_t)qa, (int)(uint32_t)(qa >> 32), (int)(uint32_t)ra, (int)(uint32_t)(ra >> 32)};
                const long long room = (long long)tcap - (long long)(MQ_TW + 64u) - (long long)tt_in;
                const unsigned long long nb_room = room < 0 ? 0ull : (unsigned long long)nblocks + (unsigned long long)room / MQ_TW + 1ull;
                const uint32_t nb_lim = (uint32_t)(nb_room < (unsigned long long)bcap ? nb_room : (unsigned long long)bcap);
                *(int4*)(lsc + MQ_LSC_PAIR + 4) = int4{live ? (int)bp.q_len[pair] : 0, live ? (int)bp.r_len[pair] : 0, (int)nb_lim, 0};
                const unsigned long long ta = (unsigned long long)(bp.trace_arena + (uint64_t)tslot * bp.trace_stride), ba = (unsigned long long)(bp.blocks + (uint64_t)tslot * bp.blocks_stride);
                *(int4*)(lsc + MQ_LSC_PAIR + 8) = int4{(int)(uint32_t)ta, (int)(uint32_t)(ta >> 32), (int)(uint32_t)ba, (int)(uint32_t)(ba >> 32)};
            }
            if (live) {
                const char* cb = slot_mem + sel * BUFA;
                char* d = lbuf + sel * BUFL + l * 16;
#pragma unroll
                for (int a = 0; a < 4; a++) {
                    const char* sp = cb + a * ARR + l * 16;
                    *(int4*)(d + a * ARR) = cells_split(int4{mq_load(sp), mq_load(sp + 4), mq_load(sp + 8), mq_load(sp + 12)});
                }
                if ((uint32_t)l < MQ_LSC_STATE) lsc[sel * MQ_LSC_STATE + l] = mq_load(cb + BUFL + 4 * l);
            }
            lds_sync();
            uint2 pf_qv = {0, 0}, pf_rv = {0, 0}, pf_qc = {0, 0}, pf_rc = {0, 0}; bool pf_ok = false;
            bool leave = false;
            auto stage = [&](uint32_t lb, uint32_t ls, uint32_t which, uint32_t s_i, uint32_t s_j, int s_off, uint32_t s_tt, uint32_t s_nb, int s_dir, int s_offadd, int s_corner) {
                typedef __attribute__((address_space(3))) lds_v4i* lds_int4_ptr;
                typedef __attribute__((address_space(3))) int* lds_int_ptr;
                const lds_int4_ptr b = (lds_int4_ptr)(uintptr_t)(lb + which * BUFL);
                b[0] = lds_v4i{A_d[0], A_d[1], A_d[2], A_d[3]}; b[ARR / 16] = lds_v4i{A_c[0], A_c[1], A_c[2], A_c[3]};
                b[2 * ARR / 16] = lds_v4i{P_d[0], P_d[1], P_d[2], P_d[3]}; b[3 * ARR / 16] = lds_v4i{P_r[0], P_r[1], P_r[2], P_r[3]};
                if (l == 0) {
                    const lds_int_ptr sc = (lds_int_ptr)(uintptr_t)ls + which * MQ_LSC_STATE;
                    sc[0] = 1; sc[1] = (int)s_i; sc[2] = (int)s_j; sc[3] = s_off; sc[4] = (int)s_tt; sc[5] = (int)s_nb; sc[6] = s_dir; sc[7] = s_offadd; sc[8] = s_corner;
                }
            };
            const uint32_t base32 = (uint32_t)(uintptr_t)base;
            do {
                const bool right = dir == DIR_RIGHT;
                uint32_t lid;
                asm volatile("v_mbcnt_lo_u32_b32 %0, -1, 0\n\tv_mbcnt_hi_u32_b32 %0, -1, %0" : "=v"(lid));
                const uint32_t l8 = (lid & (uint32_t)(SL - 1)) * 8u;
                const uint32_t lbuf_s = base32 + (lid / (uint32_t)SL) * (2u * BUFL) + 2u * l8;
                const uint32_t lsc_s = base32 + (uint32_t)MQ_LDS_SCALARS + (lid / (uint32_t)SL) * (4u * (uint32_t)MQ_LSC_INTS);
                int4 cA = {0, 0, 0, 0}, cB = {0, 0, 0, 0}, cC = {0, 0, 0, 0};
                if (TRACE) {
                    typedef const __attribute__((address_space(3))) lds_v4i* lds_cint4_ptr;
                    const lds_v4i a4 = *(lds_cint4_ptr)(uintptr_t)(lsc_s + 4u * MQ_LSC_PAIR), b4 = *(lds_cint4_ptr)(uintptr_t)(lsc_s + 4u * (MQ_LSC_PAIR + 4u)),
                                  c4 = *(lds_cint4_ptr)(uintptr_t)(lsc_s + 4u * (MQ_LSC_PAIR + 8u));
                    cA = int4{a4.x, a4.y, a4.z, a4.w}; cB = int4{b4.x, b4.y, b4.z, b4.w}; cC = int4{c4.x, c4.y, c4.z, c4.w};
                }
                const uint8_t* const qp = TRACE ? (const uint8_t*)((unsigned long long)(uint32_t)cA.x | ((unsigned long long)(uint32_t)cA.y << 32)) : (const uint8_t*)qa_r;
                const uint8_t* const rp = TRACE ? (const uint8_t*)((unsigned long long)(uint32_t)cA.z | ((unsigned long long)(uint32_t)cA.w << 32)) : (const uint8_t*)ra_r;
                const uint32_t qlen = TRACE ? (uint32_t)cB.x : qlen_r, rlen = TRACE ? (uint32_t)cB.y : rlen_r;
                const uint32_t ri = right ? si : sj, rj = (right ? sj : si) + (MB - STEP);
                const uint32_t lenV = right ? qlen : rlen, lenC = right ? rlen : qlen;
                const bool q_out = si + MB > qlen, r_out = sj + MB > rlen;
                bool elig = XDROP || ri + MB <= lenV || rj + STEP <= lenC;
                const uint32_t trace_top = tt0 + nblocks * MQ_TW;
                if (TRACE) elig = elig && nblocks < (uint32_t)cB.z;
                leave = live && !elig;
                const bool run = live && !leave;
                const int off_n = off_max;
                const int off_add = sat16(off - off_n);
                const int corner = (prev_dir != dir && prev_dir != DIR_GROW) ? sat16(D_corner + off_add) : 0;
#ifndef MQ_X_NOSTAGE
                if (live) stage(lbuf_s, lsc_s, sel ^ 1u, si, sj, off_n, trace_top, nblocks, dir, off_add, corner);
#endif
                asm volatile("" : "+v"(mc.laneKG), "+v"(mc.lanem1KG), "+v"(mc.w0));
                uint2 vb, cbv;
                {
                    const uint8_t* Vp = right ? qp : rp; const uint8_t* Cp = right ? rp : qp;
                    vb = right ? pf_qv : pf_rv; cbv = right ? pf_rc : pf_qc;
                    if (__any(run && !pf_ok)) {
                        if (run && !pf_ok) {
                            const uint32_t* vp = (const uint32_t*)(Vp + (ri + l8));
                            vb.x = vp[0]; vb.y = vp[1];
                            const uint32_t* cp = (const uint32_t*)(Cp + rj);
                            cbv.x = cp[0]; cbv.y = cp[1];
                        }
                    }
                    asm volatile("" : "+v"(vb.x), "+v"(vb.y));
                    if (run) {
                        const uint32_t* a = (const uint32_t*)(qp + (si + l8)); const uint32_t* b = (const uint32_t*)(rp + (sj + l8));
                        const uint32_t* cq = (const uint32_t*)(qp + si + MB); const uint32_t* cr = (const uint32_t*)(rp + sj + MB);
                        pf_qv.x = a[0]; pf_qv.y = a[1]; pf_rv.x = b[0]; pf_rv.y = b[1];
                        pf_qc.x = cq[0]; pf_qc.y = cq[1]; pf_rc.x = cr[0]; pf_rc.y = cr[1];
                        pf_ok = true;
                    }
                }
                uint32_t* tw = nullptr;
                if (TRACE) {
                    typedef __attribute__((address_space(1))) uint32_t* glb_u32_ptr;
                    tw = (uint32_t*)(glb_u32_ptr)((unsigned long long)(uint32_t)cC.x | ((unsigned long long)(uint32_t)cC.y << 32)) + (trace_top + l8);
                    if (run && l == 0) {
                        static_assert(sizeof(BlockRec) == 16, "a record as four words");
                        const uint32_t hw = right ? ((uint32_t)MB | ((uint32_t)STEP << 16)) : ((uint32_t)STEP | ((uint32_t)MB << 16));
                        typedef __attribute__((address_space(1))) vec_v4i* glb_rec_ptr;
                        ((glb_rec_ptr)((unsigned long long)(uint32_t)cC.z | ((unsigned long long)(uint32_t)cC.w << 32)))[nblocks] =
                            vec_v4i{(int)((right ? ri : rj) | 0x80000000u) , (int)(right ? rj : ri), (int)hw, (int)(trace_top | (right ? 0x80000000u : 0u))};
                    }
                }
                MultiOut o;
                int zw[2] = {0, 0};
                multi_rect<KIND, TRACE, SPM, SL>(smem, fq, mc, l, A_d, A_c, P_d, P_r, vb, cbv.x, cbv.y, corner, off_add, tw, run, o, SPM ? splat(sat16(ZERO - off_n)) : 0,
                                             SPM == 2 && right && ri == 0u && l == 0, zw);
                if (TRACE && SPM == 1 && run) *(int2*)(tw - 8 * l + 128 + 2 * l) = int2{zw[0], zw[1]};

                const int right_max = right ? o.act_max8 : o.pas_max8, down_max = right ? o.pas_max8 : o.act_max8;
                const int new_off_max = off_n + o.mx - ZERO;
                const bool improve = new_off_max > best_max;
                const uint32_t new_y = improve ? 0u : y_drop + 1;
                bool stop = q_out && r_out;
                if (XDROP) stop = stop || (!improve && new_off_max < best_max - x_drop && x_iter >= 1);
                stop = stop || (!q_out && !r_out && 2 * MB <= max_size && new_y > MB / STEP - 1);
                const bool commit = run && !stop;
                leave = leave || (run && stop);
                {
                    const bool imp = commit && improve;
                    if (keep_pre) sel ^= imp ? 1u : 0u;
                    best_max = imp ? new_off_max : best_max;
                    off = commit ? off_n : off; off_max = commit ? new_off_max : off_max; y_drop = commit ? new_y : y_drop;
                    prev_dir = commit ? dir : prev_dir; D_corner = commit ? o.corner_new : D_corner;
                    if (TRACE) nblocks += commit ? 1u : 0u;
                    if (XDROP) x_iter = commit ? ((new_off_max < best_max - x_drop) ? x_iter + 1 : 0) : x_iter;
                    const bool go_down = r_out || (!q_out && down_max > right_max);
                    si += (commit && go_down) ? (uint32_t)STEP : 0u; sj += (commit && !go_down) ? (uint32_t)STEP : 0u;
                    const int ndir = go_down ? DIR_DOWN : DIR_RIGHT;
                    const unsigned long long swap_m = __ballot(ndir != dir);
#pragma unroll
                    for (int k = 0; k < 4; k++) {
                        const int td = A_d[k], tc = A_c[k];
                        A_d[k] = sel_mask(swap_m, P_d[k], td); A_c[k] = sel_mask(swap_m, P_r[k], tc); P_d[k] = sel_mask(swap_m, td, P_d[k]); P_r[k] = sel_mask(swap_m, tc, P_r[k]);
                    }
                    dir = commit ? ndir : dir;
                }
#ifdef BA_TIMING
                n_quad++;
#endif
            } while (!__any(leave));
            const uint32_t trace_top = tt0 + nblocks * MQ_TW;
            if (live && !leave) stage((uint32_t)(uintptr_t)(lbuf + l * 16), (uint32_t)(uintptr_t)lsc, sel ^ 1u, si, sj, 0, trace_top, nblocks, dir, 0, 0);
            lds_sync();
            if (live) {
#pragma unroll
                for (int w = 0; w < 2; w++) {
                    const char* sp = lbuf + w * BUFL + l * 16;
                    char* d = slot_mem + w * BUFA + l * 16;
#pragma unroll
                    for (int a = 0; a < 4; a++) *(int4*)(d + a * ARR) = cells_join(*(const int4*)(sp + a * ARR));
                    if ((uint32_t)l < MQ_LSC_STATE) *(int*)(slot_mem + w * BUFA + BUFL + 4 * l) = lsc[w * MQ_LSC_STATE + l];
                }
            }
            lds_sync();
            if (live && l == 0) {
                int* rc = (int*)(slot_mem + 2 * BUFA);
                const uint32_t nsteps = (uint32_t)mq_load((const char*)(rc + MR_NSTEPS)) + ((si + sj) - (uint32_t)mq_load((const char*)(rc + MR_SI)) - (uint32_t)mq_load((const char*)(rc + MR_SJ))) / (uint32_t)STEP;
                rc[MR_SI] = (int)si; rc[MR_SJ] = (int)sj; rc[MR_DIR] = dir; rc[MR_PREV_DIR] = prev_dir; rc[MR_OFF] = off; rc[MR_OFF_MAX] = off_max; rc[MR_BEST_MAX] = best_max;
                rc[MR_Y_DROP] = (int)y_drop; rc[MR_X_ITER] = x_iter; rc[MR_D_CORNER] = D_corner; rc[MR_NSTEPS] = (int)nsteps; rc[MR_TRACE_TOP] = (int)trace_top;
                rc[MR_NBLOCKS] = (int)nblocks; rc[MR_SEL] = (int)sel;
            }
            const unsigned long long lm = __ballot(leave && l == 0);
            pend_m = 0;
#pragma unroll
            for (int sl_i = 0; sl_i < NSLOT; sl_i++) pend_m |= (uint32_t)((lm >> (sl_i * SL)) & 1ull) << sl_i;
#ifdef BA_TIMING
            t_quad += __builtin_amdgcn_s_memtime() - tq_a;
#endif
        }
    }
#ifdef BA_TIMING
    if (bp.prof && is_lane(0)) {
        atomicMax(bp.prof + 40, (unsigned long long)__builtin_amdgcn_s_memrealtime());
        atomicAdd(bp.prof + 50, t_solo); atomicAdd(bp.prof + 51, t_quad); atomicAdd(bp.prof + 52, t_wait); atomicAdd(bp.prof + 53, n_solo); atomicAdd(bp.prof + 54, n_quad); atomicAdd(bp.prof + 55, 1ull);
    }
#endif
#ifdef BA_ENDHIST
    if (bp.prof && is_lane(0)) {
        const unsigned long long t0 = __hip_atomic_load(bp.prof + 43, BA_RLX_AGENT), t = __builtin_amdgcn_s_memrealtime();
        const unsigned long long k = t0 && t > t0 ? (t - t0) / 400000ull : 0ull;
        atomicAdd(bp.prof + 64 + (k < 63ull ? k : 63ull), 1ull);
        atomicMax(bp.prof + 40, t);
    }
#endif
    if (batch_traceback) {
        lds_sync();
#ifndef MQ_HELPER_LANES
#define MQ_HELPER_LANES 0u
#endif
        if constexpr (SPM != 0) traceback_consumer<TB_LB>(bp, TB_MASK, (unsigned char*)base, 4u, false);
        else {
#if MQ_HELPER_LANES == 0
        traceback_helper_wave<true>(bp, (uint32_t*)base, 2048u);
#else
        traceback_consumer<(int)TB_LANE_BYTES_L2>(bp, (uint32_t)F_CIGAR_EQ, (unsigned char*)base, MQ_HELPER_LANES, false);
#endif
        }
#if defined(BA_TIMING) || defined(BA_ENDHIST)
        if (bp.prof && is_lane(0)) atomicMax(bp.prof + 41, (unsigned long long)__builtin_amdgcn_s_memrealtime());
#endif
    }
}

#undef don_final
#undef don_offers
}
```

### block_aligner_amd/csrc/ba_params.h

```cpp
#pragma once
#include <stdint.h>

namespace ba {

constexpr int ZERO = 1 << 14;
constexpr int STEP = 8;
constexpr int KIND_AA = 0, KIND_NUC = 1, KIND_BYTES = 2, KIND_PROFILE = 3;
constexpr int DIR_RIGHT = 0, DIR_DOWN = 1, DIR_GROW = 2;

enum : uint32_t {
    F_TRACE = 1u << 0, F_XDROP = 1u << 1, F_LOCAL = 1u << 2, F_FQS = 1u << 3, F_FQE = 1u << 4, F_CIGAR_EQ = 1u << 5,
    F_PAD_NEG = 1u << 14
};
enum : uint32_t { ST_OK = 0, ST_TRACE_OVERFLOW = 1, ST_BLOCKS_OVERFLOW = 2, ST_CIGAR_OVERFLOW = 4, ST_TRACEBACK_LOST = 8, ST_WATCHDOG = 16, ST_SLOT_TIMEOUT = 32, ST_MODE = 64,
                  ST_CLASS_OVERFLOW = 128  };

struct BlockRec {
    uint32_t i, j;
    uint16_t h, w;
    uint32_t trace_base;
};

struct SlotInfo { uint32_t pair, nblocks, end_i, end_j; };

#if defined(__HIPCC__)
#define BA_HD __host__ __device__
#else
#define BA_HD
#endif
BA_HD inline uint32_t profile_positions(uint32_t len, uint32_t max_size) { return (len + max_size + 17u) & ~1u; }
BA_HD inline uint64_t profile_image_bytes(uint32_t len, uint32_t max_size) { return (uint64_t)profile_positions(len, max_size) * (32 + 64 + 6); }

struct PairCont {
    uint32_t pair, si, sj; int32_t dir, prev_dir, off, off_max, best_max;
    uint32_t y_drop_iter; int32_t x_drop_iter, D_corner; uint32_t best_i, best_j, ck_i, ck_j; int32_t ck_off;
    unsigned long long cells; uint32_t step_budget;
    uint32_t trace_top, nblocks, ck_trace_top, ck_nblocks, status;
    uint32_t borders[4][16];
    uint32_t ckpt[4][16];
};
static_assert(sizeof(PairCont) == 96 + 512, "PairCont layout");

struct BatchParams {
    const uint8_t* pool;
    const uint64_t* q_off; const uint32_t* q_len;
    const uint64_t* r_off; const uint32_t* r_len;
    uint32_t n;
    int32_t gap_open, gap_extend;
    uint32_t min_size, max_size;
    int32_t x_drop;
    uint32_t flags;
    const int8_t* matrix;
    int32_t* score; uint32_t* query_idx; uint32_t* reference_idx;
    uint32_t* cig_ops; const uint64_t* cig_off; uint32_t* cig_start; uint32_t* cig_len;
    unsigned long long* cells;
    uint32_t* status;
    uint32_t* nblocks_out;
    uint32_t* slot_out;
    uint32_t* trace_words_out;
    uint32_t* trace_arena; uint64_t trace_stride;
    BlockRec* blocks; uint64_t blocks_stride;
    const uint64_t* trace_off; const uint64_t* blocks_off;
    short* ckpt;
    short* big;
    uint32_t* work_counter;
    unsigned long long* prof;
    uint32_t tb_stride;
    uint32_t slots_per_wave;
    uint32_t n_slots;
    uint32_t tb_reserve;
    uint32_t tb_qmask;
    uint32_t* tb_queue;
    uint32_t* tb_ctrl;
    uint32_t* slot_free;
    SlotInfo* slot_info;
    uint32_t cont_mode;
    const PairCont* cont_in; const uint32_t* cont_in_flag;
    PairCont* cont_out; uint32_t* cont_out_flag;
    uint32_t* cq_queue;
    uint32_t* cq_ctrl;
    uint32_t cq_producers;
    uint32_t cq_side;
    uint32_t inline_len2;
    uint32_t ckpt_wave0;
    uint32_t mq_drain;
    uint32_t* mq_donate;
    uint32_t mq_waves;
    uint32_t walk_wave_n;
    uint32_t work_chunk;
    uint32_t sm_excl_first;
    uint32_t sm_excl_n;
    uint32_t tb_i, tb_j, tb_nblocks, tb_slot;
};


constexpr uint32_t BIG_TILE = 2048;
BA_HD constexpr uint64_t big_array_shorts(uint32_t max_size) { return (uint64_t)max_size + 64; }
BA_HD constexpr uint64_t big_wave_shorts(uint32_t max_size) { return 8 * big_array_shorts(max_size); }

constexpr uint32_t MQ_B_HOST = 128;
constexpr uint32_t MQ_BUF_BYTES = 4 * 256 + 64, MQ_SLOT_BYTES = 2 * MQ_BUF_BYTES + 128, MQ_WAVE_BYTES = 4 * MQ_SLOT_BYTES;
constexpr uint32_t MQ_LDS_SCALARS = 8192, MQ_LSC_INTS = 32, MQ_LDS_BYTES = 8192 + 4 * MQ_LSC_INTS * 4;
constexpr uint32_t SM_B_HOST = 32, SM_SLOTS = 16;
constexpr uint32_t SM_BUF_BYTES = 4 * 64 + 32, SM_SLOT_BYTES = 2 * SM_BUF_BYTES + 128, SM_WAVE_BYTES = SM_SLOTS * SM_SLOT_BYTES;
constexpr uint32_t SM_LDS_SCALARS = 8192, SM_LDS_BYTES = 8192 + SM_SLOTS * 2 * 32;
#ifndef BA_WAVES_PER_WG
#define BA_WAVES_PER_WG 8
#endif
constexpr int WAVES_PER_WG = BA_WAVES_PER_WG;
constexpr int MQ_GEOM_WPW = 4;

BA_HD constexpr uint32_t lds_array_bytes_h(uint32_t max_size) { return max_size * 2 + 32; }
BA_HD constexpr uint32_t lds_wave_bytes_h(uint32_t max_size) { return 4 * lds_array_bytes_h(max_size) + 128; }
BA_HD constexpr uint32_t lds_table_bytes_h(int kind) { return kind == KIND_NUC ? 8192 : 896; }
BA_HD constexpr uint32_t lds_wg_bytes_h(int kind, uint32_t max_size) { return lds_table_bytes_h(kind) + WAVES_PER_WG * lds_wave_bytes_h(max_size); }
BA_HD constexpr uint32_t mq_wave_bytes_h(uint32_t max_size) { return lds_wave_bytes_h(max_size) > MQ_LDS_BYTES ? lds_wave_bytes_h(max_size) : MQ_LDS_BYTES; }
BA_HD constexpr uint32_t mq_wg_bytes_h(int kind, uint32_t max_size, uint32_t wpw = WAVES_PER_WG) { return lds_table_bytes_h(kind) + wpw * mq_wave_bytes_h(max_size); }
constexpr uint32_t SM_PROF_STAGE = 16 * 256;
BA_HD constexpr uint32_t sm_wave_bytes_h(uint32_t max_size, int kind = 0) {
    return (lds_wave_bytes_h(max_size) > SM_LDS_BYTES ? lds_wave_bytes_h(max_size) : SM_LDS_BYTES) + (kind == KIND_PROFILE ? SM_PROF_STAGE : 0u);
}
BA_HD constexpr uint32_t sm_wg_bytes_h(int kind, uint32_t max_size) { return lds_table_bytes_h(kind) + WAVES_PER_WG * sm_wave_bytes_h(max_size, kind); }
constexpr uint32_t TB_LANE_BYTES = 76, TB_LUT_BYTES = 128, TB_LDS_BYTES = 5120;
constexpr uint32_t TB_LANE_BYTES_L2 = 100;
constexpr uint32_t TB_LANE_BYTES_LOC = 116, TB_LDS_BYTES_LOC = 7680;
static_assert(TB_LUT_BYTES + 64 * TB_LANE_BYTES_LOC <= TB_LDS_BYTES_LOC, "k_walk LDS (LOCAL_START)");
constexpr uint32_t TB_LDS_BYTES_L2 = 6784;
static_assert(TB_LUT_BYTES + 64 * TB_LANE_BYTES_L2 <= TB_LDS_BYTES_L2, "k_walk LDS (slot rectangles)");
static_assert(MQ_LDS_BYTES % 16 == 0 && TB_LUT_BYTES + 64 * TB_LANE_BYTES_L2 <= MQ_LDS_BYTES, "k_multi LDS");
constexpr uint32_t TB_DIAG_LUT_L2 = 256, TB_DIAG_LUT_STD = 64;
static_assert(TB_LUT_BYTES + 64 * TB_LANE_BYTES + TB_DIAG_LUT_STD <= TB_LDS_BYTES && TB_LUT_BYTES + TB_LANE_BYTES + 8 + TB_DIAG_LUT_STD <= lds_wave_bytes_h(128), "traceback LDS regions");
static_assert((TB_LUT_BYTES + 64 * TB_LANE_BYTES) % 8 == 0 && (TB_LUT_BYTES + 64 * TB_LANE_BYTES_L2) % 8 == 0, "tb_diag's tables are read 8 bytes at a time");
static_assert(TB_LUT_BYTES + 64 * TB_LANE_BYTES_L2 + TB_DIAG_LUT_L2 <= TB_LDS_BYTES_L2 && TB_LUT_BYTES + 64 * TB_LANE_BYTES_L2 + TB_DIAG_LUT_L2 <= MQ_LDS_BYTES, "tb_diag's tables (slot rectangles)");
static_assert(TB_LUT_BYTES + 64 * TB_LANE_BYTES_LOC <= MQ_LDS_BYTES && TB_LUT_BYTES + 64 * TB_LANE_BYTES_LOC <= SM_LDS_BYTES, "special-mode walk records in a wave's region");

}
```

Baseline: 2644.

## Store slot trace nibbles unpermuted and address sequences via 32-bit pool offsets

Drops the per-pair perm shuffle on trace accumulator words in the multi-slot DP kernel. Every traceback path (scalar, wave walk, lane step, diagonal LUT) reads the resulting byte order through a templated remapping. Separately, the multi-queue kernel keeps 32-bit query/reference offsets into the pool and loads through a global-address-space base pointer from the kernarg segment, saving 64-bit pointer arithmetic. Prefetch is skipped when a new host flag marks the pool as too large for 32-bit offsets. The cost is more template variants and the risk of a layout mismatch between writer and readers.

```diff
diff --git a/block_aligner_amd/csrc/ba_driver.hpp b/block_aligner_amd/csrc/ba_driver.hpp
--- a/block_aligner_amd/csrc/ba_driver.hpp
+++ b/block_aligner_amd/csrc/ba_driver.hpp
@@ -80,6 +80,10 @@
     return (next == TB_PENDING && v == 0) ? (right_blk ? 2u : 1u) : next;
 }
 
+template <bool RO>
+__host__ __device__ constexpr uint32_t slot_cell_byte(uint32_t c) { return RO ? (((c & 2u) << 1) | ((c & 4u) >> 1) | (c & 1u)) : c; }
+
+template <bool RO = false>
 __device__ __forceinline__ uint32_t traceback(const BlockRec* __restrict__ blocks, uint32_t nblocks, const uint32_t* __restrict__ trace,
                                      uint32_t i, uint32_t j, const uint8_t* __restrict__ q, const uint8_t* __restrict__ r, uint32_t flags,
                                      uint32_t* __restrict__ out, uint64_t out_lo, uint64_t out_hi, uint32_t* status) {
@@ -111,8 +115,9 @@
             if (right_blk && fqs && i == 0) { stop = true; break; }
             uint32_t nib;
             if (l2) {
-                const uint32_t word = trace[tbase + (v >> 3) * 8 + (w >> 1) * 2 + ((v >> 2) & 1)];
-                nib = ((word >> ((v & 3) * 8 + (w & 1) * 4)) ^ 15u) & 15u;
+                const uint32_t cb = slot_cell_byte<RO>(v & 7u);
+                const uint32_t word = trace[tbase + (v >> 3) * 8 + (w >> 1) * 2 + (cb >> 2)];
+                nib = ((word >> ((cb & 3) * 8 + (w & 1) * 4)) ^ 15u) & 15u;
             } else {
                 const uint32_t word = trace[tbase + (((w >> 2) * nch + chunk) * nl + lane) * (local ? 2u : 1u)];
                 nib = ((word >> ((v & 1) * 16 + (w & 3) * 4)) ^ 15u) & 15u;
@@ -158,7 +163,7 @@
     }
     return s - x;
 }
-template <bool L2OK>
+template <bool L2OK, bool RO = false>
 __device__ __forceinline__ uint32_t walk_wave(const BlockRec* __restrict__ blocks, uint32_t nblocks_in, const uint32_t* __restrict__ trace,
                                               uint32_t i_in, uint32_t j_in, const uint8_t* __restrict__ q, const uint8_t* __restrict__ r, bool eq,
                                               uint32_t* __restrict__ out, uint64_t out_lo, uint64_t out_hi, uint32_t* status,
@@ -236,7 +241,7 @@
                 const uint32_t ci = i - bi, cj = j - bj;
                 const uint32_t v = right ? ci : cj, w = right ? cj : ci;
                 uint32_t widx, sh;
-                if (l2) { widx = (v >> 3) * 8u + (w >> 1) * 2u + ((v >> 2) & 1u); sh = (v & 3u) * 8u + (w & 1u) * 4u; }
+                if (l2) { const uint32_t cb = slot_cell_byte<RO>(v & 7u); widx = (v >> 3) * 8u + (w >> 1) * 2u + (cb >> 2); sh = (cb & 3u) * 8u + (w & 1u) * 4u; }
                 else { widx = ((w >> 2) * nch + (v >> 7)) * nl + ((v & 127u) >> 1); sh = (v & 1u) * 16u + (w & 3u) * 4u; }
                 uint32_t word;
                 if (table == 0u && i > 0u && j > 0u && min(v, w) >= 1u) {
@@ -244,7 +249,7 @@
                     const bool valid = lane <= lim;
                     const uint32_t vv = v - lane, ww = w - lane;
                     uint32_t widx_k, sh_k;
-                    if (l2) { widx_k = (vv >> 3) * 8u + (ww >> 1) * 2u + ((vv >> 2) & 1u); sh_k = (vv & 3u) * 8u + (ww & 1u) * 4u; }
+                    if (l2) { const uint32_t cb = slot_cell_byte<RO>(vv & 7u); widx_k = (vv >> 3) * 8u + (ww >> 1) * 2u + (cb >> 2); sh_k = (cb & 3u) * 8u + (ww & 1u) * 4u; }
                     else { widx_k = ((ww >> 2) * nch + (vv >> 7)) * nl + ((vv & 127u) >> 1); sh_k = (vv & 1u) * 16u + (ww & 3u) * 4u; }
                     uint32_t word_k = 0;
                     if (valid) { if constexpr (DIRECT) word_k = trace[off + widx_k]; else word_k = lds[off + widx_k]; }
@@ -347,7 +352,7 @@
 #ifndef BA_HELPER_CELLS
 #define BA_HELPER_CELLS 4
 #endif
-template <int CELLS = TB_CELLS_PER_STEP, int DEPTH = 1, int LB = (int)TB_LANE_BYTES>
+template <int CELLS = TB_CELLS_PER_STEP, int DEPTH = 1, int LB = (int)TB_LANE_BYTES, bool RO = false>
 __device__ __forceinline__ void tb_step(TbLane& t, uint32_t flags, uint32_t* __restrict__ out, unsigned char* lrec,
                                         const unsigned char* lut, unsigned long long* tacc = nullptr) {
     constexpr bool LOCREC = LB == (int)TB_LANE_BYTES_LOC;
@@ -482,7 +487,7 @@
             if (L2OK && t.l2) {
                 const uint32_t k8 = (v >> 3) - t.tw_lane0;
                 alive = alive && t.tw_chunk == 0xffffu && k8 <= 1u;
-                baddr = k8 * 32 + (w >> 1) * 8 + ((v >> 2) & 1) * 4 + (v & 3);
+                baddr = k8 * 32 + (w >> 1) * 8 + slot_cell_byte<RO>(v & 7u);
                 zaddr = 64 + k8 * 8 + ((v >> 2) & 1) * 4 + (v & 3); zbit = w;
             } else {
                 const uint32_t k = lc - t.tw_lane0;
@@ -548,7 +553,7 @@
     if (t.bidx > 1u) t.nrec[1] = *(const uint4*)(t.blocks + t.bidx - 2);
     t.nq = min(2u, t.bidx);
 }
-template <bool L2W>
+template <bool L2W, bool RO = false>
 __device__ __forceinline__ void tb_diag_lut_fill(unsigned char* dlut) {
     if constexpr (L2W) {
 #pragma unroll
@@ -556,7 +561,7 @@
             const uint32_t idx = (uint32_t)lane_id() + 64u * e;
             const uint32_t k = idx & 7u, p = idx >> 3;
             const uint32_t x = (p - k) & 15u, c = ((p - 16u) - k) & 7u;
-            dlut[idx] = (unsigned char)(p < 16u ? (((x & 8u) << 2) | (x & 7u)) : ((c >> 1) << 3));
+            dlut[idx] = (unsigned char)(p < 16u ? (((x & 8u) << 2) | slot_cell_byte<RO>(x & 7u)) : ((c >> 1) << 3));
         }
     }
     {
@@ -645,7 +650,7 @@
     t.table = pos ? 0u : t.table;
 }
 
-template <int DEPTH, int LB>
+template <int DEPTH, int LB, bool RO = false>
 __device__ __forceinline__ void tb_step_fast(TbLane& t, const bool eq, uint32_t* __restrict__ out, unsigned char* lrec, const unsigned char* lut, const unsigned char* dlut) {
     static_assert(DEPTH >= 2 && DEPTH <= 4 && (BA_TB_FCELLS) >= 1 && (BA_TB_FCELLS) <= 2, "");
     constexpr bool L2OK = LB == (int)TB_LANE_BYTES_L2;
@@ -740,7 +745,7 @@
             if (L2OK && t.l2) {
                 const uint32_t k8 = (v >> 3) - t.tw_lane0;
                 alive = alive && t.tw_chunk == 0xffffu && k8 <= 1u;
-                baddr = k8 * 32 + (w >> 1) * 8 + ((v >> 2) & 1) * 4 + (v & 3);
+                baddr = k8 * 32 + (w >> 1) * 8 + slot_cell_byte<RO>(v & 7u);
             } else {
                 const uint32_t k = lc - t.tw_lane0;
                 alive = alive && (v >> 7) == t.tw_chunk && gi <= 1u && k <= 4u;
@@ -771,7 +776,7 @@
     if (ovf) { t.status |= ST_CIGAR_OVERFLOW; t.i = t.j = 0; }
 }
 
-template <int LB = (int)TB_LANE_BYTES, int CELLS = TB_CELLS_PER_STEP, int DEPTH = BA_RING_DEPTH>
+template <int LB = (int)TB_LANE_BYTES, int CELLS = TB_CELLS_PER_STEP, int DEPTH = BA_RING_DEPTH, bool RO = false>
 __device__ __forceinline__ void traceback_consumer(const BatchParams& bp, uint32_t flag_mask, unsigned char* tb_lds, uint32_t nlanes, bool dedicated, int prio = -1) {
     enum { IDLE = 0, WAIT = 1, WALK = 2, RETIRED = 3 };
     int phase = (uint32_t)lane_id() < nlanes ? IDLE : RETIRED;
@@ -790,7 +795,7 @@
         const Move mv = tb_lut(idx >> 6, idx & 3, (idx >> 2) & 1, (idx >> 4) & 3);
         lut[idx] = (unsigned char)(mv.op | (mv.di << 3) | (mv.dj << 4) | (mv.next << 5));
     }
-    if constexpr (FASTP) tb_diag_lut_fill<LB == (int)TB_LANE_BYTES_L2>(dlut);
+    if constexpr (FASTP) tb_diag_lut_fill<LB == (int)TB_LANE_BYTES_L2, RO>(dlut);
     lds_sync();
 #ifndef BA_TB_PRIO
 #define BA_TB_PRIO 3
@@ -846,16 +851,16 @@
 #ifdef BA_TIMING
             const unsigned long long tq0 = __builtin_amdgcn_s_memtime();
             if (t.i > 0 || t.j > 0) {
-                if constexpr (FASTP) tb_step_fast<BA_TB_FDEPTH, LB>(t, eq != 0u, bp.cig_ops, lrec, lut, dlut);
-                else tb_step<CELLS, DEPTH, LB>(t, eq, bp.cig_ops, lrec, lut, c_sec);
+                if constexpr (FASTP) tb_step_fast<BA_TB_FDEPTH, LB, RO>(t, eq != 0u, bp.cig_ops, lrec, lut, dlut);
+                else tb_step<CELLS, DEPTH, LB, RO>(t, eq, bp.cig_ops, lrec, lut, c_sec);
             }
             c_sec[2] += __builtin_amdgcn_s_memtime() - tq0;
 #else
             if (t.i > 0 || t.j > 0) {
-                if constexpr (FASTP) tb_step_fast<BA_TB_FDEPTH, LB>(t, eq != 0u, bp.cig_ops, lrec, lut, dlut);
+                if constexpr (FASTP) tb_step_fast<BA_TB_FDEPTH, LB, RO>(t, eq != 0u, bp.cig_ops, lrec, lut, dlut);
                 else
-                if (BA_HELPER_CELLS != CELLS && !dedicated) tb_step<BA_HELPER_CELLS, BA_WALK_DEPTH, LB>(t, eq, bp.cig_ops, lrec, lut);
-                else tb_step<CELLS, DEPTH, LB>(t, eq, bp.cig_ops, lrec, lut);
+                if (BA_HELPER_CELLS != CELLS && !dedicated) tb_step<BA_HELPER_CELLS, BA_WALK_DEPTH, LB, RO>(t, eq, bp.cig_ops, lrec, lut);
+                else tb_step<CELLS, DEPTH, LB, RO>(t, eq, bp.cig_ops, lrec, lut);
             }
 #endif
             if (!(t.i > 0 || t.j > 0)) {
@@ -884,7 +889,7 @@
 #endif
 }
 
-template <int LB = (int)TB_LANE_BYTES>
+template <int LB = (int)TB_LANE_BYTES, bool RO = false>
 __device__ __forceinline__ bool traceback_help_one(const BatchParams& bp, uint32_t flag_mask, unsigned char* tb_lds) {
     uint32_t entry = 0;
     if (is_lane(0)) {
@@ -927,7 +932,7 @@
         t.lo = bp.cig_off[t.pair]; t.wp = bp.cig_off[t.pair + 1];
         t.status = bp.status[t.pair];
         if (t.status || (bp.flags & 0x200u)) t.i = t.j = 0;
-        while (t.i > 0 || t.j > 0) tb_step<TB_CELLS_PER_STEP, BA_RING_DEPTH, LB>(t, eq, bp.cig_ops, lrec, lut);
+        while (t.i > 0 || t.j > 0) tb_step<TB_CELLS_PER_STEP, BA_RING_DEPTH, LB, RO>(t, eq, bp.cig_ops, lrec, lut);
         tb_emit(t, bp.cig_ops);
         bp.cig_len[t.pair] = t.status ? 0u : (uint32_t)(bp.cig_off[t.pair + 1] - t.wp);
         if (t.status) bp.status[t.pair] = t.status;
@@ -937,7 +942,7 @@
     return true;
 }
 
-template <bool L2OK>
+template <bool L2OK, bool RO = false>
 __device__ __forceinline__ void traceback_helper_wave(const BatchParams& bp, uint32_t* lds, uint32_t budget) {
     uint32_t* head = bp.tb_ctrl + 32;
     for (;;) {
@@ -961,7 +966,7 @@
         uint32_t st = bp.status[pair], ncig = 0;
         lds_sync();
         if (!st && !(bp.flags & 0x200u))
-            ncig = walk_wave<L2OK>(bp.blocks + (uint64_t)slot * bp.blocks_stride, si.nblocks, bp.trace_arena + (uint64_t)slot * bp.trace_stride, si.end_i, si.end_j,
+            ncig = walk_wave<L2OK, RO>(bp.blocks + (uint64_t)slot * bp.blocks_stride, si.nblocks, bp.trace_arena + (uint64_t)slot * bp.trace_stride, si.end_i, si.end_j,
                                    bp.pool + bp.q_off[pair], bp.pool + bp.r_off[pair], (bp.flags & F_CIGAR_EQ) != 0, bp.cig_ops, bp.cig_off[pair], bp.cig_off[pair + 1],
                                    &st, lds, budget);
         lds_sync();
@@ -1091,6 +1096,7 @@
 template <int PMAX, int KIND, bool TRACE, bool XDROP, bool SPECIAL, bool MULTI = false, int SLOT_B_ = 128>
 struct Aligner {
     static constexpr uint32_t SLOT_B = (uint32_t)SLOT_B_;
+    static constexpr bool SLOT_RO = MULTI && SLOT_B_ >= 128;
     typedef std::conditional_t<MULTI, PairState, NoState> RunOut;
     uint32_t h_flags, h_max_size; int h_x_drop;
     typedef const __attribute__((address_space(4))) BatchParams* ColdPtr;
@@ -1795,13 +1801,13 @@
             if constexpr (SPECIAL) {
                 if (is_lane(0)) {
                     uint32_t st = 0;
-                    ncig = traceback(blocks, nblocks, trace, ri, rj, q, r, h_flags, coldp()->cig_ops, coldp()->cig_off[pair], coldp()->cig_off[pair + 1], &st);
+                    ncig = traceback<SLOT_RO>(blocks, nblocks, trace, ri, rj, q, r, h_flags, coldp()->cig_ops, coldp()->cig_off[pair], coldp()->cig_off[pair + 1], &st);
                     status |= st;
                 }
             } else {
                 uint32_t st = 0;
                 lds_sync();
-                ncig = walk_wave<MULTI>(blocks, nblocks, trace, ri, rj, q, r, (h_flags & F_CIGAR_EQ) != 0, coldp()->cig_ops, coldp()->cig_off[pair],
+                ncig = walk_wave<MULTI, SLOT_RO>(blocks, nblocks, trace, ri, rj, q, r, (h_flags & F_CIGAR_EQ) != 0, coldp()->cig_ops, coldp()->cig_off[pair],
                                         coldp()->cig_off[pair + 1], &st, (uint32_t*)L.D_col, lds_array_bytes_h(kBig ? 128u : (uint32_t)PMAX * 128u));
                 lds_sync();
                 status |= st;
diff --git a/block_aligner_amd/csrc/ba_host.cpp b/block_aligner_amd/csrc/ba_host.cpp
--- a/block_aligner_amd/csrc/ba_host.cpp
+++ b/block_aligner_amd/csrc/ba_host.cpp
@@ -246,7 +246,7 @@
         bp.q_off = q_off.as<uint64_t>(); bp.q_len = q_len.as<uint32_t>();
         bp.r_off = r_off.as<uint64_t>(); bp.r_len = r_len.as<uint32_t>();
         bp.n = n; bp.gap_open = gap_open; bp.gap_extend = gap_extend;
-        bp.min_size = min_size; bp.max_size = max_size; bp.x_drop = x_drop; bp.flags = mode | (dev_env("BA_NO_FAST") ? 0x100u : 0u) | ((dev_env("BA_SKIP_WALK") || dev_env("BA_NO_TRACEBACK")) ? 0x200u : 0u) | ((handle_mode || dev_env("BA_NO_SPEC")) ? 0x400u : 0u) | (dev_env("BA_NO_TB_WAVES") ? 0x800u : 0u) | (dev_env("BA_NO_REFILL") ? 0x1000u : 0u) | (dev_env("BA_NO_STEAL") ? 0x2000u : 0u) | ((pad_negative && !dev_env("BA_NO_END_CLIP")) ? (uint32_t)ba::F_PAD_NEG : 0u);
+        bp.min_size = min_size; bp.max_size = max_size; bp.x_drop = x_drop; bp.flags = mode | (dev_env("BA_NO_FAST") ? 0x100u : 0u) | ((dev_env("BA_SKIP_WALK") || dev_env("BA_NO_TRACEBACK")) ? 0x200u : 0u) | ((handle_mode || dev_env("BA_NO_SPEC")) ? 0x400u : 0u) | (dev_env("BA_NO_TB_WAVES") ? 0x800u : 0u) | (dev_env("BA_NO_REFILL") ? 0x1000u : 0u) | (dev_env("BA_NO_STEAL") ? 0x2000u : 0u) | ((pad_negative && !dev_env("BA_NO_END_CLIP")) ? (uint32_t)ba::F_PAD_NEG : 0u) | (((uint64_t)pool.bytes + 2ull * max_size + 8ull > 0xffffffffull || dev_env("BA_POOL64")) ? (uint32_t)ba::F_POOL64 : 0u);
         bp.matrix = matrix.as<int8_t>();
         bp.score = score.as<int32_t>(); bp.query_idx = qidx.as<uint32_t>(); bp.reference_idx = ridx.as<uint32_t>();
         bp.cig_ops = ((mode & BA_TRACE) && !handle_mode && !dev_env("BA_NO_TRACEBACK")) ? cig_ops.as<uint32_t>() : nullptr;
diff --git a/block_aligner_amd/csrc/ba_multi.hpp b/block_aligner_amd/csrc/ba_multi.hpp
--- a/block_aligner_amd/csrc/ba_multi.hpp
+++ b/block_aligner_amd/csrc/ba_multi.hpp
@@ -184,10 +184,6 @@
                 const uint32_t nib = bfi(0x33333333u, lo2, hi2);
                 if (j & 1) tacc[2 * (j >> 1) + p2] = (int)bfi(0xF0F0F0F0u, nib, (uint32_t)tacc[2 * (j >> 1) + p2]);
                 else tacc[2 * (j >> 1) + p2] = (int)nib;
-            }
-            if (j & 1) {
-                const int wa = tacc[j - 1], wb = tacc[j];
-                tacc[j - 1] = __builtin_amdgcn_perm(wb, wa, 0x05040100); tacc[j] = __builtin_amdgcn_perm(wb, wa, 0x07060302);
             }
         }
         if (j >= 4) { nvD[j - 4] = __builtin_amdgcn_perm(dn[3], holdD[j - 4], 0x07060302); nvR[j - 4] = __builtin_amdgcn_perm(r[3], holdR[j - 4], 0x07060302); }
@@ -271,7 +267,7 @@
 #endif
     if (batch_traceback && wave == 0 && blockIdx.x % stride == 0) {
         if (!(bp.flags & 0x800u))
-        traceback_consumer<TB_LB, 8, 3>(bp, TB_MASK, (unsigned char*)base, 64u, true, 1);
+        traceback_consumer<TB_LB, 8, 3, true>(bp, TB_MASK, (unsigned char*)base, 64u, true, 1);
 #if defined(BA_TIMING) || defined(BA_ENDHIST)
         if (bp.prof && is_lane(0)) atomicMax(bp.prof + 42, (unsigned long long)__builtin_amdgcn_s_memrealtime());
 #endif
@@ -439,7 +435,7 @@
                         }
                         head = (uint32_t)uni((int)head);
                         if (head != seen) { seen = head; idle_n = 0; }
-                        else if ((++idle_n & 2047u) == 0 && traceback_help_one<TB_LB>(bp, TB_MASK, (unsigned char*)base)) idle_n = 0;
+                        else if ((++idle_n & 2047u) == 0 && traceback_help_one<TB_LB, true>(bp, TB_MASK, (unsigned char*)base)) idle_n = 0;
                         __builtin_amdgcn_s_sleep(64);
                     }
 #ifdef BA_TIMING
@@ -579,8 +575,8 @@
             const unsigned long long qa_r = TRACE ? 0ull : (unsigned long long)(bp.pool + (live ? bp.q_off[pair] : 0ull)), ra_r = TRACE ? 0ull : (unsigned long long)(bp.pool + (live ? bp.r_off[pair] : 0ull));
             const uint32_t qlen_r = (!TRACE && live) ? bp.q_len[pair] : 0u, rlen_r = (!TRACE && live) ? bp.r_len[pair] : 0u;
             if (TRACE && l == 0) {
-                const unsigned long long qa = (unsigned long long)(bp.pool + (live ? bp.q_off[pair] : 0ull)), ra = (unsigned long long)(bp.pool + (live ? bp.r_off[pair] : 0ull));
-                *(int4*)(lsc + MQ_LSC_PAIR) = int4{(int)(uint32_t)qa, (int)(uint32_t)(qa >> 32), (int)(uint32_t)ra, (int)(uint32_t)(ra >> 32)};
+                const unsigned long long qo = live ? bp.q_off[pair] : 0ull, ro = live ? bp.r_off[pair] : 0ull;
+                *(int4*)(lsc + MQ_LSC_PAIR) = int4{(int)(uint32_t)qo, (int)(uint32_t)(qo >> 32), (int)(uint32_t)ro, (int)(uint32_t)(ro >> 32)};
                 const long long room = (long long)tcap - (long long)(MQ_TW + 64u) - (long long)tt_in;
                 const unsigned long long nb_room = room < 0 ? 0ull : (unsigned long long)nblocks + (unsigned long long)room / MQ_TW + 1ull;
                 const uint32_t nb_lim = (uint32_t)(nb_room < (unsigned long long)bcap ? nb_room : (unsigned long long)bcap);
@@ -613,6 +609,8 @@
                 }
             };
             const uint32_t base32 = (uint32_t)(uintptr_t)base;
+            typedef const __attribute__((address_space(1))) uint8_t* glb_cu8_ptr;
+            typedef const __attribute__((address_space(1))) uint32_t* glb_cu32_ptr;
             do {
                 const bool right = dir == DIR_RIGHT;
                 uint32_t lid;
@@ -620,6 +618,10 @@
                 const uint32_t l8 = (lid & (uint32_t)(SL - 1)) * 8u;
                 const uint32_t lbuf_s = base32 + (lid / (uint32_t)SL) * (2u * BUFL) + 2u * l8;
                 const uint32_t lsc_s = base32 + (uint32_t)MQ_LDS_SCALARS + (lid / (uint32_t)SL) * (4u * (uint32_t)MQ_LSC_INTS);
+                const __attribute__((address_space(4))) BatchParams* kargs = (const __attribute__((address_space(4))) BatchParams*)__builtin_amdgcn_kernarg_segment_ptr();
+                asm volatile("" : "+s"(kargs));
+                const glb_cu8_ptr pool_g = (glb_cu8_ptr)kargs->pool;
+                const bool pool64 = TRACE && (kargs->flags & (uint32_t)F_POOL64);
                 int4 cA = {0, 0, 0, 0}, cB = {0, 0, 0, 0}, cC = {0, 0, 0, 0};
                 if (TRACE) {
                     typedef const __attribute__((address_space(3))) lds_v4i* lds_cint4_ptr;
@@ -627,8 +629,8 @@
                                   c4 = *(lds_cint4_ptr)(uintptr_t)(lsc_s + 4u * (MQ_LSC_PAIR + 8u));
                     cA = int4{a4.x, a4.y, a4.z, a4.w}; cB = int4{b4.x, b4.y, b4.z, b4.w}; cC = int4{c4.x, c4.y, c4.z, c4.w};
                 }
-                const uint8_t* const qp = TRACE ? (const uint8_t*)((unsigned long long)(uint32_t)cA.x | ((unsigned long long)(uint32_t)cA.y << 32)) : (const uint8_t*)qa_r;
-                const uint8_t* const rp = TRACE ? (const uint8_t*)((unsigned long long)(uint32_t)cA.z | ((unsigned long long)(uint32_t)cA.w << 32)) : (const uint8_t*)ra_r;
+                const uint8_t* const qp = (const uint8_t*)qa_r; const uint8_t* const rp = (const uint8_t*)ra_r;
+                const uint32_t qo32 = (uint32_t)cA.x, ro32 = (uint32_t)cA.z;
                 const uint32_t qlen = TRACE ? (uint32_t)cB.x : qlen_r, rlen = TRACE ? (uint32_t)cB.y : rlen_r;
                 const uint32_t ri = right ? si : sj, rj = (right ? sj : si) + (MB - STEP);
                 const uint32_t lenV = right ? qlen : rlen, lenC = right ? rlen : qlen;
@@ -651,18 +653,32 @@
                     vb = right ? pf_qv : pf_rv; cbv = right ? pf_rc : pf_qc;
                     if (__any(run && !pf_ok)) {
                         if (run && !pf_ok) {
+                            if constexpr (TRACE) {
+                                const unsigned long long vo = right ? ((unsigned long long)(uint32_t)cA.x | ((unsigned long long)(uint32_t)cA.y << 32)) : ((unsigned long long)(uint32_t)cA.z | ((unsigned long long)(uint32_t)cA.w << 32));
+                                const unsigned long long co = right ? ((unsigned long long)(uint32_t)cA.z | ((unsigned long long)(uint32_t)cA.w << 32)) : ((unsigned long long)(uint32_t)cA.x | ((unsigned long long)(uint32_t)cA.y << 32));
+                                const glb_cu32_ptr vp = (glb_cu32_ptr)(pool_g + (vo + (ri + l8))), cp = (glb_cu32_ptr)(pool_g + (co + rj));
+                                vb.x = vp[0]; vb.y = vp[1]; cbv.x = cp[0]; cbv.y = cp[1];
+                            } else {
                             const uint32_t* vp = (const uint32_t*)(Vp + (ri + l8));
                             vb.x = vp[0]; vb.y = vp[1];
                             const uint32_t* cp = (const uint32_t*)(Cp + rj);
                             cbv.x = cp[0]; cbv.y = cp[1];
+                            }
                         }
                     }
                     asm volatile("" : "+v"(vb.x), "+v"(vb.y));
-                    if (run) {
+                    if (!pool64) if (run) {
+                        if constexpr (TRACE) {
+                            const glb_cu32_ptr a = (glb_cu32_ptr)(pool_g + (unsigned long long)(qo32 + (si + l8))), b = (glb_cu32_ptr)(pool_g + (unsigned long long)(ro32 + (sj + l8)));
+                            const glb_cu32_ptr cq = (glb_cu32_ptr)(pool_g + (unsigned long long)(qo32 + si) + MB), cr = (glb_cu32_ptr)(pool_g + (unsigned long long)(ro32 + sj) + MB);
+                            pf_qv.x = a[0]; pf_qv.y = a[1]; pf_rv.x = b[0]; pf_rv.y = b[1];
+                            pf_qc.x = cq[0]; pf_qc.y = cq[1]; pf_rc.x = cr[0]; pf_rc.y = cr[1];
+                        } else {
                         const uint32_t* a = (const uint32_t*)(qp + (si + l8)); const uint32_t* b = (const uint32_t*)(rp + (sj + l8));
                         const uint32_t* cq = (const uint32_t*)(qp + si + MB); const uint32_t* cr = (const uint32_t*)(rp + sj + MB);
                         pf_qv.x = a[0]; pf_qv.y = a[1]; pf_rv.x = b[0]; pf_rv.y = b[1];
                         pf_qc.x = cq[0]; pf_qc.y = cq[1]; pf_rc.x = cr[0]; pf_rc.y = cr[1];
+                        }
                         pf_ok = true;
                     }
                 }
@@ -765,12 +781,12 @@
 #ifndef MQ_HELPER_LANES
 #define MQ_HELPER_LANES 0u
 #endif
-        if constexpr (SPM != 0) traceback_consumer<TB_LB>(bp, TB_MASK, (unsigned char*)base, 4u, false);
+        if constexpr (SPM != 0) traceback_consumer<TB_LB, TB_CELLS_PER_STEP, BA_RING_DEPTH, true>(bp, TB_MASK, (unsigned char*)base, 4u, false);
         else {
 #if MQ_HELPER_LANES == 0
-        traceback_helper_wave<true>(bp, (uint32_t*)base, 2048u);
+        traceback_helper_wave<true, true>(bp, (uint32_t*)base, 2048u);
 #else
-        traceback_consumer<(int)TB_LANE_BYTES_L2>(bp, (uint32_t)F_CIGAR_EQ, (unsigned char*)base, MQ_HELPER_LANES, false);
+        traceback_consumer<(int)TB_LANE_BYTES_L2, TB_CELLS_PER_STEP, BA_RING_DEPTH, true>(bp, (uint32_t)F_CIGAR_EQ, (unsigned char*)base, MQ_HELPER_LANES, false);
 #endif
         }
 #if defined(BA_TIMING) || defined(BA_ENDHIST)
diff --git a/block_aligner_amd/csrc/ba_params.h b/block_aligner_amd/csrc/ba_params.h
--- a/block_aligner_amd/csrc/ba_params.h
+++ b/block_aligner_amd/csrc/ba_params.h
@@ -10,6 +10,7 @@
 
 enum : uint32_t {
     F_TRACE = 1u << 0, F_XDROP = 1u << 1, F_LOCAL = 1u << 2, F_FQS = 1u << 3, F_FQE = 1u << 4, F_CIGAR_EQ = 1u << 5,
+    F_POOL64 = 1u << 15,
     F_PAD_NEG = 1u << 14
 };
 enum : uint32_t { ST_OK = 0, ST_TRACE_OVERFLOW = 1, ST_BLOCKS_OVERFLOW = 2, ST_CIGAR_OVERFLOW = 4, ST_TRACEBACK_LOST = 8, ST_WATCHDOG = 16, ST_SLOT_TIMEOUT = 32, ST_MODE = 64,
```

Measured after the change: 2684, median of 6. +1.5%, better.
